# eragonruan/text-detection-ctpn

Hardware: AMD Instinct MI355X
Metric: images/sec at 600x900 (VGG16-CTPN inference) (higher is better)
Workload: dtype bf16

## Files before the change

include/ctpn_hip.h:

```cpp
#ifndef CTPN_HIP_H
#define CTPN_HIP_H

#include <stddef.h>
#include <stdint.h>

#ifdef __cplusplus
extern "C" {
#endif

#define CTPN_ABI_VERSION 10

#define CTPN_OK            0
#define CTPN_ERR_ARG      -1
#define CTPN_ERR_HIP      -2
#define CTPN_ERR_STATE    -3
#define CTPN_ERR_CAPACITY -4
#define CTPN_ERR_NODEVICE -5
#define CTPN_ERR_UNSUPPORTED -6

#define CTPN_PREC_FP32  0
#define CTPN_PREC_BF16  1
#define CTPN_PREC_FP16  2
#define CTPN_PREC_SPLIT 3

// ... 59 lines not shown
                double fx, double fy, void* dst, int dst_on_device, long long dst_capacity,
                int* out_h, int* out_w);

int ctpn_nms(int* keep_out, int* num_out, const float* boxes_host, int boxes_num, int boxes_dim,
             float nms_overlap_thresh, int device_id);

int ctpn_text_lines(const float* boxes, const float* scores, int r, int im_h, int im_w, int mode,
                    int device_id, double* recs_out, int capacity, int* count_out);
int ctpn_text_lines_cfg(const float* boxes, const float* scores, int r, int im_h, int im_w, int mode,
                        int device_id, const double* cfg8, double* recs_out, int capacity, int* count_out);
int ctpn_connector_constants(double* out8);

int ctpn_result_text(const double* recs, int n_lines, double scale, char* out, size_t capacity, size_t* bytes_out, int* lines_out);
int ctpn_write_result_file(const char* path, const double* recs, int n_lines, double scale, int* lines_out);
int ctpn_draw_boxes(uint8_t* img_bgr, int h, int w, const double* recs, int n_lines);

int ctpn_detect(ctpn_ctx* ctx, const uint8_t* images, int images_on_device, int n, int h, int w,
                const float* scales, int mode, double* recs_out, int line_capacity, int* line_counts,
                float* rois_out, int* roi_counts);

int ctpn_detect_submit(ctpn_ctx* ctx, const uint8_t* images, int images_on_device, int n, int h, int w,
                       const float* scales, int slot);
int ctpn_detect_collect(ctpn_ctx* ctx, int slot, int mode, double* recs_out, int line_capacity, int* line_counts,
                        float* rois_out, int* roi_counts);

int ctpn_detect_ragged(ctpn_ctx* ctx, const uint8_t* canvas, int canvas_on_device, int n, int hc, int w, const int* heights,
                       const float* scales, int mode, double* recs_out, int line_capacity, int* line_counts,
                       float* rois_out, int* roi_counts);
int ctpn_detect_submit_ragged(ctpn_ctx* ctx, const uint8_t* canvas, int canvas_on_device, int n, int hc, int w, const int* heights,
                              const float* scales, int slot);

#define CTPN_KIND_CONV_FIRST  0
#define CTPN_KIND_CONV_GEMM   1
#define CTPN_KIND_POOL        2
#define CTPN_KIND_GEMM        3
#define CTPN_KIND_BILSTM      4
#define CTPN_KIND_DECODE      5
#define CTPN_KIND_SORT        6
#define CTPN_KIND_NMS         7
#define CTPN_KIND_COUNT       8
int ctpn_profile_enable(ctpn_ctx* ctx, int on);
int ctpn_profile_reset(ctpn_ctx* ctx);
int ctpn_profile_read(ctpn_ctx* ctx, int kind, double* ms, long long* launches, double* work);

int ctpn_debug_cvt_bf16(int device_id, const float* in, uint16_t* out, int n, int use_hw_instruction);
int ctpn_debug_lds_dma(int device_id, const uint8_t* src, size_t bytes, uint8_t* out_clobber, uint8_t* out_keep);
int ctpn_debug_conv3x3(int device_id, const float* in_nhwc, const float* w_hwio, const float* bias, int n, int h, int w,
                       int ci, int co, int precision, int impl, int fuse_pool, float* out_full, float* out_pool);
#define CTPN_CONV_PLAN_INTS 6
int ctpn_debug_conv3x3_plan(int precision, int n, int h, int w_first, int w_count, int ci, int co, int fuse_pool, int keep_full, int dup_hi,
                            int conv_p64, int split_edge, int cu_count, int* plans);
const char* ctpn_debug_conv3x3_form_name(int kind, int id);
int ctpn_debug_lstm_pre_plan(long long cells, int cu_count, int* plan_out);
int ctpn_debug_lstm_pre(int device_id, const float* x, const float* wx, const float* bias, int n, int hf, int wf, int precision, int cu_count,
                        float* out);
int ctpn_debug_bilstm(int device_id, const float* pre, const float* wh, int rows, int T, int split, int fast_gates, int pre_f16, float* out,
                      int* form_out);
int ctpn_debug_gemm(int device_id, const float* a, const float* w, const float* bias, int M, int K, int Co, int ldc, int in_precision, float* out);
int ctpn_debug_connect(int device_id, const float* rois, int r, int im_h, int im_w, float scale, int mode, double* recs_out,
                       int capacity, int* count_out);
int ctpn_debug_text_lines(ctpn_ctx* ctx, const float* rois, const int* roi_counts, int n, int im_h, int im_w, const float* scales, int mode,
                          double* recs_out, int line_capacity, int* line_counts, int* keep_out, int* keep_counts);

int    ctpn_jpeg_probe(const uint8_t* data, size_t len, int* h, int* w, int* ncomp, int* luma_sampling);
size_t ctpn_jpeg_coef_capacity(int h, int w);
int    ctpn_jpeg_entropy_decode(const uint8_t* data, size_t len, int16_t* coef, size_t coef_capacity, uint16_t* qt, int* layout8);
int    ctpn_decode_jpeg_batch(ctpn_ctx* ctx, const uint8_t* const* files, const size_t* sizes, int n, int h, int w, double fx, double fy,
                              const uint8_t** images_dev_out, int* out_h, int* out_w);
int    ctpn_decode_jpeg_files(ctpn_ctx* ctx, const char* const* paths, int n, int h, int w, double fx, double fy,
                              const uint8_t** images_dev_out, int* out_h, int* out_w);
int    ctpn_jpeg_probe_files(const char* const* paths, int n, int* info4, int threads);
int    ctpn_jpeg_batch_fetch(ctpn_ctx* ctx, const uint8_t* images_dev, uint8_t* host_out, size_t capacity);

int    ctpn_decode_jpeg_batch_device(ctpn_ctx* ctx, const uint8_t* const* files, const size_t* sizes, int n, int h, int w, double fx, double fy,
                                     const uint8_t** images_dev_out, int* out_h, int* out_w);
int    ctpn_decode_jpeg_files_device(ctpn_ctx* ctx, const char* const* paths, int n, int h, int w, double fx, double fy,
                                     const uint8_t** images_dev_out, int* out_h, int* out_w);
int    ctpn_jpeg_entropy_decode_device(ctpn_ctx* ctx, const uint8_t* const* files, const size_t* sizes, int n, int subseq_bits, int16_t* coef_out,
                                       size_t coef_capacity_per_file, uint16_t* qt_out, int* layout8_out, int* status_out);
int    ctpn_jpeg_entropy_device_stats(ctpn_ctx* ctx, long long* out4);

int    ctpn_decode_jpeg_batch_ragged(ctpn_ctx* ctx, const uint8_t* const* files, const size_t* sizes, int n, const int* file_h, const int* file_w,
                                     const double* factors, int hc, int wc, int entropy_on_device, const uint8_t** canvas_dev_out, int* heights_out);
int    ctpn_decode_jpeg_files_ragged(ctpn_ctx* ctx, const char* const* paths, int n, const int* file_h, const int* file_w, const double* factors,
                                     int hc, int wc, int entropy_on_device, const uint8_t** canvas_dev_out, int* heights_out);

size_t ctpn_jpeg_encode_capacity(int h, int w);
int    ctpn_jpeg_entropy_encode(const int16_t* coef, const int* layout8, const uint16_t* qt, uint8_t* out, size_t capacity, size_t* bytes_out);
int    ctpn_encode_jpeg_batch(ctpn_ctx* ctx, const uint8_t* images, int images_on_device, int n, int h, int w, int quality, uint8_t* const* out,
                              const size_t* capacities, size_t* bytes_out);
int    ctpn_write_annotated_files(ctpn_ctx* ctx, const uint8_t* images_dev, int n, int h, int w, const double* recs, int line_capacity,
                                  const int* line_counts, double scale, const char* const* paths, int quality);

int    ctpn_encode_jpeg_batch_device(ctpn_ctx* ctx, const uint8_t* images, int images_on_device, int n, int h, int w, int quality, uint8_t* const* out,
                                     const size_t* capacities, size_t* bytes_out);
int    ctpn_write_annotated_files_device(ctpn_ctx* ctx, const uint8_t* images_dev, int n, int h, int w, const double* recs, int line_capacity,
                                         const int* line_counts, double scale, const char* const* paths, int quality);
int    ctpn_jpeg_entropy_encode_device(ctpn_ctx* ctx, const int16_t* const* coef, const int* layout8, const uint16_t* qt, int n, uint8_t* const* out,
                                       const size_t* capacities, size_t* bytes_out, int* status_out);
int    ctpn_jpeg_entropy_encode_device_stats(ctpn_ctx* ctx, long long* out4);

int    ctpn_line_crop_width(const double* rec9, int crop_h, int max_w, int* width_out);
int    ctpn_crop_lines(ctpn_ctx* ctx, const uint8_t* images, int images_on_device, int n, int h, int w, const double* recs, int line_capacity,
                       const int* line_counts, int crop_h, int max_w, int pad_value, uint8_t* crops_out, int crops_on_device,
                       size_t capacity_bytes, int* widths_out, int* total_out);

// ... 48 lines not shown
```

text-detection-ctpn_amd/_binding.py:

```python
import collections
import ctypes as C
import os
import sys

import numpy as np

_HERE = os.path.dirname(os.path.abspath(__file__))
_LIB = None

CTPN_OK = 0
CTPN_ERR_UNSUPPORTED = -6
CTPN_ERR_CAPACITY = -4
PREC_FP32, PREC_BF16, PREC_FP16, PREC_SPLIT = 0, 1, 2, 3
PRECISIONS = {"fp32": PREC_FP32, "f32": PREC_FP32, "bf16": PREC_BF16, "fp16": PREC_FP16, "f16": PREC_FP16, "split": PREC_SPLIT}


def precision_code(p):
    if isinstance(p, int) and p in (PREC_FP32, PREC_BF16, PREC_FP16, PREC_SPLIT):
        return p
    try:
        return PRECISIONS[p]
    except KeyError:
        raise ValueError("unknown precision %r (fp32 | bf16 | fp16 | split)" % (p,))

# ... 30 lines not shown
        "ctpn_param_name": (C.c_char_p, [C.c_int]),
        "ctpn_param_default": (C.c_int, [C.c_char_p, f64p]),
        "ctpn_last_error": (C.c_char_p, []),
        "ctpn_device_count": (C.c_int, []),
        "ctpn_create": (C.c_int, [C.POINTER(vp), C.c_int, C.c_int, C.c_int, C.c_int, C.c_int]),
        "ctpn_create_postproc": (C.c_int, [C.POINTER(vp), C.c_int, C.c_int, C.c_int, C.c_int]),
        "ctpn_host_thread_budget": (C.c_int, [C.c_int, C.c_int, C.c_int]),
        "ctpn_host_threads": (C.c_int, [vp, i32p]),
        "ctpn_proposal_anchors": (C.c_int, [vp, i32p, C.c_int]),
        "ctpn_debug_connect": (C.c_int, [C.c_int, f32p, C.c_int, C.c_int, C.c_int, C.c_float, C.c_int, f64p, C.c_int, i32p]),
        "ctpn_debug_text_lines": (C.c_int, [vp, f32p, i32p, C.c_int, C.c_int, C.c_int, f32p, C.c_int, f64p, C.c_int, i32p, i32p, i32p]),
        "ctpn_destroy": (C.c_int, [vp]),
        "ctpn_sync": (C.c_int, [vp]),
        "ctpn_stream": (C.c_int, [vp, C.POINTER(vp)]),
        "ctpn_weight_manifest": (C.c_int, [C.c_int, C.POINTER(C.c_char_p), i32p, i32p, C.POINTER(C.c_size_t)]),
        "ctpn_weight_count": (C.c_int, []),
        "ctpn_load_weights_host": (C.c_int, [vp, f32p]),
        "ctpn_load_weights_device": (C.c_int, [vp, vp]),
        "ctpn_broadcast_weights": (C.c_int, [C.POINTER(vp), C.c_int]),
        "ctpn_comm_unique_id": (C.c_int, [C.c_char_p, C.c_size_t]),
        "ctpn_broadcast_weights_rank": (C.c_int, [vp, C.c_char_p, C.c_int, C.c_int, C.c_int]),
        "ctpn_forward": (C.c_int, [vp, vp, C.c_int, C.c_int, C.c_int, C.c_int]),
        "ctpn_forward_blob": (C.c_int, [vp, vp, C.c_int, C.c_int, C.c_int, C.c_int]),
        "ctpn_ragged_valid_rows": (C.c_int, [C.c_int, C.c_int]),
        "ctpn_forward_ragged": (C.c_int, [vp, vp, C.c_int, C.c_int, C.c_int, C.c_int, i32p]),
        "ctpn_detect_ragged": (C.c_int, [vp, vp, C.c_int, C.c_int, C.c_int, C.c_int, i32p, f32p, C.c_int, f64p, C.c_int, i32p, f32p, i32p]),
        "ctpn_detect_submit_ragged": (C.c_int, [vp, vp, C.c_int, C.c_int, C.c_int, C.c_int, i32p, f32p, C.c_int]),
        "ctpn_feat_shape": (C.c_int, [vp, i32p, i32p, i32p]),
        "ctpn_get_tensor": (C.c_int, [vp, C.c_char_p, f32p, C.c_size_t, i32p]),
        "ctpn_proposals": (C.c_int, [vp, f32p, C.c_int, C.c_int, C.c_float, C.c_float, f32p, i32p]),
        "ctpn_proposals_from_host": (C.c_int, [vp, f32p, f32p, C.c_int, C.c_int, C.c_int, f32p, C.c_int, C.c_int,
                                               C.c_float, C.c_float, f32p, i32p]),
        "ctpn_nms": (C.c_int, [i32p, i32p, f32p, C.c_int, C.c_int, C.c_float, C.c_int]),
        "ctpn_resize_dims": (C.c_int, [C.c_int, C.c_int, C.c_double, C.c_double, i32p, i32p]),
        "ctpn_resize": (C.c_int, [C.c_int, vp, C.c_int, C.c_int, C.c_int, C.c_int, C.c_int, C.c_double, C.c_double, vp, C.c_int,
                                  C.c_longlong, i32p, i32p]),
        "ctpn_result_text": (C.c_int, [f64p, C.c_int, C.c_double, C.c_char_p, C.c_size_t, C.POINTER(C.c_size_t), i32p]),
        "ctpn_write_result_file": (C.c_int, [C.c_char_p, f64p, C.c_int, C.c_double, i32p]),
        "ctpn_draw_boxes": (C.c_int, [u8p, C.c_int, C.c_int, f64p, C.c_int]),
        "ctpn_text_lines": (C.c_int, [f32p, f32p, C.c_int, C.c_int, C.c_int, C.c_int, C.c_int, f64p, C.c_int, i32p]),
        "ctpn_text_lines_cfg": (C.c_int, [f32p, f32p, C.c_int, C.c_int, C.c_int, C.c_int, C.c_int, f64p, f64p, C.c_int, i32p]),
        "ctpn_connector_constants": (C.c_int, [f64p]),
        "ctpn_detect": (C.c_int, [vp, vp, C.c_int, C.c_int, C.c_int, C.c_int, f32p, C.c_int, f64p, C.c_int, i32p,
                                  f32p, i32p]),
        "ctpn_detect_submit": (C.c_int, [vp, vp, C.c_int, C.c_int, C.c_int, C.c_int, f32p, C.c_int]),
        "ctpn_detect_collect": (C.c_int, [vp, C.c_int, C.c_int, f64p, C.c_int, i32p, f32p, i32p]),
        "ctpn_debug_cvt_bf16": (C.c_int, [C.c_int, f32p, C.POINTER(C.c_uint16), C.c_int, C.c_int]),
        "ctpn_debug_lds_dma": (C.c_int, [C.c_int, u8p, C.c_size_t, u8p, u8p]),
        "ctpn_debug_conv3x3": (C.c_int, [C.c_int, f32p, f32p, f32p, C.c_int, C.c_int, C.c_int, C.c_int, C.c_int, C.c_int, C.c_int,
                                         C.c_int, f32p, f32p]),
        "ctpn_debug_conv3x3_plan": (C.c_int, [C.c_int] * 13 + [i32p]),
        "ctpn_debug_conv3x3_form_name": (C.c_char_p, [C.c_int, C.c_int]),
        "ctpn_debug_lstm_pre_plan": (C.c_int, [C.c_longlong, C.c_int, i32p]),
        "ctpn_debug_lstm_pre": (C.c_int, [C.c_int, f32p, f32p, f32p, C.c_int, C.c_int, C.c_int, C.c_int, C.c_int, f32p]),
        "ctpn_debug_bilstm": (C.c_int, [C.c_int, f32p, f32p, C.c_int, C.c_int, C.c_int, C.c_int, C.c_int, f32p, i32p]),
        "ctpn_debug_gemm": (C.c_int, [C.c_int, f32p, f32p, f32p, C.c_int, C.c_int, C.c_int, C.c_int, C.c_int, f32p]),
        "ctpn_jpeg_probe": (C.c_int, [u8p, C.c_size_t, i32p, i32p, i32p, i32p]),
        "ctpn_jpeg_coef_capacity": (C.c_size_t, [C.c_int, C.c_int]),
        "ctpn_jpeg_entropy_decode": (C.c_int, [u8p, C.c_size_t, C.POINTER(C.c_int16), C.c_size_t, C.POINTER(C.c_uint16), i32p]),
        "ctpn_decode_jpeg_batch": (C.c_int, [vp, C.POINTER(u8p), C.POINTER(C.c_size_t), C.c_int, C.c_int, C.c_int, C.c_double, C.c_double,
                                             C.POINTER(vp), i32p, i32p]),
        "ctpn_jpeg_batch_fetch": (C.c_int, [vp, vp, u8p, C.c_size_t]),
        "ctpn_decode_jpeg_files": (C.c_int, [vp, C.POINTER(C.c_char_p), C.c_int, C.c_int, C.c_int, C.c_double, C.c_double, C.POINTER(vp), i32p, i32p]),
        "ctpn_jpeg_probe_files": (C.c_int, [C.POINTER(C.c_char_p), C.c_int, i32p, C.c_int]),
        "ctpn_decode_jpeg_batch_device": (C.c_int, [vp, C.POINTER(u8p), C.POINTER(C.c_size_t), C.c_int, C.c_int, C.c_int, C.c_double, C.c_double,
                                                    C.POINTER(vp), i32p, i32p]),
        "ctpn_decode_jpeg_files_device": (C.c_int, [vp, C.POINTER(C.c_char_p), C.c_int, C.c_int, C.c_int, C.c_double, C.c_double, C.POINTER(vp), i32p, i32p]),
        "ctpn_jpeg_entropy_decode_device": (C.c_int, [vp, C.POINTER(u8p), C.POINTER(C.c_size_t), C.c_int, C.c_int, C.POINTER(C.c_int16), C.c_size_t,
                                                      C.POINTER(C.c_uint16), i32p, i32p]),
        "ctpn_jpeg_entropy_device_stats": (C.c_int, [vp, C.POINTER(C.c_longlong)]),
        "ctpn_decode_jpeg_batch_ragged": (C.c_int, [vp, C.POINTER(u8p), C.POINTER(C.c_size_t), C.c_int, i32p, i32p, f64p, C.c_int, C.c_int, C.c_int,
                                                    C.POINTER(vp), i32p]),
        "ctpn_decode_jpeg_files_ragged": (C.c_int, [vp, C.POINTER(C.c_char_p), C.c_int, i32p, i32p, f64p, C.c_int, C.c_int, C.c_int, C.POINTER(vp), i32p]),
        "ctpn_jpeg_encode_capacity": (C.c_size_t, [C.c_int, C.c_int]),
        "ctpn_jpeg_entropy_encode": (C.c_int, [C.POINTER(C.c_int16), i32p, C.POINTER(C.c_uint16), u8p, C.c_size_t, C.POINTER(C.c_size_t)]),
        "ctpn_encode_jpeg_batch": (C.c_int, [vp, vp, C.c_int, C.c_int, C.c_int, C.c_int, C.c_int, C.POINTER(vp), C.POINTER(C.c_size_t),
                                             C.POINTER(C.c_size_t)]),
        "ctpn_write_annotated_files": (C.c_int, [vp, vp, C.c_int, C.c_int, C.c_int, f64p, C.c_int, i32p, C.c_double, C.POINTER(C.c_char_p), C.c_int]),
        "ctpn_encode_jpeg_batch_device": (C.c_int, [vp, vp, C.c_int, C.c_int, C.c_int, C.c_int, C.c_int, C.POINTER(vp), C.POINTER(C.c_size_t),
                                                    C.POINTER(C.c_size_t)]),
        "ctpn_write_annotated_files_device": (C.c_int, [vp, vp, C.c_int, C.c_int, C.c_int, f64p, C.c_int, i32p, C.c_double, C.POINTER(C.c_char_p), C.c_int]),
        "ctpn_jpeg_entropy_encode_device": (C.c_int, [vp, C.POINTER(C.POINTER(C.c_int16)), i32p, C.POINTER(C.c_uint16), C.c_int, C.POINTER(vp), C.POINTER(C.c_size_t),
                                                      C.POINTER(C.c_size_t), i32p]),
        "ctpn_jpeg_entropy_encode_device_stats": (C.c_int, [vp, C.POINTER(C.c_longlong)]),
        "ctpn_line_crop_width": (C.c_int, [f64p, C.c_int, C.c_int, i32p]),
        "ctpn_crop_lines": (C.c_int, [vp, vp, C.c_int, C.c_int, C.c_int, C.c_int, f64p, C.c_int, i32p, C.c_int, C.c_int, C.c_int, vp, C.c_int, C.c_size_t,
                                      i32p, i32p]),
        "ctpn_encode_jpeg_mixed": (C.c_int, [vp, vp, C.c_int, C.c_size_t, C.c_int, i32p, i32p, C.POINTER(C.c_size_t), C.POINTER(C.c_size_t), C.c_int,
                                             C.POINTER(vp), C.POINTER(C.c_size_t), C.POINTER(C.c_size_t)]),
        "ctpn_encode_jpeg_mixed_device": (C.c_int, [vp, vp, C.c_int, C.c_size_t, C.c_int, i32p, i32p, C.POINTER(C.c_size_t), C.POINTER(C.c_size_t), C.c_int,
                                                    C.POINTER(vp), C.POINTER(C.c_size_t), C.POINTER(C.c_size_t)]),
        "ctpn_write_line_crops": (C.c_int, [vp, vp, C.c_int, C.c_int, C.c_int, C.c_int, f64p, C.c_int, i32p, C.c_int, C.c_int, C.c_int, C.c_int,
                                            C.POINTER(C.c_char_p), i32p, i32p]),
        "ctpn_write_line_crops_device": (C.c_int, [vp, vp, C.c_int, C.c_int, C.c_int, C.c_int, f64p, C.c_int, i32p, C.c_int, C.c_int, C.c_int, C.c_int,
                                                   C.POINTER(C.c_char_p), i32p, i32p]),
        "ctpn_write_annotated_files_ragged": (C.c_int, [vp, vp, C.c_int, C.c_int, C.c_int, C.c_int, i32p, f64p, C.c_int, i32p, f64p, C.POINTER(C.c_char_p),
                                                        C.c_int]),
        "ctpn_write_annotated_files_ragged_device": (C.c_int, [vp, vp, C.c_int, C.c_int, C.c_int, C.c_int, i32p, f64p, C.c_int, i32p, f64p,
                                                               C.POINTER(C.c_char_p), C.c_int]),
        "ctpn_crop_lines_ragged": (C.c_int, [vp, vp, C.c_int, C.c_int, C.c_int, C.c_int, i32p, f64p, C.c_int, i32p, C.c_int, C.c_int, C.c_int, vp, C.c_int,
                                             C.c_size_t, i32p, i32p]),
        "ctpn_write_line_crops_ragged": (C.c_int, [vp, vp, C.c_int, C.c_int, C.c_int, C.c_int, i32p, f64p, C.c_int, i32p, C.c_int, C.c_int, C.c_int, C.c_int,
                                                   C.POINTER(C.c_char_p), i32p, i32p]),
        "ctpn_write_line_crops_ragged_device": (C.c_int, [vp, vp, C.c_int, C.c_int, C.c_int, C.c_int, i32p, f64p, C.c_int, i32p, C.c_int, C.c_int, C.c_int, C.c_int,
                                                          C.POINTER(C.c_char_p), i32p, i32p]),
        "ctpn_debug_png_backend": (C.c_int, [C.c_int]),
# ... 528 lines not shown
    out = np.zeros((rows, T, 256), np.float32)
    form = C.c_int(-1)
    _check(load_library().ctpn_debug_bilstm(int(device_id), _ptr(pre, C.c_float), _ptr(wh, C.c_float), rows, T, 1 if split else 0,
                                            1 if fast_gates else 0, 1 if pre_f16 else 0, _ptr(out, C.c_float), C.byref(form)))
    return out, BILSTM_FORMS[form.value]


def debug_gemm(a, w, bias, ldc=None, precision="fp32", device_id=0):
    a = _f32(a); w = _f32(w); bias = _f32(bias)
    (M, K), Co = a.shape, w.shape[1]
    assert w.shape[0] == K and bias.shape == (Co,)
    ldc = Co if ldc is None else int(ldc)
    out = np.zeros((M, ldc), np.float32)
    _check(load_library().ctpn_debug_gemm(int(device_id), _ptr(a, C.c_float), _ptr(w, C.c_float), _ptr(bias, C.c_float), M, K, Co, ldc,
                                          precision_code(precision), _ptr(out, C.c_float)))
    return out


class Context:

    def __init__(self, device_id=0, max_batch=1, max_h=600, max_w=900, precision="bf16", postproc_only=False, options=None):
        self._lib = load_library()
        self._h = C.c_void_p()
        self.precision = precision
        self.postproc_only = bool(postproc_only)
        prec = precision_code(precision)
        if postproc_only:
            _check(self._lib.ctpn_create_postproc(C.byref(self._h), int(device_id), int(max_batch), int(max_h) // 16, int(max_w) // 16))
        else:
            _check(self._lib.ctpn_create(C.byref(self._h), int(device_id), int(max_batch), int(max_h), int(max_w), prec))
        self.device_id = device_id
        self.max_batch, self.max_h, self.max_w = max_batch, max_h, max_w
        opts = {k: int(os.environ[e]) for k, e in OPTION_ENV.items() if os.environ.get(e, "") != ""}
        opts.update(options or {})
        for k, v in opts.items():
            self.set_option(k, v)

    def set_option(self, key, value):
        _check(self._lib.ctpn_set_option(self._h, key.encode(), int(value)))

    def get_option(self, key):
        v = C.c_int(0)
        _check(self._lib.ctpn_get_option(self._h, key.encode(), C.byref(v)))
        return v.value

    def set_param(self, name, value):
        _check(self._lib.ctpn_set_param(self._h, name.encode(), float(value)))

    def get_param(self, name):
        v = C.c_double(0.0)
        _check(self._lib.ctpn_get_param(self._h, name.encode(), C.byref(v)))
        return v.value

    def host_threads(self):
        n = C.c_int(0)
        _check(self._lib.ctpn_host_threads(self._h, C.byref(n)))
        return n.value

    def close(self):
        if getattr(self, "_h", None) is not None and self._h.value:
            self._lib.ctpn_destroy(self._h)
            self._h = C.c_void_p()

    def __del__(self):
        try:
            self.close()
        except Exception:
            pass

    def __enter__(self):
        return self

    def __exit__(self, *a):
        self.close()

    def load_weights(self, arena):
        a = _f32(arena).reshape(-1)
        from .weights import WEIGHT_FLOATS
        if a.size != WEIGHT_FLOATS:
            raise ValueError("weight arena must hold %d floats, got %d" % (WEIGHT_FLOATS, a.size))
        _check(self._lib.ctpn_load_weights_host(self._h, _ptr(a, C.c_float)))

    def load_weights_device(self, dev_ptr):
        _check(self._lib.ctpn_load_weights_device(self._h, C.c_void_p(int(dev_ptr))))

    def broadcast_weights_rank(self, unique_id, rank, world, root=0):
        if len(unique_id) != COMM_ID_BYTES:
            raise ValueError("unique_id must be %d bytes" % COMM_ID_BYTES)
        _check(self._lib.ctpn_broadcast_weights_rank(self._h, C.c_char_p(bytes(unique_id)), int(rank), int(world), int(root)))

    def forward(self, images, device_ptr=None, shape=None):
        if device_ptr is not None:
            n, h, w = shape
            _check(self._lib.ctpn_forward(self._h, C.c_void_p(int(device_ptr)), 1, int(n), int(h), int(w)))
            return
        im = np.ascontiguousarray(images, dtype=np.uint8)
        if im.ndim == 3:
            im = im[None]
        n, h, w, c = im.shape
        assert c == 3
        self._keepalive = im
        _check(self._lib.ctpn_forward(self._h, im.ctypes.data_as(C.c_void_p), 0, n, h, w))

    @staticmethod
    def _canvas(canvas, heights, device_ptr, shape):
        if device_ptr is not None:
# ... 486 lines not shown
```

text-detection-ctpn_amd/csrc/api_ctx.hip:

```cpp
#include "ctx.h"

namespace ctpn {

static thread_local std::string t_err;
void set_error(const std::string& s) { t_err = s; }
int fail(int code, const std::string& s) { t_err = s; return code; }

static int env_int(const char* name, int dflt) { const char* v = std::getenv(name); return v && *v ? std::atoi(v) : dflt; }

static int dev_alloc(ctpn_ctx* c, void** p, size_t bytes, bool zero) {
  if (bytes == 0) bytes = 256;
  CTPN_HIP_TRY(hipMalloc(p, bytes));
  c->allocs.push_back(*p);
  if (zero) CTPN_HIP_TRY(hipMemsetAsync(*p, 0, bytes, c->stream));
  return CTPN_OK;
}

int debug_sync() { static const int v = env_int("CTPN_DEBUG_SYNC", 0); return v; }
const RoctxApi& roctx_api() {
  static const RoctxApi api = [] {
    RoctxApi a;
    if (!env_int("CTPN_ROCTX", 0)) return a;
    void* h = dlopen("librocprofiler-sdk-roctx.so", RTLD_NOW | RTLD_GLOBAL);
    if (!h) h = dlopen("librocprofiler-sdk-roctx.so.1", RTLD_NOW | RTLD_GLOBAL);
    if (!h) {
      const char* rp = std::getenv("ROCM_PATH");
      const std::string p = std::string(rp && *rp ? rp : "/opt/rocm") + "/lib/librocprofiler-sdk-roctx.so";
      h = dlopen(p.c_str(), RTLD_NOW | RTLD_GLOBAL);
    }
    if (h) {
      a.push = (int (*)(const char*))dlsym(h, "roctxRangePushA");
      a.pop = (int (*)())dlsym(h, "roctxRangePop");
      if (!a.push || !a.pop) { a.push = nullptr; a.pop = nullptr; }
    }
    return a;
  }();
  return api;
}
int roctx_on() { return roctx_api().push != nullptr; }

static int prof_drain(ctpn_ctx* c) {
  if (c->pending.empty()) return CTPN_OK;
  CTPN_HIP_TRY(hipStreamSynchronize(c->stream));
  CTPN_HIP_TRY(hipStreamSynchronize(c->stream_p));
  for (auto& r : c->pending) {
    float ms = 0.f;
    if (hipEventElapsedTime(&ms, r.a, r.b) == hipSuccess) {
      c->prof_ms[r.kind] += ms; c->prof_n[r.kind] += r.launches; c->prof_work[r.kind] += r.work;
    }
    c->free_events.push_back(r.a); c->free_events.push_back(r.b);
  }
  c->pending.clear();
  return CTPN_OK;
}

struct PackLayout { size_t tlb, tls, keep, kcnt, rois, rcnt, total; };
static PackLayout pack_layout(size_t mb, size_t post) {
  auto al = [](size_t x) { return (x + 255) & ~(size_t)255; };
  PackLayout L; size_t o = 0;
  L.tlb = o; o = al(o + mb * post * 4 * sizeof(float));
  L.tls = o; o = al(o + mb * post * sizeof(float));
  L.keep = o; o = al(o + mb * post * sizeof(int));
  L.kcnt = o; o = al(o + mb * sizeof(int));
  L.rois = o; o = al(o + mb * post * 5 * sizeof(float));
  L.rcnt = o; o = al(o + mb * sizeof(int));
  L.total = o;
  return L;
}

static int create_impl(ctpn_ctx** out, int device_id, int max_batch, int max_h, int max_w, int precision, bool postproc_only) {
  if (!out) return fail(CTPN_ERR_ARG, "ctpn_create: out is null");
  *out = nullptr;
  if (max_batch <= 0 || max_h < 16 || max_w < 16) return fail(CTPN_ERR_ARG, "ctpn_create: max_batch > 0 and max_h, max_w >= 16 required");
  if (precision < CTPN_PREC_FP32 || precision > CTPN_PREC_SPLIT) return fail(CTPN_ERR_ARG, "ctpn_create: unknown precision");
  int ndev = ctpn_device_count();
  if (ndev <= 0) return fail(CTPN_ERR_NODEVICE, "ctpn_create: no HIP device visible (this library has no CPU fallback)");
  if (device_id < 0 || device_id >= ndev) {
    const char* hv = getenv("HIP_VISIBLE_DEVICES");
    const char* rv = getenv("ROCR_VISIBLE_DEVICES");
    return fail(CTPN_ERR_ARG, "ctpn_create: device_id " + std::to_string(device_id) + " out of range: " + std::to_string(ndev) +
                " device(s) visible (HIP_VISIBLE_DEVICES=" + (hv ? hv : "unset") + ", ROCR_VISIBLE_DEVICES=" + (rv ? rv : "unset") + "); one process per GPU needs LOCAL_RANK < that count");
  }
  CTPN_HIP_TRY(hipSetDevice(device_id));
  hipDeviceProp_t prop;
  CTPN_HIP_TRY(hipGetDeviceProperties(&prop, device_id));
  if (std::string(prop.gcnArchName).find("gfx950") == std::string::npos)
    return fail(CTPN_ERR_NODEVICE, std::string("ctpn_create: device is ") + prop.gcnArchName + ", kernels are built for gfx950 only");

  ctpn_ctx* c = new ctpn_ctx();
  c->device = device_id; c->max_batch = max_batch; c->max_h = max_h; c->max_w = max_w;
  c->prec = prec_dtype(precision);
  c->es = dtype_bytes(c->prec);
  c->wx_row_bytes = c->prec == DType::SPLIT ? (size_t)3 * 512 * 2 : (size_t)512 * c->es;
  c->lstm_split = (dtype_is_half(c->prec) || c->prec == DType::SPLIT) ? 1 : 0;
  c->tail_confine = 0;
  c->postproc_only = postproc_only;
  for (int i = 0; i < TAIL_PARAM_COUNT; ++i) c->tail_raw[i] = tail_param(i)->dflt;
  {
    const unsigned hw = std::thread::hardware_concurrency();
    c->host_threads = ctpn_host_thread_budget((int)(hw ? hw : 1), env_int("LOCAL_WORLD_SIZE", 1), env_int("CTPN_HOST_THREADS", 0));
    const int first_cpu = env_int("CTPN_AFFINITY", 0) ? env_int("LOCAL_RANK", 0) * c->host_threads : -1;
    c->pool.reset(new HostPool(c->host_threads, first_cpu));
  }
  int rc = CTPN_OK;
  auto A = [&](void** p, size_t bytes, bool zero) { if (rc == CTPN_OK) rc = dev_alloc(c, p, bytes, zero); };
  if (hipStreamCreateWithFlags(&c->stream, hipStreamNonBlocking) != hipSuccess) { delete c; return fail(CTPN_ERR_HIP, "hipStreamCreate failed"); }
  if (hipStreamCreateWithFlags(&c->stream_p, hipStreamNonBlocking) != hipSuccess) { (void)hipStreamDestroy(c->stream); delete c; return fail(CTPN_ERR_HIP, "hipStreamCreate failed"); }
  if (hipEventCreateWithFlags(&c->ev_conv, hipEventDisableTiming) != hipSuccess || hipEventCreateWithFlags(&c->ev_tail, hipEventDisableTiming) != hipSuccess) {
    ctpn_destroy(c); return fail(CTPN_ERR_HIP, "ctpn_create: events");
  }
  for (auto& sl : c->slot) {
    const size_t mb = (size_t)max_batch;
    const PackLayout L = pack_layout(mb, (size_t)c->post_max);
    bool ok = hipHostMalloc((void**)&sl.pack, L.total) == hipSuccess;
    if (ok) {
      sl.tlb = (float*)(sl.pack + L.tlb); sl.tls = (float*)(sl.pack + L.tls); sl.keep = (int*)(sl.pack + L.keep); sl.kcnt = (int*)(sl.pack + L.kcnt);
      sl.rois = (float*)(sl.pack + L.rois); sl.rcnt = (int*)(sl.pack + L.rcnt);
    }
    ok = ok &&
              hipHostMalloc((void**)&sl.im_info, mb * 3 * sizeof(float)) == hipSuccess &&
              hipHostMalloc((void**)&sl.crecs, mb * 2 * CONN_CAP * 9 * sizeof(double)) == hipSuccess &&
              hipHostMalloc((void**)&sl.ccnt, mb * 3 * sizeof(int)) == hipSuccess &&
              hipEventCreateWithFlags(&sl.ev_heads, hipEventDisableTiming) == hipSuccess &&
              hipEventCreateWithFlags(&sl.ev_decoded, hipEventDisableTiming) == hipSuccess &&
              hipEventCreateWithFlags(&sl.ev_done, hipEventDisableTiming) == hipSuccess;
    if (!ok) { ctpn_destroy(c); return fail(CTPN_ERR_HIP, "ctpn_create: pinned host buffers / events"); }
  }

  const int hf = lvl(max_h, 4), wf = lvl(max_w, 4);
  c->m5_max = (size_t)max_batch * hf * wf;
  if (!postproc_only) {
  A((void**)&c->arena, (size_t)CTPN_WEIGHT_FLOATS * sizeof(float), false);
  A((void**)&c->w_first, 27 * 64 * sizeof(float), false);
  A(&c->w_first_frags, CF_FRAGS_TOTAL, true);
  for (int i = 0; i < 14; ++i) {
    A((void**)&c->b_conv[i], (size_t)kConvs[i].co * sizeof(float), true);
    if (i > 0) A(&c->wt_conv[i], (size_t)kConvs[i].co * 9 * kConvs[i].ci * (c->prec == DType::SPLIT ? 6 : c->es), true);
  }
  A(&c->wt_x, (size_t)1024 * c->wx_row_bytes, true);
  if (dtype_is_half(c->prec)) A(&c->wt_xf, (size_t)1024 * 512 * 2, true);
  A((void**)&c->b_x, 1024 * sizeof(float), true);
  A((void**)&c->wh, (size_t)2 * 128 * 512 * sizeof(float), true);
  A((void**)&c->wt_fc, (size_t)512 * 256 * sizeof(float), true);
  A((void**)&c->b_fc, 512 * sizeof(float), true);
  A((void**)&c->wt_h, (size_t)64 * 512 * sizeof(float), true);
  A((void**)&c->b_h, 64 * sizeof(float), true);
  A((void**)&c->wt_fold, (size_t)64 * 256 * sizeof(float), true);
  A((void**)&c->b_fold, 64 * sizeof(float), true);

  for (int i = 0; i < 14; ++i) {
    const int hl = lvl(max_h, kConvs[i].level), wl = lvl(max_w, kConvs[i].level);
    const size_t pix_b = (size_t)kConvs[i].co * ((c->prec == DType::SPLIT && i == 13) ? 6 : c->es);
    c->act_conv_bytes[i] = ((size_t)max_batch * (hl + 2) * (wl + 2) + act_slack_pixels(wl)) * pix_b;
    const size_t front = act_front_pixels(wl) * pix_b;
    A(&c->act_conv[i], front + c->act_conv_bytes[i], true);
    if (c->act_conv[i]) c->act_conv[i] = (char*)c->act_conv[i] + front;
  }
  {
    const int pool_src[4] = {1, 3, 6, 9};
    for (int p = 0; p < 4; ++p) {
      const int hl = lvl(max_h, p + 1), wl = lvl(max_w, p + 1);
      c->act_pool_bytes[p] = ((size_t)max_batch * (hl + 2) * (wl + 2) + act_slack_pixels(wl)) * kConvs[pool_src[p]].co * c->es;
      const size_t front = act_front_pixels(wl) * kConvs[pool_src[p]].co * c->es;
      A(&c->act_pool[p], front + c->act_pool_bytes[p], true);
      if (c->act_pool[p]) c->act_pool[p] = (char*)c->act_pool[p] + front;
    }
  }
  if (dtype_is_half(c->prec)) { c->q_img_bytes = conv1_q_bytes(max_batch, max_h, max_w); A(&c->q_img, c->q_img_bytes, true); }
  A((void**)&c->img_dev, (size_t)max_batch * max_h * max_w * 3 * sizeof(float), false);
  c->img_dev_b[0] = c->img_dev;
  A((void**)&c->img_dev_b[1], (size_t)max_batch * max_h * max_w * 3 * sizeof(float), false);
  if (rc == CTPN_OK) {
    bool ok = hipStreamCreateWithFlags(&c->stream_c, hipStreamNonBlocking) == hipSuccess;
    for (int b = 0; b < 2 && ok; ++b)
      ok = hipEventCreateWithFlags(&c->ev_copied[b], hipEventDisableTiming) == hipSuccess && hipEventCreateWithFlags(&c->ev_consumed[b], hipEventDisableTiming) == hipSuccess;
    if (!ok) rc = fail(CTPN_ERR_HIP, "ctpn_create: copy stream / events");
  }
  A((void**)&c->xp, c->m5_max * 1024 * sizeof(float), false);
  A((void**)&c->lstm_out, c->m5_max * 256 * sizeof(float), false);
  A((void**)&c->fc_out, c->m5_max * 512 * sizeof(float), false);
  A((void**)&c->heads, c->m5_max * 64 * sizeof(float), true);
  }
  A((void**)&c->cls_prob, c->m5_max * 20 * sizeof(float), false);
  A((void**)&c->bbox_pred, c->m5_max * 40 * sizeof(float), false);
  A((void**)&c->cls_in, c->m5_max * 20 * sizeof(float), false);
  A((void**)&c->bbox_in, c->m5_max * 40 * sizeof(float), false);
  c->npad_max = next_pow2(hf * wf * 10);
  A((void**)&c->keys, (size_t)max_batch * c->npad_max * sizeof(unsigned long long), false);
  A((void**)&c->keys_tmp, (size_t)max_batch * c->npad_max * sizeof(unsigned long long), false);
  A((void**)&c->boxes4, (size_t)max_batch * hf * wf * 10 * 4 * sizeof(float), false);
  A((void**)&c->sorted_boxes, (size_t)max_batch * c->topn_max * 4 * sizeof(float), false);
  A((void**)&c->sorted_scores, (size_t)max_batch * c->topn_max * sizeof(float), false);
  A((void**)&c->valid_counts, (size_t)max_batch * sizeof(int), true);
  A((void**)&c->keep_idx, (size_t)max_batch * c->topn_max * sizeof(int), false);
  {
    const PackLayout L = pack_layout((size_t)max_batch, (size_t)c->post_max);
    c->pack_bytes = L.total;
    A((void**)&c->out_pack, L.total, true);
    if (c->out_pack) {
      c->tl_boxes = (float*)(c->out_pack + L.tlb); c->tl_scores = (float*)(c->out_pack + L.tls); c->tl_keep = (int*)(c->out_pack + L.keep);
      c->tl_keep_counts = (int*)(c->out_pack + L.kcnt); c->rois = (float*)(c->out_pack + L.rois); c->keep_counts = (int*)(c->out_pack + L.rcnt);
    }
  }
  A((void**)&c->kept_spill, (size_t)max_batch * c->topn_max * 4 * sizeof(float), false);
  A((void**)&c->sorted_anchor, (size_t)max_batch * c->topn_max * sizeof(int), false);
  A((void**)&c->roi_anchor, (size_t)max_batch * c->post_max * sizeof(int), true);
  A((void**)&c->tl_counts, (size_t)max_batch * sizeof(int), true);
  A((void**)&c->tl_spill, (size_t)max_batch * c->post_max * 4 * sizeof(float), false);
  A((void**)&c->nms_mw_scratch, (size_t)NMS_MW_CAP_BATCH * NMS_MW_SCRATCH_BYTES, true);
  A((void**)&c->nms_colid, (size_t)NMS_MW_CAP_BATCH * ((c->topn_max + 15) & ~15), true);
  A((void**)&c->conn_recs, (size_t)max_batch * 2 * CONN_CAP * 9 * sizeof(double), false);
  A((void**)&c->conn_counts, (size_t)max_batch * 3 * sizeof(int), true);
  A((void**)&c->conn_scratch, (size_t)max_batch * 1024 * 20 * sizeof(double), false);
  A((void**)&c->im_info_dev, (size_t)max_batch * 3 * sizeof(float), true);
  if (rc == CTPN_OK && hipStreamSynchronize(c->stream) != hipSuccess) rc = fail(CTPN_ERR_HIP, "ctpn_create: sync failed");
  if (rc != CTPN_OK) { ctpn_destroy(c); return rc; }
  *out = c;
  return CTPN_OK;
}

struct Option { const char* name; int ctpn_ctx::* member; int lo, hi; };
static const Option kOptions[] = {
    {"keep_acts", &ctpn_ctx::keep_acts, 0, 1},
    {"conv1_kernel", &ctpn_ctx::conv1_mfma, 0, 2},
    {"conv1_fuse", &ctpn_ctx::conv1_fuse, 0, 1},
    {"lstm_split", &ctpn_ctx::lstm_split, 0, 1},
    {"nms_columns", &ctpn_ctx::nms_columns, 0, 3},
    {"nms_check", &ctpn_ctx::nms_check, 0, 1},
    {"connect_device", &ctpn_ctx::connect_device, 0, 1},
    {"tail_overlap", &ctpn_ctx::tail_overlap, 0, 1},
    {"conv_p64", &ctpn_ctx::conv_p64, 0, 1},
    {"tail_confine", &ctpn_ctx::tail_confine, 0, 1},
    {"nms_prefix", &ctpn_ctx::nms_prefix, 0, 1},
    {"debug_hog", &ctpn_ctx::debug_hog, 0, 200000},
    {"debug_nms", &ctpn_ctx::debug_nms, 0, 15},
    {"split_edge", &ctpn_ctx::split_edge, 0, 1},
};
static const Option* find_option(const std::string& k) {
  for (const Option& o : kOptions) if (k == o.name) return &o;
  return nullptr;
}

}

extern "C" {

int ctpn_abi_version(void) { return CTPN_ABI_VERSION; }
const char* ctpn_last_error(void) { return t_err.c_str(); }
int ctpn_device_count(void) {
  int n = 0;
  if (hipGetDeviceCount(&n) != hipSuccess) return 0;
  return n;
}

int ctpn_host_thread_budget(int cpu_count, int local_world_size, int requested) {
  if (requested > 0) return requested > 256 ? 256 : requested;
  if (cpu_count < 1) cpu_count = 1;
  if (local_world_size < 1) local_world_size = 1;
  int b = cpu_count / local_world_size;
  return b < 1 ? 1 : (b > 32 ? 32 : b);
}

int ctpn_create(ctpn_ctx** out, int device_id, int max_batch, int max_h, int max_w, int precision) {
  return create_impl(out, device_id, max_batch, max_h, max_w, precision, false);
}

int ctpn_create_postproc(ctpn_ctx** out, int device_id, int max_batch, int max_hf, int max_wf) {
  if (max_hf < 1 || max_wf < 1 || max_hf > (1 << 20) / 16 || max_wf > (1 << 20) / 16) return fail(CTPN_ERR_ARG, "ctpn_create_postproc: feature-map size out of range");
  return create_impl(out, device_id, max_batch, max_hf * 16, max_wf * 16, CTPN_PREC_FP32, true);
}

int ctpn_option_count(void) { return (int)(sizeof(kOptions) / sizeof(kOptions[0])); }
const char* ctpn_option_name(int index) { return index >= 0 && index < ctpn_option_count() ? kOptions[index].name : nullptr; }
int ctpn_set_option(ctpn_ctx* c, const char* key, int value) {
  if (!c || !key) return fail(CTPN_ERR_ARG, "ctpn_set_option: null pointer");
  const Option* o = find_option(key);
  if (!o) return fail(CTPN_ERR_ARG, std::string("ctpn_set_option: unknown option ") + key);
  if (value < o->lo || value > o->hi) return fail(CTPN_ERR_ARG, std::string("ctpn_set_option: value out of range for ") + key);
  if (c->*(o->member) == value) return CTPN_OK;
  CTPN_HIP_TRY(hipSetDevice(c->device));
  CTPN_HIP_TRY(hipStreamSynchronize(c->stream));
  CTPN_HIP_TRY(hipStreamSynchronize(c->stream_p));
  for (auto& sl : c->slot) if (sl.busy) return fail(CTPN_ERR_STATE, "ctpn_set_option: a submitted batch has not been collected");
  c->tail_pending = false;
  c->nms_mw_dirty = true;
  c->*(o->member) = value;
  return CTPN_OK;
}
int ctpn_get_option(ctpn_ctx* c, const char* key, int* value_out) {
  if (!c || !key || !value_out) return fail(CTPN_ERR_ARG, "ctpn_get_option: null pointer");
  const Option* o = find_option(key);
  if (!o) return fail(CTPN_ERR_ARG, std::string("ctpn_get_option: unknown option ") + key);
  *value_out = c->*(o->member);
  return CTPN_OK;
}

int ctpn_set_param(ctpn_ctx* c, const char* name, double value) {
  if (!c || !name) return fail(CTPN_ERR_ARG, "ctpn_set_param: null pointer");
  const int idx = tail_param_index(name);
  if (idx < 0) return fail(CTPN_ERR_ARG, std::string("ctpn_set_param: unknown parameter ") + name);
  if (!tail_param_ok(idx, value)) return fail(CTPN_ERR_ARG, std::string("ctpn_set_param: value out of range for ") + name);
  if (c->tail_raw[idx] == value) return CTPN_OK;
  CTPN_HIP_TRY(hipSetDevice(c->device));
  CTPN_HIP_TRY(hipStreamSynchronize(c->stream));
  CTPN_HIP_TRY(hipStreamSynchronize(c->stream_p));
  for (auto& sl : c->slot) if (sl.busy) return fail(CTPN_ERR_STATE, "ctpn_set_param: a submitted batch has not been collected");
  c->tail_pending = false;
  c->nms_mw_dirty = true;
  c->tail_raw[idx] = value;
  switch (idx) {
    case TP_RPN_PRE_NMS_TOP_N: c->rpn_pre = (int)value; break;
    case TP_RPN_POST_NMS_TOP_N: c->rpn_post = (int)value; break;
    case TP_RPN_NMS_THRESH: c->rpn_nms_thresh = (float)value; break;
    case TP_RPN_MIN_SIZE: c->rpn_min_size = (float)value; break;
    default: connector_cfg_set(c->conn, idx, value); break;
  }
  return CTPN_OK;
}
int ctpn_get_param(ctpn_ctx* c, const char* name, double* value_out) {
  if (!c || !name || !value_out) return fail(CTPN_ERR_ARG, "ctpn_get_param: null pointer");
  const int idx = tail_param_index(name);
  if (idx < 0) return fail(CTPN_ERR_ARG, std::string("ctpn_get_param: unknown parameter ") + name);
  *value_out = c->tail_raw[idx];
  return CTPN_OK;
}

int ctpn_host_threads(ctpn_ctx* c, int* threads_out) {
  if (!c || !threads_out) return fail(CTPN_ERR_ARG, "null pointer");
  *threads_out = c->host_threads;
  return CTPN_OK;
}

int ctpn_destroy(ctpn_ctx* c) {
  if (!c) return CTPN_OK;
  (void)hipSetDevice(c->device);
  if (c->stream) (void)hipStreamSynchronize(c->stream);
  if (c->stream_p) (void)hipStreamSynchronize(c->stream_p);
  if (c->stream_c) { (void)hipStreamSynchronize(c->stream_c); (void)hipStreamDestroy(c->stream_c); }
  for (int b = 0; b < 2; ++b) { if (c->pin_stage[b]) (void)hipHostFree(c->pin_stage[b]); if (c->ev_h2d_done[b]) (void)hipEventDestroy(c->ev_h2d_done[b]); }
  for (int b = 0; b < 2; ++b) { if (c->ev_copied[b]) (void)hipEventDestroy(c->ev_copied[b]); if (c->ev_consumed[b]) (void)hipEventDestroy(c->ev_consumed[b]); }
  for (auto& sl : c->slot) {
    for (void* p : {(void*)sl.pack, (void*)sl.im_info, (void*)sl.crecs, (void*)sl.ccnt}) if (p) (void)hipHostFree(p);
    for (hipEvent_t e : {sl.ev_heads, sl.ev_decoded, sl.ev_done}) if (e) (void)hipEventDestroy(e);
  }
  for (hipEvent_t e : {c->ev_conv, c->ev_tail}) if (e) (void)hipEventDestroy(e);
  for (auto& r : c->ragged) { if (r.host) (void)hipHostFree(r.host); if (r.dev) (void)hipFree(r.dev); if (r.ev_copied) (void)hipEventDestroy(r.ev_copied); }
  if (c->ragged_blob) (void)hipFree(c->ragged_blob);
  for (auto& j : c->jpeg) {
    if (j.coef_host) (void)hipHostFree(j.coef_host);
    if (j.qt_host) (void)hipHostFree(j.qt_host);
    if (j.tab_host) (void)hipHostFree(j.tab_host);
    for (void* p : {(void*)j.coef_dev, (void*)j.qt_dev, (void*)j.out_dev, (void*)j.tab_dev}) if (p) (void)hipFree(p);
    for (hipEvent_t e : {j.ev_h2d, j.ev_ready, j.ev_consumed}) if (e) (void)hipEventDestroy(e);
  }
  for (void* p : {(void*)c->jpeg_planes, (void*)c->jpeg_raw}) if (p) (void)hipFree(p);
  for (void* p : {(void*)c->jh.stage_dev, (void*)c->jh.work_dev}) if (p) (void)hipFree(p);
  for (void* p : {(void*)c->jh.stage_host, (void*)c->jh.res_host}) if (p) (void)hipHostFree(p);
  for (void* p : c->jpeg_retired) (void)hipFree(p);
  for (void* p : {(void*)c->stage.img_dev, (void*)c->stage.rs_dev, (void*)c->stage.recs_dev, (void*)c->stage.cnt_dev, (void*)c->stage.rm_dev}) if (p) (void)hipFree(p);
  if (c->stage.rm_host) (void)hipHostFree(c->stage.rm_host);
  for (void* p : {(void*)c->enc.coef_dev, c->enc.qtab_dev, (void*)c->enc.huff_dev, c->enc.huff_tab_dev, (void*)c->enc.mix_dev}) if (p) (void)hipFree(p);
  for (void* p : {(void*)c->enc.coef_host, c->enc.qtab_host, (void*)c->enc.huff_host, (void*)c->enc.scan_host, (void*)c->enc.mix_host}) if (p) (void)hipHostFree(p);
  if (c->enc.ev_done) (void)hipEventDestroy(c->enc.ev_done);
  if (c->pnge.dev) (void)hipFree(c->pnge.dev);
  for (void* p : {(void*)c->pnge.host, (void*)c->pnge.file_host}) if (p) (void)hipHostFree(p);
  if (c->pnge.ev_done) (void)hipEventDestroy(c->pnge.ev_done);
  for (void* p : {(void*)c->crop.img_dev, (void*)c->crop.out_dev, c->crop.desc_dev}) if (p) (void)hipFree(p);
  if (c->crop.desc_host) (void)hipHostFree(c->crop.desc_host);
  if (c->crop.ev_done) (void)hipEventDestroy(c->crop.ev_done);
  if (c->stream_p) (void)hipStreamDestroy(c->stream_p);
  for (auto& r : c->pending) { (void)hipEventDestroy(r.a); (void)hipEventDestroy(r.b); }
  for (auto e : c->free_events) (void)hipEventDestroy(e);
  for (void* p : c->allocs) (void)hipFree(p);
  if (c->stream) (void)hipStreamDestroy(c->stream);
  delete c;
  return CTPN_OK;
}

int ctpn_sync(ctpn_ctx* c) {
  if (!c) return fail(CTPN_ERR_ARG, "null ctx");
  CTPN_HIP_TRY(hipStreamSynchronize(c->stream));
  CTPN_HIP_TRY(hipStreamSynchronize(c->stream_p));
  if (c->stream_c) CTPN_HIP_TRY(hipStreamSynchronize(c->stream_c));
  return CTPN_OK;
}
int ctpn_stream(ctpn_ctx* c, void** stream_out) {
  if (!c || !stream_out) return fail(CTPN_ERR_ARG, "null pointer");
  *stream_out = (void*)c->stream;
  return CTPN_OK;
}

int ctpn_profile_enable(ctpn_ctx* c, int on) {
  if (!c) return fail(CTPN_ERR_ARG, "null ctx");
  if (!on) { int rc = prof_drain(c); if (rc) return rc; }
  c->prof = on != 0;
  c->prof_mode = on == 2 ? 2 : 1;
  return CTPN_OK;
}
int ctpn_profile_reset(ctpn_ctx* c) {
  if (!c) return fail(CTPN_ERR_ARG, "null ctx");
  int rc = prof_drain(c);
  if (rc) return rc;
  for (int k = 0; k < CTPN_KIND_COUNT; ++k) { c->prof_ms[k] = 0; c->prof_n[k] = 0; c->prof_work[k] = 0; }
  return CTPN_OK;
}
int ctpn_profile_read(ctpn_ctx* c, int kind, double* ms, long long* launches, double* work) {
  if (!c) return fail(CTPN_ERR_ARG, "null ctx");
  if (kind < 0 || kind >= CTPN_KIND_COUNT) return fail(CTPN_ERR_ARG, "kind out of range");
  int rc = prof_drain(c);
  if (rc) return rc;
  if (ms) *ms = c->prof_ms[kind];
  if (launches) *launches = c->prof_n[kind];
  if (work) *work = c->prof_work[kind];
  return CTPN_OK;
}

}
```

text-detection-ctpn_amd/csrc/api_debug.hip:

```cpp
#include "ctx.h"
#include "conv3x3_plan.h"

extern "C" {

int ctpn_debug_cvt_bf16(int device_id, const float* in, uint16_t* out, int n, int use_hw_instruction) {
  if (!in || !out || n <= 0) return fail(CTPN_ERR_ARG, "ctpn_debug_cvt_bf16: bad argument");
  if (ctpn_device_count() <= 0) return fail(CTPN_ERR_NODEVICE, "ctpn_debug_cvt_bf16: no HIP device visible (no CPU fallback)");
  CTPN_HIP_TRY(hipSetDevice(device_id));
  float* d_in = nullptr; uint16_t* d_out = nullptr;
  CTPN_HIP_TRY(hipMalloc((void**)&d_in, (size_t)n * 4));
  CTPN_HIP_TRY(hipMalloc((void**)&d_out, (size_t)n * 2 + 4));
  CTPN_HIP_TRY(hipMemcpy(d_in, in, (size_t)n * 4, hipMemcpyHostToDevice));
  int rc = launch_cvt_bf16(d_in, d_out, n, use_hw_instruction, nullptr);
  if (!rc && hipDeviceSynchronize() != hipSuccess) rc = fail(CTPN_ERR_HIP, "ctpn_debug_cvt_bf16: kernel failed");
  if (!rc && hipMemcpy(out, d_out, (size_t)n * 2, hipMemcpyDeviceToHost) != hipSuccess) rc = fail(CTPN_ERR_HIP, "ctpn_debug_cvt_bf16: copy failed");
  (void)hipFree(d_in); (void)hipFree(d_out);
  return rc;
}

int ctpn_debug_lds_dma(int device_id, const uint8_t* src, size_t bytes, uint8_t* out_clobber, uint8_t* out_keep) {
  if (!src || !out_clobber || !out_keep || bytes == 0 || bytes % 1024 != 0 || bytes > ((size_t)1 << 30)) return fail(CTPN_ERR_ARG, "ctpn_debug_lds_dma: bytes must be a positive multiple of 1024 (<= 1 GiB)");
  if (ctpn_device_count() <= 0) return fail(CTPN_ERR_NODEVICE, "ctpn_debug_lds_dma: no HIP device visible (no CPU fallback)");
  CTPN_HIP_TRY(hipSetDevice(device_id));
  char *d_in = nullptr, *d_a = nullptr, *d_b = nullptr;
// ... 114 lines not shown
        out_pool[(((size_t)in * ho + y) * wo + x) * co + c] = std::max(std::max(at(2 * y, 2 * x), at(2 * y, 2 * x + 1)), std::max(at(2 * y + 1, 2 * x), at(2 * y + 1, 2 * x + 1)));
      }
  }
  if (!rc && out_pool && fuse_pool && !host_pool) rc = fetch(d_pool, ho, wo, out_pool, 0);
  return rc;
}

int ctpn_debug_conv3x3_plan(int precision, int n, int h, int w_first, int w_count, int ci, int co, int fuse_pool, int keep_full, int dup_hi,
                            int conv_p64, int split_edge, int cu_count, int* plans) {
  if (!plans || w_count <= 0) return fail(CTPN_ERR_ARG, "ctpn_debug_conv3x3_plan: no output");
  if (precision < CTPN_PREC_FP32 || precision > CTPN_PREC_SPLIT) return fail(CTPN_ERR_ARG, "ctpn_debug_conv3x3_plan: unknown precision");
  const DType t = prec_dtype(precision);
  if (n <= 0 || h <= 0 || w_first <= 0 || w_first > 0x7fffffff - w_count || ci <= 0 || ci % (t == DType::F32 ? 32 : 64) != 0 || co <= 0 || co % (t == DType::F32 ? 4 : 8) != 0)
    return fail(CTPN_ERR_ARG, "ctpn_debug_conv3x3_plan: shape out of range (Ci a multiple of 32 / 64, Co of 4 / 8)");
  if (dup_hi && t != DType::SPLIT) return fail(CTPN_ERR_ARG, "ctpn_debug_conv3x3_plan: dup_hi is a split-precision layout");
  if (cu_count < 0) return fail(CTPN_ERR_ARG, "ctpn_debug_conv3x3_plan: cu_count is a CU count, or 0 for the current device's");
  if (cu_count == 0) {
    if (ctpn_device_count() <= 0) return fail(CTPN_ERR_NODEVICE, "ctpn_debug_conv3x3_plan: cu_count 0 asks the current device, and no HIP device is visible");
    int dev = 0, rc;
    if ((rc = current_device(dev)) || (rc = device_cu_count(dev, cu_count))) return rc;
  }
  for (int i = 0; i < w_count; ++i) {
    const C3Plan p = c3_plan(t, n, h, w_first + i, ci, co, fuse_pool != 0, keep_full != 0 || !fuse_pool, dup_hi, true, true, (conv_p64 ? 1 : 0) | (split_edge ? 2 : 0), cu_count);
    if (p.main_form == C3M_NONE) return fail(CTPN_ERR_ARG, "ctpn_debug_conv3x3_plan: no kernel for this shape (split precision: Co <= 64 or a multiple of 128)");
    int* o = plans + (size_t)i * CTPN_CONV_PLAN_INTS;
    o[0] = p.main_form; o[1] = p.strip; o[2] = p.strip_cols; o[3] = p.w_cover; o[4] = p.deep; o[5] = p.edge_ks;
  }
  return CTPN_OK;
}

const char* ctpn_debug_conv3x3_form_name(int kind, int id) { return kind == 0 ? c3_main_name(id) : (kind == 1 ? c3_strip_name(id) : nullptr); }

}
namespace {
constexpr int DBG_GUARD_ROWS = 64;
constexpr int DBG_FILL = 0xC3;
bool dbg_fill_intact(const char* p, size_t n) {
  for (size_t i = 0; i < n; ++i) if ((unsigned char)p[i] != DBG_FILL) return false;
  return true;
}
inline uint16_t dbg_to16(DType t, float v) { return t == DType::F16 ? host_f32_to_f16(v) : host_f32_to_bf16(v); }
struct DevBufs {
  std::vector<void*> p;
  ~DevBufs() { for (void* q : p) if (q) (void)hipFree(q); }
  int alloc(void** out, size_t bytes) {
    CTPN_HIP_TRY(hipMalloc(out, bytes));
    p.push_back(*out);
    return CTPN_OK;
  }
};
}
extern "C" {

int ctpn_debug_lstm_pre_plan(long long cells, int cu_count, int* plan_out) {
  if (!plan_out) return fail(CTPN_ERR_ARG, "ctpn_debug_lstm_pre_plan: no output");
  if (cells <= 0 || cells > 0x7fffffffLL) return fail(CTPN_ERR_ARG, "ctpn_debug_lstm_pre_plan: cells out of range (1 .. 2^31 - 1)");
  if (cu_count < 0) return fail(CTPN_ERR_ARG, "ctpn_debug_lstm_pre_plan: cu_count is a CU count, or 0 for the current device's");
  if (cu_count == 0) {
    if (ctpn_device_count() <= 0) return fail(CTPN_ERR_NODEVICE, "ctpn_debug_lstm_pre_plan: cu_count 0 asks the current device, and no HIP device is visible");
    int dev = 0, rc;
    if ((rc = current_device(dev)) || (rc = device_cu_count(dev, cu_count))) return rc;
  }
  const LstmPrePlan p = lstm_pre_plan(cells, cu_count);
  plan_out[0] = p.small ? 0 : 1; plan_out[1] = p.waves; plan_out[2] = (int)p.workgroups; plan_out[3] = p.idle_waves;
  return CTPN_OK;
}

int ctpn_debug_lstm_pre(int device_id, const float* x, const float* wx, const float* bias, int n, int hf, int wf, int precision, int cu_count, float* out) {
  if (!x || !wx || !bias || !out) return fail(CTPN_ERR_ARG, "ctpn_debug_lstm_pre: null pointer");
  if (precision < CTPN_PREC_FP32 || precision > CTPN_PREC_SPLIT) return fail(CTPN_ERR_ARG, "ctpn_debug_lstm_pre: unknown precision");
  if (n <= 0 || hf <= 0 || wf <= 0 || (long long)n * hf * wf > (1 << 24)) return fail(CTPN_ERR_ARG, "ctpn_debug_lstm_pre: n, hf, wf positive, at most 2^24 cells");
  if (cu_count < 0) return fail(CTPN_ERR_ARG, "ctpn_debug_lstm_pre: cu_count is a CU count, or 0 for the current device's");
  if (ctpn_device_count() <= 0) return fail(CTPN_ERR_NODEVICE, "ctpn_debug_lstm_pre: no HIP device visible (no CPU fallback)");
  CTPN_HIP_TRY(hipSetDevice(device_id));
  const DType t = prec_dtype(precision);
  const bool split = t == DType::SPLIT, half = dtype_is_half(t);
  const long long M = (long long)n * hf * wf;
  const int Hp = hf + 2, Wp = wf + 2;
  const int es = t == DType::F32 ? 4 : 2, pix = split ? 1536 : 512;
  const int oes = half ? 2 : 4;
  std::vector<char> hin((size_t)n * Hp * Wp * pix * es);
  auto put = [&](size_t pixel, int c, float v) {
    const size_t o = pixel * pix + c;
    if (t == DType::F32) { std::memcpy(&hin[o * 4], &v, 4); return; }
    const uint16_t b = dbg_to16(t, v);
    std::memcpy(&hin[o * 2], &b, 2);
    if (split) {
      const uint16_t l = host_f32_to_bf16(v - host_bf16_to_f32(b));
      std::memcpy(&hin[(o + 512) * 2], &l, 2);
      std::memcpy(&hin[(o + 1024) * 2], &b, 2);
    }
  };
  for (int in = 0; in < n; ++in) for (int y = 0; y < Hp; ++y) for (int xx = 0; xx < Wp; ++xx) {
    const size_t pixel = ((size_t)in * Hp + y) * Wp + xx;
    const bool inside = y >= 1 && y <= hf && xx >= 1 && xx <= wf;
    const float* src = inside ? x + (((size_t)in * hf + (y - 1)) * wf + (xx - 1)) * 512 : nullptr;
    for (int c = 0; c < 512; ++c) put(pixel, c, inside ? src[c] : 3e4f);
  }
  DevBufs bufs;
  void *d_a = nullptr, *d_wx = nullptr, *d_b = nullptr, *d_wt = nullptr, *d_wtf = nullptr, *d_bx = nullptr, *d_out = nullptr;
  const size_t row_bytes = split ? (size_t)3 * 512 * 2 : (size_t)512 * es;
  const size_t out_bytes = (size_t)M * 1024 * oes, guard_bytes = (size_t)DBG_GUARD_ROWS * 1024 * oes;
  int rc;
  if ((rc = bufs.alloc(&d_a, hin.size())) || (rc = bufs.alloc(&d_wx, (size_t)512 * 1024 * 4)) || (rc = bufs.alloc(&d_b, 1024 * 4)) ||
      (rc = bufs.alloc(&d_wt, 1024 * row_bytes)) || (half && (rc = bufs.alloc(&d_wtf, (size_t)1024 * 512 * 2))) || (rc = bufs.alloc(&d_bx, 1024 * 4)) ||
      (rc = bufs.alloc(&d_out, out_bytes + guard_bytes))) return rc;
// ... 115 lines not shown
```

text-detection-ctpn_amd/csrc/api_detect.hip:

```cpp
#include "ctx.h"

namespace ctpn {

static int enqueue_text_lines(ctpn_ctx* c, ctpn_ctx::Slot& sl, int n, int w, hipStream_t p, int* nms_form = nullptr) {
  const int post = c->rpn_post;
  const float tl_thresh = c->conn.nms_thresh;
  int rc;
  {
    Timed t(c, CTPN_KIND_NMS, (double)n * post * 24.0, p);
    if ((rc = launch_lines_prep(c->rois, c->keep_counts, c->im_info_dev, post, c->conn.min_score, c->tl_boxes, c->tl_scores, c->tl_counts, n, p))) return rc;
    float max_scale = 0.f;
    for (int i = 0; i < n; ++i) max_scale = sl.im_info[3 * i + 2] > max_scale ? sl.im_info[3 * i + 2] : max_scale;
    if (c->nms_columns && nms_columns_tl_ok(lvl(w, 4), post, tl_thresh, max_scale)) {
      const bool mw = nms_multi_wg(c, n, 0);
      if (nms_form) *nms_form = mw ? 2 : 1;
      if ((rc = launch_nms_columns(c->tl_boxes, c->tl_scores, c->tl_counts, post, tl_thresh, post, c->tl_keep, post, c->tl_keep_counts, nullptr,
                                   c->tl_spill, n, lvl(w, 4), p, nullptr, nullptr, c->im_info_dev, mw ? c->nms_mw_scratch : nullptr))) return rc;
    } else {
      if (nms_form) *nms_form = 0;
      if ((rc = launch_nms(c->tl_boxes, c->tl_scores, c->tl_counts, post, tl_thresh, post, c->tl_keep, post, c->tl_keep_counts, nullptr,
                           c->tl_spill, n, p))) return rc;
    }
  }
  if (c->connect_device) {
    if ((rc = launch_connect(c->tl_boxes, c->tl_scores, c->tl_keep, c->tl_keep_counts, post, c->im_info_dev, c->conn_recs, c->conn_counts,
                             c->conn_scratch, CONN_CAP, n, c->conn, p))) return rc;
    CTPN_HIP_TRY(hipMemcpyAsync(sl.crecs, c->conn_recs, (size_t)n * 2 * CONN_CAP * 9 * sizeof(double), hipMemcpyDeviceToHost, p));
    CTPN_HIP_TRY(hipMemcpyAsync(sl.ccnt, c->conn_counts, (size_t)n * 3 * sizeof(int), hipMemcpyDeviceToHost, p));
  }
  return CTPN_OK;
}

static int detect_submit_body(ctpn_ctx* c, const uint8_t* images, int images_on_device, int n, int h, int w, const float* scales, int slot, bool lone,
                              const int* heights) {
  if (!c) return fail(CTPN_ERR_ARG, "ctpn_detect_submit: null ctx");
  if (slot < 0 || slot > 1) return fail(CTPN_ERR_ARG, "ctpn_detect_submit: slot must be 0 or 1");
  ctpn_ctx::Slot& sl = c->slot[slot];
  if (sl.busy) return fail(CTPN_ERR_STATE, "ctpn_detect_submit: slot still holds an uncollected batch");
  int rc = forward_impl(c, images, 0, images_on_device, n, h, w, c->tail_overlap != 0, heights, slot);
  if (rc) {
    const std::string first = ctpn_last_error();
    (void)hipStreamSynchronize(c->stream); (void)hipStreamSynchronize(c->stream_p);
    c->tail_pending = false; c->ev_last_decoded = nullptr; c->ev_last_done = nullptr;
    return fail(rc, first);
  }
  sl.hts.assign(n, h);
  if (heights) sl.hts.assign(heights, heights + n);
  for (int i = 0; i < n; ++i) { sl.im_info[3 * i] = (float)sl.hts[i]; sl.im_info[3 * i + 1] = (float)w; sl.im_info[3 * i + 2] = scales ? scales[i] : 1.0f; }
  hipStream_t p = lone ? c->stream : c->stream_p;
  if (!lone) {
    CTPN_HIP_TRY(hipEventRecord(sl.ev_heads, c->stream));
    CTPN_HIP_TRY(hipStreamWaitEvent(p, sl.ev_heads, 0));
  }
  rc = enqueue_proposals(c, c->heads, 0, n, lvl(h, 4), lvl(w, 4), sl.im_info, c->rpn_pre, c->rpn_post, c->rpn_nms_thresh, c->rpn_min_size, p, sl.ev_decoded,
                         c->fwd_ragged >= 0 ? c->ragged[c->fwd_ragged].dev + n : nullptr);
  if (rc) return rc;
  c->ev_last_decoded = sl.ev_decoded;
  if ((rc = enqueue_text_lines(c, sl, n, w, p))) return rc;
  CTPN_HIP_TRY(hipMemcpyAsync(sl.pack, c->out_pack, c->pack_bytes, hipMemcpyDeviceToHost, p));
  CTPN_HIP_TRY(hipEventRecord(sl.ev_done, p));
  c->ev_last_done = sl.ev_done;
  sl.n = n; sl.h = h; sl.w = w; sl.busy = true;
  return CTPN_OK;
}
static int detect_submit_impl(ctpn_ctx* c, const uint8_t* images, int images_on_device, int n, int h, int w, const float* scales, int slot, bool lone,
                              const int* heights = nullptr) {
  const int rc = detect_submit_body(c, images, images_on_device, n, h, w, scales, slot, lone, heights);
  if (rc != CTPN_OK && c) c->nms_mw_dirty = true;
  return rc;
}

static int lines_of_slot(ctpn_ctx* c, ctpn_ctx::Slot& sl, int n, int w, int mode, double* recs_out, int line_capacity, int* line_counts) {
  const int post = c->rpn_post;
  const ConnectorCfg cfg = c->conn;
  if (c->connect_device) {
    for (int i = 0; i < n; ++i) {
      if (sl.ccnt[3 * i + 2] != 0) return fail(CTPN_ERR_ARG, "text_lines: proposal x1 outside the image (reference raises IndexError)");
      const int cnt = sl.ccnt[3 * i + (mode == CTPN_MODE_O ? 1 : 0)];
      line_counts[i] = cnt;
      if (cnt > line_capacity || cnt > CONN_CAP) return fail(CTPN_ERR_CAPACITY, "ctpn_detect: more lines than line_capacity");
      if (cnt) std::memcpy(recs_out + (size_t)i * line_capacity * 9, sl.crecs + ((size_t)i * 2 + (mode == CTPN_MODE_O ? 1 : 0)) * CONN_CAP * 9, (size_t)cnt * 9 * sizeof(double));
    }
    return CTPN_OK;
  }
  std::vector<int> status(n, 0);
  std::vector<std::string> errs(n);
  auto work = [&](int i) {
    const int nk = sl.kcnt[i];
    std::vector<float> kb((size_t)nk * 4), ks(nk);
    for (int j = 0; j < nk; ++j) {
      const int src = sl.keep[(size_t)i * post + j];
      std::memcpy(&kb[4 * j], &sl.tlb[((size_t)i * post + src) * 4], 4 * sizeof(float));
      ks[j] = sl.tls[(size_t)i * post + src];
    }
    std::vector<double> recs;
    int st = connect_lines(kb.data(), ks.data(), nk, sl.hts[i], w, mode, cfg, recs);
    if (st) { status[i] = st; errs[i] = ctpn_last_error(); return; }
    const int cnt = (int)(recs.size() / 9);
    line_counts[i] = cnt;
    if (cnt > line_capacity) { status[i] = CTPN_ERR_CAPACITY; errs[i] = "ctpn_detect: more lines than line_capacity"; return; }
    if (cnt) std::memcpy(recs_out + (size_t)i * line_capacity * 9, recs.data(), recs.size() * sizeof(double));
  };
  c->pool->run(n, work);
  for (int i = 0; i < n; ++i) if (status[i]) return fail(status[i], errs[i]);
  return CTPN_OK;
}

static int debug_text_lines_body(ctpn_ctx* c, const float* rois, const int* roi_counts, int n, int im_h, int im_w, const float* scales, int mode,
                                 double* recs_out, int line_capacity, int* line_counts, int* keep_out, int* keep_counts) {
  if (!rois || !roi_counts || !recs_out || !line_counts) return fail(CTPN_ERR_ARG, "ctpn_debug_text_lines: null pointer");
  if (keep_out && !keep_counts) return fail(CTPN_ERR_ARG, "ctpn_debug_text_lines: keep_out without keep_counts");
  if (mode != CTPN_MODE_H && mode != CTPN_MODE_O) return fail(CTPN_ERR_ARG, "ctpn_debug_text_lines: mode must be H(0) or O(1)");
  if (n <= 0 || n > c->max_batch) return fail(CTPN_ERR_CAPACITY, "ctpn_debug_text_lines: 1 <= n <= max_batch images");
  if (im_h < 1 || im_w < 16 || line_capacity < 0) return fail(CTPN_ERR_ARG, "ctpn_debug_text_lines: im_h >= 1, im_w >= 16, line_capacity >= 0 required");
  const int post = c->rpn_post, post_max = c->post_max;
  for (int i = 0; i < n; ++i)
    if (roi_counts[i] < 0 || roi_counts[i] > post) return fail(CTPN_ERR_ARG, "ctpn_debug_text_lines: 0 <= roi_counts[i] <= RPN_POST_NMS_TOP_N (1000) rows of [score,x1,y1,x2,y2]");
  if (c->slot[0].busy || c->slot[1].busy) return fail(CTPN_ERR_STATE, "ctpn_debug_text_lines: a submitted batch has not been collected");
  CTPN_HIP_TRY(hipSetDevice(c->device));
  CTPN_HIP_TRY(hipStreamSynchronize(c->stream));
  CTPN_HIP_TRY(hipStreamSynchronize(c->stream_p));
  ctpn_ctx::Slot& sl = c->slot[0];
  hipStream_t p = c->stream_p;
  sl.hts.assign(n, im_h);
  for (int i = 0; i < n; ++i) { sl.im_info[3 * i] = (float)im_h; sl.im_info[3 * i + 1] = (float)im_w; sl.im_info[3 * i + 2] = scales ? scales[i] : 1.0f; }
  if (c->nms_mw_scratch && c->nms_mw_dirty) {
    CTPN_HIP_TRY(hipMemsetAsync(c->nms_mw_scratch, 0, (size_t)NMS_MW_CAP_BATCH * NMS_MW_SCRATCH_BYTES, p));
    c->nms_mw_dirty = false;
  }
  CTPN_HIP_TRY(hipMemcpyAsync(c->im_info_dev, sl.im_info, (size_t)n * 3 * sizeof(float), hipMemcpyHostToDevice, p));
  if (post == post_max) CTPN_HIP_TRY(hipMemcpyAsync(c->rois, rois, (size_t)n * post * 5 * sizeof(float), hipMemcpyHostToDevice, p));
  else CTPN_HIP_TRY(hipMemcpy2DAsync(c->rois, (size_t)post * 5 * sizeof(float), rois, (size_t)post_max * 5 * sizeof(float), (size_t)post * 5 * sizeof(float), n, hipMemcpyHostToDevice, p));
  CTPN_HIP_TRY(hipMemcpyAsync(c->keep_counts, roi_counts, (size_t)n * sizeof(int), hipMemcpyHostToDevice, p));
  int form = 0, rc;
  if ((rc = enqueue_text_lines(c, sl, n, im_w, p, &form))) return rc;
  CTPN_HIP_TRY(hipMemcpyAsync(sl.pack, c->out_pack, c->pack_bytes, hipMemcpyDeviceToHost, p));
  CTPN_HIP_TRY(hipStreamSynchronize(p));
  for (int i = 0; i < n; ++i)
    if (sl.kcnt[i] < 0 || sl.kcnt[i] > post) return fail(CTPN_ERR_HIP, "ctpn_debug_text_lines: device returned an impossible keep count");
  if (keep_counts) std::memcpy(keep_counts, sl.kcnt, (size_t)n * sizeof(int));
  if (keep_out) for (int i = 0; i < n; ++i) std::memcpy(keep_out + (size_t)i * post_max, sl.keep + (size_t)i * post, (size_t)post * sizeof(int));
  if (c->nms_check && form != 0 &&
      (rc = nms_check_generic(c, c->tl_boxes, c->tl_scores, c->tl_counts, post, c->conn.nms_thresh, post, sl.keep, post, sl.kcnt, n, form == 2, p, "connector NMS"))) return rc;
  return lines_of_slot(c, sl, n, im_w, mode, recs_out, line_capacity, line_counts);
}

}

extern "C" {

int ctpn_text_lines_cfg(const float* boxes, const float* scores, int r, int im_h, int im_w, int mode, int device_id, const double* cfg8,
                        double* recs_out, int capacity, int* count_out) {
  if (!count_out) return fail(CTPN_ERR_ARG, "ctpn_text_lines: count_out is null");
  *count_out = 0;
  if (r > 0 && (!boxes || !scores)) return fail(CTPN_ERR_ARG, "ctpn_text_lines: null input");
  ConnectorCfg cfg = default_connector_cfg();
  int rc = connector_cfg_from8(cfg8, cfg);
  if (rc) return rc;
  std::vector<double> recs;
  rc = text_lines_host(boxes, scores, r, im_h, im_w, mode, device_id, cfg, recs);
  if (rc) return rc;
  const int cnt = (int)(recs.size() / 9);
  *count_out = cnt;
  if (cnt > capacity) return fail(CTPN_ERR_CAPACITY, "ctpn_text_lines: more lines than capacity");
  if (cnt && !recs_out) return fail(CTPN_ERR_ARG, "ctpn_text_lines: recs_out is null");
  if (cnt) std::memcpy(recs_out, recs.data(), recs.size() * sizeof(double));
  return CTPN_OK;
}

int ctpn_text_lines(const float* boxes, const float* scores, int r, int im_h, int im_w, int mode, int device_id, double* recs_out,
                    int capacity, int* count_out) {
  return ctpn_text_lines_cfg(boxes, scores, r, im_h, im_w, mode, device_id, nullptr, recs_out, capacity, count_out);
}
// ... 110 lines not shown
```

text-detection-ctpn_amd/csrc/api_forward.hip:

```cpp
#include "ctx.h"

namespace ctpn {

static void parallel_memcpy(HostPool* pool, void* dst, const void* src, size_t bytes) {
  const size_t chunk = (size_t)8 << 20;
  const int nt = (int)std::min<size_t>(8, (bytes + chunk - 1) / chunk);
  if (nt <= 1 || !pool) { std::memcpy(dst, src, bytes); return; }
  const size_t per = ((bytes + nt - 1) / nt + 63) & ~(size_t)63;
  pool->run(nt, [=](int i) {
    const size_t lo = (size_t)i * per, hi = std::min(bytes, lo + per);
    if (lo < hi) std::memcpy((char*)dst + lo, (const char*)src + lo, hi - lo);
  }, 8);
}

static int ragged_upload(ctpn_ctx* c, ctpn_ctx::RaggedSet& r, const int* heights, int n, hipStream_t s) {
  if (!r.host) {
    CTPN_HIP_TRY(hipHostMalloc((void**)&r.host, (size_t)c->max_batch * 2 * sizeof(int)));
    CTPN_HIP_TRY(hipMalloc((void**)&r.dev, (size_t)c->max_batch * 2 * sizeof(int)));
    CTPN_HIP_TRY(hipEventCreateWithFlags(&r.ev_copied, hipEventDisableTiming));
  }
  if (r.copied_valid) CTPN_HIP_TRY(hipEventSynchronize(r.ev_copied));
  for (int i = 0; i < n; ++i) { r.host[i] = heights[i]; r.host[n + i] = ragged_valid_rows(heights[i], 4); }
  CTPN_HIP_TRY(hipMemcpyAsync(r.dev, r.host, (size_t)n * 2 * sizeof(int), hipMemcpyHostToDevice, s));
  CTPN_HIP_TRY(hipEventRecord(r.ev_copied, s));
  r.copied_valid = true;
  return CTPN_OK;
}

static int ragged_mask_act(void* buf, size_t pix_bytes, int level, const int* heights, const int* heights_dev, int n, int hc, int w, hipStream_t s) {
  const int hl = lvl(hc, level), wl = lvl(w, level);
  RaggedMap m;
  m.row_bytes = (long long)(wl + 2) * (long long)pix_bytes; m.img_bytes = (long long)(hl + 2) * m.row_bytes;
  m.top = 1; m.left_bytes = (int)pix_bytes; m.span_bytes = (int)(wl * pix_bytes); m.rows = hl; m.level = level;
  int pad = 0;
  for (int i = 0; i < n; ++i) pad = std::max(pad, hl - ragged_valid_rows(heights[i], level));
  return launch_ragged_mask(buf, m, heights_dev, n, pad, s);
}

int forward_impl(ctpn_ctx* c, const void* images, int is_f32, int images_on_device, int n, int h, int w, bool tail_on_p, const int* heights, int rset) {
  if (!c || !images) return fail(CTPN_ERR_ARG, "null pointer");
  if (c->postproc_only) return fail(CTPN_ERR_STATE, "ctpn_forward: post-processing-only ctx (ctpn_create_postproc) has no network");
  if (!c->weights_loaded) return fail(CTPN_ERR_STATE, "ctpn_forward: weights not loaded");
  if (n <= 0 || n > c->max_batch || h < 16 || w < 16 || h > c->max_h || w > c->max_w)
    return fail(CTPN_ERR_CAPACITY, "ctpn_forward: batch/size outside what the ctx was created for (h, w >= 16)");
  bool ragged = false;
  if (heights) {
    if (is_f32 || rset < 0 || rset > 2) return fail(CTPN_ERR_ARG, "ragged forward: uint8 canvas only");
    for (int i = 0; i < n; ++i) {
      if (heights[i] < 16 || heights[i] > h) return fail(CTPN_ERR_ARG, "ragged forward: every height must lie in 16 .. the canvas height");
      ragged = ragged || heights[i] != h;
    }
  }
  CTPN_HIP_TRY(hipSetDevice(c->device));
  hipStream_t s = c->stream;
  int rc;
  hipStream_t ts = tail_on_p ? c->stream_p : s;
  if (!tail_on_p) {
    if (c->tail_pending) { CTPN_HIP_TRY(hipStreamWaitEvent(s, c->ev_tail, 0)); c->tail_pending = false; }
  }
  auto wait_decoded = [&]() -> int {
    if (!tail_on_p && c->ev_last_decoded) CTPN_HIP_TRY(hipStreamWaitEvent(ts, c->ev_last_decoded, 0));
    return CTPN_OK;
  };
  if (c->gn != n || c->gh != h || c->gw != w) {
    if (c->tail_pending) { CTPN_HIP_TRY(hipStreamWaitEvent(s, c->ev_tail, 0)); c->tail_pending = false; }
    for (int i = 0; i < 14; ++i) CTPN_HIP_TRY(hipMemsetAsync(c->act_conv[i], 0, c->act_conv_bytes[i], s));
    for (int p = 0; p < 4; ++p) CTPN_HIP_TRY(hipMemsetAsync(c->act_pool[p], 0, c->act_pool_bytes[p], s));
    if (c->q_img) CTPN_HIP_TRY(hipMemsetAsync(c->q_img, 0, c->q_img_bytes, s));
    c->gn = n; c->gh = h; c->gw = w;
  }
  const void* img = images;
  int staged = -1;
  if (!images_on_device) {
    staged = c->img_flip;
    c->img_flip ^= 1;
    if (c->consumed_valid[staged]) CTPN_HIP_TRY(hipStreamWaitEvent(c->stream_c, c->ev_consumed[staged], 0));
    const size_t bytes = (size_t)n * h * w * 3 * (is_f32 ? 4 : 1);
    const void* src = images;
    hipPointerAttribute_t attr;
    const bool locked = hipPointerGetAttributes(&attr, images) == hipSuccess && attr.type == hipMemoryTypeHost;
    if (!locked) {
      (void)hipGetLastError();
      if (c->pin_stage_bytes[staged] < bytes) {
        if (c->pin_stage[staged]) { CTPN_HIP_TRY(hipStreamSynchronize(c->stream_c)); CTPN_HIP_TRY(hipHostFree(c->pin_stage[staged])); c->pin_stage[staged] = nullptr; }
        CTPN_HIP_TRY(hipHostMalloc(&c->pin_stage[staged], bytes));
        c->pin_stage_bytes[staged] = bytes;
        if (!c->ev_h2d_done[staged]) CTPN_HIP_TRY(hipEventCreateWithFlags(&c->ev_h2d_done[staged], hipEventDisableTiming));
        c->h2d_valid[staged] = false;
      }
      if (c->h2d_valid[staged]) CTPN_HIP_TRY(hipEventSynchronize(c->ev_h2d_done[staged]));
      parallel_memcpy(c->pool.get(), c->pin_stage[staged], images, bytes);
      src = c->pin_stage[staged];
    }
    CTPN_HIP_TRY(hipMemcpyAsync(c->img_dev_b[staged], src, bytes, hipMemcpyHostToDevice, c->stream_c));
    if (!locked) { CTPN_HIP_TRY(hipEventRecord(c->ev_h2d_done[staged], c->stream_c)); c->h2d_valid[staged] = true; }
    CTPN_HIP_TRY(hipEventRecord(c->ev_copied[staged], c->stream_c));
    CTPN_HIP_TRY(hipStreamWaitEvent(s, c->ev_copied[staged], 0));
    img = c->img_dev_b[staged];
  }
  c->n = n; c->h = h; c->w = w;
  c->fwd_ragged = ragged ? rset : -1;
  const int* hts_dev = nullptr;
  if (ragged) {
    if ((rc = ragged_upload(c, c->ragged[rset], heights, n, s))) return rc;
    hts_dev = c->ragged[rset].dev;
  }
  int jpeg_src = -1;
  if (images_on_device && c->jpeg_ready)
    for (int b = 0; b < 2; ++b)
      if (c->jpeg[b].ready_valid && images == (const void*)c->jpeg[b].out_dev) {
        CTPN_HIP_TRY(hipStreamWaitEvent(s, c->jpeg[b].ev_ready, 0));
        jpeg_src = b;
      }
  bool via_q = false, fuse1 = false;
  {
    Timed t(c, CTPN_KIND_CONV_FIRST, (double)n * h * w * (3.0 + 64.0 * c->es));
    const bool frags = c->prec == DType::SPLIT || (c->conv1_mfma && dtype_is_half(c->prec));
    via_q = !is_f32 && dtype_is_half(c->prec) && c->conv1_mfma >= 2 && c->q_img != nullptr;
    fuse1 = via_q && c->conv1_fuse && !c->keep_acts && !ragged && conv1_fusable(c->prec, n, h, w, 64, 64, true, false);
    if (via_q) {
      if ((rc = launch_image_to_q((const uint8_t*)img, c->q_img, c->prec, n, h, w, s))) return rc;
      if (ragged) {
        RaggedMap m;
        m.row_bytes = (long long)conv1_q_w(w) * 8; m.img_bytes = (long long)conv1_q_h(h) * m.row_bytes;
        m.top = 2; m.left_bytes = 16; m.span_bytes = w * 8; m.rows = h; m.level = 0;
        int pad = 0;
        for (int i = 0; i < n; ++i) pad = std::max(pad, h - heights[i]);
        if ((rc = launch_ragged_mask(c->q_img, m, hts_dev, n, pad, s))) return rc;
      }
      if (!fuse1 && (rc = launch_conv_first_from_q(c->q_img, conv1_p_frags(c->w_first_frags, c->prec), c->act_conv[0], c->prec, n, h, w, 0, w, s))) return rc;
    } else if (ragged) {
      const size_t need = (size_t)n * h * w * 3 * sizeof(float);
      if (need > c->ragged_blob_bytes) {
        CTPN_HIP_TRY(hipStreamSynchronize(s));
        if ((rc = grow_dev((void**)&c->ragged_blob, c->ragged_blob_bytes, need))) return rc;
      }
      if ((rc = launch_ragged_blob((const uint8_t*)img, c->ragged_blob, hts_dev, n, h, w, s))) return rc;
      if ((rc = launch_conv_first(c->ragged_blob, 1, c->w_first, c->b_conv[0], c->act_conv[0], c->prec, n, h, w, s,
                                  frags ? c->w_first_frags : nullptr))) return rc;
    } else if ((rc = launch_conv_first(img, is_f32, c->w_first, c->b_conv[0], c->act_conv[0], c->prec, n, h, w, s,
                                       frags ? c->w_first_frags : nullptr))) return rc;
    if (ragged && (rc = ragged_mask_act(c->act_conv[0], (size_t)64 * c->es, 0, heights, hts_dev, n, h, w, s))) return rc;
  }
  c->act_valid[0] = !fuse1;
  if (jpeg_src >= 0) {
    CTPN_HIP_TRY(hipEventRecord(c->jpeg[jpeg_src].ev_consumed, s));
    c->jpeg[jpeg_src].consumed_valid = true;
  }
  if (staged >= 0) {
    CTPN_HIP_TRY(hipEventRecord(c->ev_consumed[staged], s));
    c->consumed_valid[staged] = true;
  }
  if (c->tail_pending) { CTPN_HIP_TRY(hipStreamWaitEvent(s, c->ev_tail, 0)); c->tail_pending = false; }
  if (c->tail_confine && c->ev_last_done) CTPN_HIP_TRY(hipStreamWaitEvent(s, c->ev_last_done, 0));
  const void* cur = c->act_conv[0];
  int pool_i = 0;
  hipEvent_t stack_a = nullptr, stack_b = nullptr;
  double stack_flops = 0.0;
  const bool stack_timed = c->prof && c->prof_mode == 2;
  if (stack_timed) {
    auto get = [&]() { hipEvent_t e; if (!c->free_events.empty()) { e = c->free_events.back(); c->free_events.pop_back(); } else { (void)hipEventCreate(&e); } return e; };
    stack_a = get(); stack_b = get();
    CTPN_HIP_TRY(hipEventRecord(stack_a, s));
  }
  for (int i = 1; i < 14; ++i) {
    const int hl = lvl(h, kConvs[i].level), wl = lvl(w, kConvs[i].level);
    double flops = 2.0 * (double)n * hl * wl * 9.0 * kConvs[i].ci * kConvs[i].co;
    if (fuse1 && i == 1) flops += 2.0 * (double)n * h * w * 27.0 * 64.0;
    stack_flops += flops;
    const bool fuse = kConvs[i].pool_after != 0;
    void* full = (!fuse || c->keep_acts) ? c->act_conv[i] : nullptr;
    {
      Timed t(c, CTPN_KIND_CONV_GEMM, flops);
      const bool f1 = fuse1 && i == 1;
      if ((rc = launch_conv3x3(cur, c->wt_conv[i], c->b_conv[i], full, fuse ? c->act_pool[pool_i] : nullptr, c->prec, n, hl, wl,
                               kConvs[i].ci, kConvs[i].co, 1, s, (c->prec == DType::SPLIT && i == 13) ? 1 : 0,
                               f1 ? c->q_img : nullptr, f1 ? conv1_p_frags(c->w_first_frags, c->prec) : nullptr, (c->conv_p64 ? 1 : 0) | (c->split_edge ? 2 : 0)))) return rc;
    }
    c->act_valid[i] = full != nullptr;
    if (ragged) {
      const size_t pix = (size_t)kConvs[i].co * ((c->prec == DType::SPLIT && i == 13) ? 6 : c->es);
      if (full && (rc = ragged_mask_act(full, pix, kConvs[i].level, heights, hts_dev, n, h, w, s))) return rc;
      if (fuse && (rc = ragged_mask_act(c->act_pool[pool_i], (size_t)kConvs[i].co * c->es, kConvs[i].level + 1, heights, hts_dev, n, h, w, s))) return rc;
    }
    cur = fuse ? c->act_pool[pool_i] : c->act_conv[i];
    if (fuse) ++pool_i;
  }
  if (stack_timed) {
    CTPN_HIP_TRY(hipEventRecord(stack_b, s));
    ProfRec r{CTPN_KIND_CONV_GEMM, stack_a, stack_b, stack_flops};
    r.launches = 13;
    c->pending.push_back(r);
  }
  const int hf = lvl(h, 4), wf = lvl(w, 4);
  const long long M5 = (long long)n * hf * wf;
  {
    IGemm g{};
    const bool sp = c->prec == DType::SPLIT;
    g.a = cur; g.wt = c->wt_x; g.bias = c->b_x; g.out = c->xp;
    g.M = M5; g.Ci = sp ? 1536 : 512; g.ntaps = 1; g.Co = 1024; g.a_plain = 0; g.H = hf; g.W = wf; g.tap_base_y = 1; g.tap_base_x = 1;
    g.out_bordered = 0; g.ldc = 1024; g.relu = 0;
    Timed t(c, CTPN_KIND_GEMM, 2.0 * (double)M5 * 512 * 1024);
    if (dtype_is_half(c->prec)) { if ((rc = launch_lstm_pre(cur, c->wt_xf, c->b_x, c->xp, c->prec, n, hf, wf, s))) return rc; }
    else if ((rc = launch_igemm(g, sp ? DType::BF16 : c->prec, DType::F32, s))) return rc;
  }
  if (tail_on_p) {
    CTPN_HIP_TRY(hipEventRecord(c->ev_conv, s));
    CTPN_HIP_TRY(hipStreamWaitEvent(ts, c->ev_conv, 0));
  }
  {
    Timed t(c, CTPN_KIND_BILSTM, (double)M5 * (1024.0 + 256.0) * 4.0, ts);
    const bool half = dtype_is_half(c->prec);
    if ((rc = launch_bilstm(c->xp, half ? 1 : 0, c->wh, c->lstm_out, n * hf, wf, ts, (c->lstm_split && c->prec != DType::F32) ? 1 : 0, half ? 1 : 0))) return rc;
  }
  const bool fold_heads = dtype_is_half(c->prec) && !c->keep_acts;
  if (fold_heads) {
    IGemm g{};
    g.a = c->lstm_out; g.wt = c->wt_fold; g.bias = c->b_fold; g.out = c->heads;
    g.M = M5; g.Ci = 256; g.ntaps = 1; g.Co = 60; g.a_plain = 1; g.lda = 256; g.out_bordered = 0; g.ldc = 64; g.relu = 0;
    if ((rc = wait_decoded())) return rc;
    Timed t(c, CTPN_KIND_GEMM, 2.0 * (double)M5 * 256 * 60, ts);
    if ((rc = launch_igemm(g, DType::F32, DType::F32, ts))) return rc;
  } else {
  {
    IGemm g{};
    g.a = c->lstm_out; g.wt = c->wt_fc; g.bias = c->b_fc; g.out = c->fc_out;
    g.M = M5; g.Ci = 256; g.ntaps = 1; g.Co = 512; g.a_plain = 1; g.lda = 256; g.out_bordered = 0; g.ldc = 512; g.relu = 0;
    Timed t(c, CTPN_KIND_GEMM, 2.0 * (double)M5 * 256 * 512, ts);
    if ((rc = launch_igemm(g, DType::F32, DType::F32, ts))) return rc;
  }
  {
    IGemm g{};
    g.a = c->fc_out; g.wt = c->wt_h; g.bias = c->b_h; g.out = c->heads;
    g.M = M5; g.Ci = 512; g.ntaps = 1; g.Co = 60; g.a_plain = 1; g.lda = 512; g.out_bordered = 0; g.ldc = 64; g.relu = 0;
    if ((rc = wait_decoded())) return rc;
    Timed t(c, CTPN_KIND_GEMM, 2.0 * (double)M5 * 512 * 60, ts);
    if ((rc = launch_igemm(g, DType::F32, DType::F32, ts))) return rc;
  }
  }
  if (tail_on_p) { CTPN_HIP_TRY(hipEventRecord(c->ev_tail, ts)); c->tail_pending = true; }
  c->fc_valid = !fold_heads;
  c->forward_done = true;
  c->proposals_done = false;
  return CTPN_OK;
}

}

extern "C" {

int ctpn_forward(ctpn_ctx* c, const uint8_t* images, int images_on_device, int n, int h, int w) {
  return forward_impl(c, images, 0, images_on_device, n, h, w);
}
int ctpn_forward_blob(ctpn_ctx* c, const float* blob, int blob_on_device, int n, int h, int w) {
  return forward_impl(c, blob, 1, blob_on_device, n, h, w);
}

int ctpn_forward_ragged(ctpn_ctx* c, const uint8_t* canvas, int canvas_on_device, int n, int hc, int w, const int* heights) {
  if (!c || !canvas || !heights) return fail(CTPN_ERR_ARG, "ctpn_forward_ragged: null pointer");
  return forward_impl(c, canvas, 0, canvas_on_device, n, hc, w, false, heights, 2);
}

int ctpn_feat_shape(ctpn_ctx* c, int* n, int* hf, int* wf) {
  if (!c) return fail(CTPN_ERR_ARG, "null ctx");
  if (!c->forward_done) return fail(CTPN_ERR_STATE, "no forward yet");
  if (n) *n = c->n; if (hf) *hf = lvl(c->h, 4); if (wf) *wf = lvl(c->w, 4);
  return CTPN_OK;
}

int ctpn_get_tensor(ctpn_ctx* c, const char* name, float* out_host, size_t capacity, int shape4[4]) {
  if (!c || !name || !out_host) return fail(CTPN_ERR_ARG, "null pointer");
  if (!c->forward_done) return fail(CTPN_ERR_STATE, "ctpn_get_tensor: no forward yet");
  CTPN_HIP_TRY(hipSetDevice(c->device));
  const std::string nm(name);
  const int n = c->n, hf = lvl(c->h, 4), wf = lvl(c->w, 4);
  const void* src = nullptr; int H = 0, W = 0, C = 0, ld = 0; bool bordered = false; DType t = DType::F32;
  for (int i = 0; i < 14; ++i) if (nm == kConvs[i].name && !c->act_valid[i])
    return fail(CTPN_ERR_STATE, "ctpn_get_tensor: " + nm + (i == 0 ? " is computed inside conv1_2's window stage" : " is fused with its max-pool") + " and not stored; set the ctx option keep_acts = 1 (ctpn_set_option)");
  for (int i = 0; i < 14; ++i) if (nm == kConvs[i].name) { src = c->act_conv[i]; H = lvl(c->h, kConvs[i].level); W = lvl(c->w, kConvs[i].level); C = kConvs[i].co; ld = C; bordered = true; t = c->prec; }
  const int pool_src[4] = {1, 3, 6, 9};
  for (int p = 0; p < 4; ++p) if (nm == kPoolNames[p]) { src = c->act_pool[p]; H = lvl(c->h, p + 1); W = lvl(c->w, p + 1); C = kConvs[pool_src[p]].co; ld = C; bordered = true; t = c->prec; }
  if (nm == "lstm_pre") { src = c->xp; H = hf; W = wf; C = 1024; ld = 1024; if (dtype_is_half(c->prec)) t = DType::F16; }
  if (nm == "lstm_out") { src = c->lstm_out; H = hf; W = wf; C = 256; ld = 256; }
  if (nm == "lstm_o" && !c->fc_valid)
    return fail(CTPN_ERR_STATE, "ctpn_get_tensor: lstm_o is folded into the heads GEMM in the 16-bit modes; set the ctx option keep_acts = 1 (ctpn_set_option)");
  if (nm == "lstm_o") { src = c->fc_out; H = hf; W = wf; C = 512; ld = 512; }
  if (nm == "heads") { src = c->heads; H = hf; W = wf; C = 60; ld = 64; }
  if (nm == "rpn_cls_prob_reshape") { src = c->cls_prob; H = hf; W = wf; C = 20; ld = 20; }
  if (nm == "rpn_bbox_pred") { src = c->bbox_pred; H = hf; W = wf; C = 40; ld = 40; }
  if (!src) return fail(CTPN_ERR_ARG, "ctpn_get_tensor: unknown tensor name " + nm);
  if ((src == c->cls_prob || src == c->bbox_pred) && !c->proposals_done)
    return fail(CTPN_ERR_STATE, "ctpn_get_tensor: " + nm + " is produced by ctpn_proposals (the softmax is fused into the decode kernel)");
  const size_t need = (size_t)n * H * W * C;
  if (shape4) { shape4[0] = n; shape4[1] = H; shape4[2] = W; shape4[3] = C; }
  if (capacity < need) return fail(CTPN_ERR_CAPACITY, "ctpn_get_tensor: output buffer too small");
  CTPN_HIP_TRY(hipStreamSynchronize(c->stream));
  CTPN_HIP_TRY(hipStreamSynchronize(c->stream_p));
  const bool split = t == DType::SPLIT;
  if (split) ld = (src == c->act_conv[13] ? 3 : 2) * C;
  const int es = split ? 2 : dtype_bytes(t);
  const int Hs = bordered ? H + 2 : H, Ws = bordered ? W + 2 : W;
  const size_t bytes = (size_t)n * Hs * Ws * ld * es;
  std::vector<char> tmp(bytes);
  CTPN_HIP_TRY(hipMemcpy(tmp.data(), src, bytes, hipMemcpyDeviceToHost));
  const int o = bordered ? 1 : 0;
  for (int in = 0; in < n; ++in)
    for (int y = 0; y < H; ++y)
      for (int x = 0; x < W; ++x) {
        const size_t sp = (((size_t)in * Hs + y + o) * Ws + x + o) * ld;
        float* d = out_host + (((size_t)in * H + y) * W + x) * C;
        if (src == c->xp) {
          if (es == 2) {
            const uint16_t* sh = (const uint16_t*)tmp.data() + sp;
            for (int ch = 0; ch < 1024; ++ch) d[ch] = host_f16_to_f32(sh[(ch & ~511) + lstm_gate_col(ch & 511)]);
          } else {
            const float* sf = (const float*)tmp.data() + sp;
            for (int ch = 0; ch < 1024; ++ch) d[ch] = sf[(ch & ~511) + lstm_gate_col(ch & 511)];
          }
        } else if (es == 4) {
          std::memcpy(d, (const float*)tmp.data() + sp, (size_t)C * 4);
        } else {
          const uint16_t* sb = (const uint16_t*)tmp.data() + sp;
          if (split) for (int ch = 0; ch < C; ++ch) d[ch] = host_bf16_to_f32(sb[ch]) + host_bf16_to_f32(sb[C + ch]);
          else if (t == DType::F16) for (int ch = 0; ch < C; ++ch) d[ch] = host_f16_to_f32(sb[ch]);
          else for (int ch = 0; ch < C; ++ch) d[ch] = host_bf16_to_f32(sb[ch]);
        }
      }
  return CTPN_OK;
}

}
```

text-detection-ctpn_amd/csrc/api_proposals.hip:

```cpp
#include "ctx.h"

namespace ctpn {

int nms_check_generic(ctpn_ctx* c, const float* boxes, const float* scores, const int* counts, int stride, float thresh, int post_topn,
                      const int* keep1, int keep_stride, const int* cnt1, int n, bool mw, hipStream_t s, const char* what) {
  std::vector<int> k2((size_t)n * keep_stride), c2(n);
  int* keep2 = nullptr; int* cnt2 = nullptr; float* spill2 = nullptr;
  struct Free3 { int*& a; int*& b; float*& c; ~Free3() { if (a) (void)hipFree(a); if (b) (void)hipFree(b); if (c) (void)hipFree(c); } } guard{keep2, cnt2, spill2};
  CTPN_HIP_TRY(hipMalloc((void**)&keep2, k2.size() * sizeof(int)));
  CTPN_HIP_TRY(hipMalloc((void**)&cnt2, c2.size() * sizeof(int)));
  CTPN_HIP_TRY(hipMalloc((void**)&spill2, (size_t)n * keep_stride * 4 * sizeof(float)));
  int rc = launch_nms(boxes, scores, counts, stride, thresh, post_topn, keep2, keep_stride, cnt2, nullptr, spill2, n, s);
  if (rc) return rc;
  CTPN_HIP_TRY(hipStreamSynchronize(s));
  CTPN_HIP_TRY(hipMemcpy(k2.data(), keep2, k2.size() * sizeof(int), hipMemcpyDeviceToHost));
  CTPN_HIP_TRY(hipMemcpy(c2.data(), cnt2, c2.size() * sizeof(int), hipMemcpyDeviceToHost));
  if (mw) {
    for (int i = 0; i < n; ++i) {
      unsigned ov = 0;
      CTPN_HIP_TRY(hipMemcpy(&ov, c->nms_mw_scratch + (size_t)i * NMS_MW_SCRATCH_BYTES + NMS_MW_OVERFLOW_OFF, 4, hipMemcpyDeviceToHost));
      if (ov) return fail(CTPN_ERR_STATE, "nms_check: a column held more candidates than the multi-workgroup NMS's list (1024): keep lists are incomplete");
    }
  }
  for (int i = 0; i < n; ++i) {
    bool same = cnt1[i] == c2[i];
    for (int k = 0; same && k < c2[i]; ++k) same = keep1[(size_t)i * keep_stride + k] == k2[(size_t)i * keep_stride + k];
    if (!same) return fail(CTPN_ERR_STATE, std::string("nms_check: column-decomposed ") + what + " differs from the generic kernel (boxes off the 16-px anchor grid?)");
  }
  return CTPN_OK;
}

static int enqueue_proposals_impl(ctpn_ctx* c, const float* heads, int heads_are_probs, int n, int hf, int wf, const float* im_info,
                                  int pre_nms_topn, int post_nms_topn, float nms_thresh, float min_size, hipStream_t s, hipEvent_t ev_decoded,
                                  const int* valid_rows_dev) {
  if (!s) s = c->stream;
  if (!im_info) return fail(CTPN_ERR_ARG, "proposals: null pointer");
  if (pre_nms_topn <= 0 || pre_nms_topn > c->topn_max) return fail(CTPN_ERR_CAPACITY, "proposals: pre_nms_topn must be in 1..12000");
  if (post_nms_topn <= 0 || post_nms_topn > c->post_max) return fail(CTPN_ERR_CAPACITY, "proposals: post_nms_topn must be in 1..1000");
  const int per_img = hf * wf * 10;
  const int npad = next_pow2(per_img);
  if (npad > c->npad_max) return fail(CTPN_ERR_CAPACITY, "proposals: feature map larger than the ctx was created for");
  if (n > 4) CTPN_HIP_TRY(hipMemcpyAsync(c->im_info_dev, im_info, (size_t)n * 3 * sizeof(float), hipMemcpyHostToDevice, s));
  ProposalCfg pc{n, hf, wf, pre_nms_topn, post_nms_topn, nms_thresh, min_size};
  int rc;
  bool mw = nms_multi_wg(c, n, hf) && nms_columns_ok(wf, pre_nms_topn, nms_thresh);
  if (c->nms_mw_scratch && c->nms_mw_dirty) {
    CTPN_HIP_TRY(hipMemsetAsync(c->nms_mw_scratch, 0, (size_t)NMS_MW_CAP_BATCH * NMS_MW_SCRATCH_BYTES, s));
    c->nms_mw_dirty = false;
  }
  const bool seg_sort = !(c->nms_columns == 2 || c->nms_columns == 0);
  const double nanch = (double)n * per_img;
  {
    Timed t(c, CTPN_KIND_DECODE, nanch * (60.0 * 4 / 10 + 8 + 16), s);
    if ((rc = launch_decode(heads, 64, heads_are_probs, c->cls_in, c->bbox_in, c->im_info_dev, heads_are_probs ? nullptr : c->cls_prob,
                            heads_are_probs ? nullptr : c->bbox_pred, c->keys, c->boxes4, pc, npad, s, seg_sort && sort_is_segmented(n, per_img), n <= 4 ? im_info : nullptr, valid_rows_dev))) return rc;
  }
  if (ev_decoded) CTPN_HIP_TRY(hipEventRecord(ev_decoded, s));
  {
    Timed t(c, CTPN_KIND_SORT, (double)n * npad * 16.0, s);
    int in_tmp = 0;
    if ((rc = launch_sort_keys(c->keys, c->keys_tmp, n, npad, per_img, s, seg_sort ? &in_tmp : nullptr))) return rc;
    const unsigned long long* sorted_keys = in_tmp ? c->keys_tmp : c->keys;
    for (int i = 0; i < n; ++i) mw = mw && im_info[3 * i + 1] >= (float)((wf - 1) * 16 + 1);
    if ((rc = launch_gather_sorted(sorted_keys, c->boxes4, c->sorted_boxes, c->sorted_scores, c->sorted_anchor, c->valid_counts, n, npad, per_img, pre_nms_topn, s,
                                   mw ? c->nms_colid : nullptr, wf))) return rc;
  }
  if (c->debug_hog > 0 && c->nms_mw_scratch) {
    const int hv = c->debug_hog;
    const int usec = hv > 100000 ? hv - 100000 : hv > 50000 ? hv - 50000 : hv, touch = hv > 100000 ? 4 : hv > 50000 ? 2 : 0;
    const void* src = nullptr; size_t src_bytes = 0;
    for (int i = 0; i < 14; ++i) if (c->act_conv[i] && c->act_conv_bytes[i] > src_bytes) { src = c->act_conv[i]; src_bytes = c->act_conv_bytes[i]; }
    if ((rc = launch_hog((unsigned*)(c->nms_colid), touch == 4 ? 2 * n : n, usec, touch, s, src, src_bytes))) return rc;
  }
  {
    Timed t(c, CTPN_KIND_NMS, (double)n * pre_nms_topn * 24.0, s);
    if (c->nms_columns && nms_columns_ok(wf, pre_nms_topn, nms_thresh)) {
      if ((rc = launch_nms_columns(c->sorted_boxes, c->sorted_scores, c->valid_counts, pre_nms_topn, nms_thresh, post_nms_topn, c->keep_idx,
                                   c->topn_max, c->keep_counts, c->rois, c->kept_spill, n, wf, s, c->sorted_anchor, c->roi_anchor, nullptr,
                                   mw ? c->nms_mw_scratch : nullptr, mw ? c->nms_colid : nullptr, c->nms_prefix ? 4096 : 0, c->debug_nms))) return rc;
      if (c->nms_check) {
        std::vector<int> k1((size_t)n * c->topn_max), c1(n);
        CTPN_HIP_TRY(hipStreamSynchronize(s));
        CTPN_HIP_TRY(hipMemcpy(k1.data(), c->keep_idx, k1.size() * sizeof(int), hipMemcpyDeviceToHost));
        CTPN_HIP_TRY(hipMemcpy(c1.data(), c->keep_counts, c1.size() * sizeof(int), hipMemcpyDeviceToHost));
        if ((rc = nms_check_generic(c, c->sorted_boxes, c->sorted_scores, c->valid_counts, pre_nms_topn, nms_thresh, post_nms_topn, k1.data(), c->topn_max,
                                    c1.data(), n, mw, s, "NMS"))) return rc;
      }
    } else if ((rc = launch_nms(c->sorted_boxes, c->sorted_scores, c->valid_counts, pre_nms_topn, nms_thresh, post_nms_topn, c->keep_idx,
                                c->topn_max, c->keep_counts, c->rois, c->kept_spill, n, s, c->sorted_anchor, c->roi_anchor))) return rc;
  }
  c->last_post = post_nms_topn; c->last_prop_n = n;
  if (!heads_are_probs) c->proposals_done = true;
  return CTPN_OK;
}
int enqueue_proposals(ctpn_ctx* c, const float* heads, int heads_are_probs, int n, int hf, int wf, const float* im_info,
                      int pre_nms_topn, int post_nms_topn, float nms_thresh, float min_size, hipStream_t s,
                      hipEvent_t ev_decoded, const int* valid_rows_dev) {
  const int rc = enqueue_proposals_impl(c, heads, heads_are_probs, n, hf, wf, im_info, pre_nms_topn, post_nms_topn, nms_thresh, min_size, s, ev_decoded, valid_rows_dev);
  if (rc != CTPN_OK) c->nms_mw_dirty = true;
  return rc;
}

static int run_proposals(ctpn_ctx* c, const float* heads, int heads_are_probs, int n, int hf, int wf, const float* im_info,
                         int pre_nms_topn, int post_nms_topn, float nms_thresh, float min_size, float* rois_out, int* counts_out,
                         const int* valid_rows_dev = nullptr) {
  if (!rois_out || !counts_out) return fail(CTPN_ERR_ARG, "proposals: null pointer");
  CTPN_HIP_TRY(hipStreamSynchronize(c->stream_p));
  int rc = enqueue_proposals(c, heads, heads_are_probs, n, hf, wf, im_info, pre_nms_topn, post_nms_topn, nms_thresh, min_size, nullptr, nullptr, valid_rows_dev);
  if (rc) return rc;
  hipStream_t s = c->stream;
  CTPN_HIP_TRY(hipMemcpyAsync(counts_out, c->keep_counts, (size_t)n * sizeof(int), hipMemcpyDeviceToHost, s));
  CTPN_HIP_TRY(hipMemcpyAsync(rois_out, c->rois, (size_t)n * post_nms_topn * 5 * sizeof(float), hipMemcpyDeviceToHost, s));
  CTPN_HIP_TRY(hipStreamSynchronize(s));
  return CTPN_OK;
}

}

namespace {
struct NmsCache {
  std::mutex mu;
  hipStream_t stream = nullptr;
  int cap = 0;
  float* boxes = nullptr; float* spill = nullptr; int* keep = nullptr; int* counts = nullptr;
};
NmsCache g_nms[16];
}

extern "C" {

int ctpn_proposals(ctpn_ctx* c, const float* im_info, int pre_nms_topn, int post_nms_topn, float nms_thresh, float min_size,
                   float* rois_out, int* counts_out) {
  if (!c) return fail(CTPN_ERR_ARG, "null ctx");
  if (!c->forward_done) return fail(CTPN_ERR_STATE, "ctpn_proposals: no forward yet");
  CTPN_HIP_TRY(hipSetDevice(c->device));
  const int* valid = c->fwd_ragged >= 0 ? c->ragged[c->fwd_ragged].dev + c->n : nullptr;
  return run_proposals(c, c->heads, 0, c->n, lvl(c->h, 4), lvl(c->w, 4), im_info, pre_nms_topn, post_nms_topn, nms_thresh, min_size,
                       rois_out, counts_out, valid);
}

int ctpn_proposals_from_host(ctpn_ctx* c, const float* cls_prob, const float* bbox_pred, int n, int hf, int wf, const float* im_info,
                             int pre_nms_topn, int post_nms_topn, float nms_thresh, float min_size, float* rois_out, int* counts_out) {
  if (!c || !cls_prob || !bbox_pred) return fail(CTPN_ERR_ARG, "null pointer");
  if (n <= 0 || n > c->max_batch || hf <= 0 || wf <= 0 || (size_t)n * hf * wf > c->m5_max)
    return fail(CTPN_ERR_CAPACITY, "ctpn_proposals_from_host: shape outside what the ctx was created for");
  CTPN_HIP_TRY(hipSetDevice(c->device));
  const size_t m = (size_t)n * hf * wf;
  CTPN_HIP_TRY(hipMemcpyAsync(c->cls_in, cls_prob, m * 20 * sizeof(float), hipMemcpyHostToDevice, c->stream));
  CTPN_HIP_TRY(hipMemcpyAsync(c->bbox_in, bbox_pred, m * 40 * sizeof(float), hipMemcpyHostToDevice, c->stream));
  return run_proposals(c, nullptr, 1, n, hf, wf, im_info, pre_nms_topn, post_nms_topn, nms_thresh, min_size, rois_out, counts_out);
}

int ctpn_proposal_anchors(ctpn_ctx* c, int* anchors_out, int post_nms_topn) {
  if (!c || !anchors_out) return fail(CTPN_ERR_ARG, "null pointer");
  if (c->last_prop_n <= 0) return fail(CTPN_ERR_STATE, "ctpn_proposal_anchors: no ctpn_proposals / ctpn_proposals_from_host call yet");
  if (post_nms_topn != c->last_post) return fail(CTPN_ERR_ARG, "ctpn_proposal_anchors: post_nms_topn differs from the proposals call");
  CTPN_HIP_TRY(hipSetDevice(c->device));
  CTPN_HIP_TRY(hipStreamSynchronize(c->stream_p));
  CTPN_HIP_TRY(hipMemcpyAsync(anchors_out, c->roi_anchor, (size_t)c->last_prop_n * post_nms_topn * sizeof(int), hipMemcpyDeviceToHost, c->stream));
  CTPN_HIP_TRY(hipStreamSynchronize(c->stream));
  return CTPN_OK;
}

int ctpn_nms(int* keep_out, int* num_out, const float* boxes_host, int boxes_num, int boxes_dim, float thresh, int device_id) {
  if (!keep_out || !num_out) return fail(CTPN_ERR_ARG, "ctpn_nms: null output");
  *num_out = 0;
  if (boxes_num == 0) return CTPN_OK;
  if (!boxes_host || boxes_num < 0 || boxes_dim < 4) return fail(CTPN_ERR_ARG, "ctpn_nms: boxes must be N x (>=4)");
  const int ndev = ctpn_device_count();
  if (ndev <= 0) return fail(CTPN_ERR_NODEVICE, "ctpn_nms: no HIP device visible (this library has no CPU fallback)");
  if (device_id < 0 || device_id >= ndev || device_id >= 16) return fail(CTPN_ERR_ARG, "ctpn_nms: device_id out of range");
  NmsCache& nc = g_nms[device_id];
  std::lock_guard<std::mutex> lk(nc.mu);
  CTPN_HIP_TRY(hipSetDevice(device_id));
  if (!nc.stream) CTPN_HIP_TRY(hipStreamCreateWithFlags(&nc.stream, hipStreamNonBlocking));
  if (nc.cap < boxes_num) {
    if (nc.boxes) { (void)hipFree(nc.boxes); (void)hipFree(nc.spill); (void)hipFree(nc.keep); (void)hipFree(nc.counts); nc.boxes = nullptr; nc.cap = 0; }
    const int cap = boxes_num < 16384 ? 16384 : boxes_num;
    CTPN_HIP_TRY(hipMalloc((void**)&nc.boxes, (size_t)cap * 4 * sizeof(float)));
    CTPN_HIP_TRY(hipMalloc((void**)&nc.spill, (size_t)cap * 4 * sizeof(float)));
    CTPN_HIP_TRY(hipMalloc((void**)&nc.keep, (size_t)cap * sizeof(int)));
    CTPN_HIP_TRY(hipMalloc((void**)&nc.counts, 2 * sizeof(int)));
    nc.cap = cap;
  }
  std::vector<float> b4((size_t)boxes_num * 4);
  for (int i = 0; i < boxes_num; ++i) std::memcpy(&b4[(size_t)i * 4], boxes_host + (size_t)i * boxes_dim, 4 * sizeof(float));
  CTPN_HIP_TRY(hipMemcpyAsync(nc.boxes, b4.data(), b4.size() * sizeof(float), hipMemcpyHostToDevice, nc.stream));
  CTPN_HIP_TRY(hipMemcpyAsync(nc.counts, &boxes_num, sizeof(int), hipMemcpyHostToDevice, nc.stream));
  int rc = launch_nms(nc.boxes, nullptr, nc.counts, boxes_num, thresh, boxes_num, nc.keep, boxes_num, nc.counts + 1, nullptr, nc.spill, 1, nc.stream);
  if (rc) return rc;
// ... 11 lines not shown
```

text-detection-ctpn_amd/csrc/conv3x3.hip:

```cpp
#include "conv3x3_base.h"

namespace ctpn {

int c3_wr_resources(int dev, hipStream_t s, char** dump_out, unsigned** claim_out) {
  static char* dump[CTPN_MAX_DEV] = {nullptr};
  static unsigned* claims[CTPN_MAX_DEV] = {nullptr};
  static unsigned ticket[CTPN_MAX_DEV] = {0};
  static std::mutex mu;
  std::lock_guard<std::mutex> lk(mu);
  if (!dump[dev]) CTPN_HIP_TRY(hipMalloc((void**)&dump[dev], (size_t)1024 * 4096));
  if (!claims[dev]) {
    CTPN_HIP_TRY(hipMalloc((void**)&claims[dev], 64 * 64 * sizeof(unsigned)));
    CTPN_HIP_TRY(hipMemsetAsync(claims[dev], 0, 64 * 64 * sizeof(unsigned), s));
    CTPN_HIP_TRY(hipStreamSynchronize(s));
  }
  *dump_out = dump[dev];
  *claim_out = claims[dev] + (size_t)(ticket[dev]++ % 64) * 64;
  return CTPN_OK;
}

__global__ __launch_bounds__(256) void c3_lds_dma_check_kernel(const char* __restrict__ src, char* __restrict__ out_clobber,
                                                              char* __restrict__ out_keep, int tiles) {
  extern __shared__ __attribute__((aligned(16))) char smem[];
  const int wave = __builtin_amdgcn_readfirstlane(threadIdx.x >> 6), lane = threadIdx.x & 63;
// ... 9 lines not shown
    __builtin_amdgcn_sched_barrier(0);
    const uint4 va = *(const uint4*)(a + lane * 16), vb = *(const uint4*)(b + lane * 16);
    *(uint4*)(out_clobber + (size_t)t * 1024 + lane * 16) = va;
    *(uint4*)(out_keep + (size_t)t * 1024 + lane * 16) = vb;
    __builtin_amdgcn_s_waitcnt(0);
  }
}

int launch_lds_dma_check(const void* src, void* out_clobber, void* out_keep, int tiles, hipStream_t s) {
  if (tiles <= 0) return fail(CTPN_ERR_ARG, "lds_dma_check: no tiles");
  const int grid = tiles < 1024 ? (tiles + 3) / 4 : 256;
  hipLaunchKernelGGL(c3_lds_dma_check_kernel, dim3(grid), dim3(256), 4 * 2048, s, (const char*)src, (char*)out_clobber, (char*)out_keep, tiles);
  CTPN_HIP_TRY(hipGetLastError());
  return CTPN_OK;
}

bool conv1_fusable(DType t, int n, int h, int w, int ci, int co, bool pool, bool keep_full) {
  return dtype_is_half(t) && ci == 64 && co == 64 && pool && !keep_full && n >= 1;
}

int launch_conv3x3(const void* in, const void* wt, const float* bias, void* out, void* pool_out, DType t, int n, int h, int w,
                   int ci, int co, int relu, hipStream_t s, int dup_hi, const void* q1, const void* q1_frags, int split_opts) {
  const int bke = (t == DType::F32) ? 32 : 64;
  if (ci <= 0 || ci % bke != 0) return fail(CTPN_ERR_ARG, "conv3x3: Ci must be a multiple of the 128-byte strip");
  const int epc = (t == DType::F32) ? 4 : 8;
  if (co % epc != 0) return fail(CTPN_ERR_ARG, "conv3x3: Co must be a multiple of a 16-byte chunk");
  if (!out && !pool_out) return fail(CTPN_ERR_ARG, "conv3x3: no output");
  if (dup_hi && t != DType::SPLIT) return fail(CTPN_ERR_ARG, "conv3x3: dup_hi is a split-precision layout");
  Conv3 g{};
  g.in = in; g.wt = wt; g.bias = bias; g.out = out; g.pool_out = pool_out;
  g.N = n; g.H = h; g.W = w; g.Ci = ci; g.Co = co; g.relu = relu;
  g.in_pitch = ci; g.out_pitch = co; g.a_wrap = 0; g.dup_hi = 0;
  if (t == DType::SPLIT) {
    if (!bias) return fail(CTPN_ERR_ARG, "conv3x3 (split precision): bias required");
    g.Ci = 3 * ci; g.in_pitch = 2 * ci; g.a_wrap = 2 * ci / 64; g.out_pitch = (dup_hi ? 3 : 2) * co; g.dup_hi = dup_hi ? 1 : 0;
  }
  const bool pool = pool_out != nullptr;
  const bool split = t == DType::SPLIT;
  int dev = 0, ncu = 0, rc;
  if ((rc = current_device(dev)) || (rc = device_cu_count(dev, ncu))) return rc;
  const C3Plan plan = c3_plan(t, n, h, w, ci, co, pool, out != nullptr, dup_hi, relu != 0, bias != nullptr, split_opts, ncu);
  if (plan.main_form == C3M_NONE) return fail(CTPN_ERR_ARG, "conv3x3 (split precision): Co must be <= 64 or a multiple of 128, with ReLU");
  const bool strip = plan.strip != C3S_NONE, edge = plan.strip == C3S_EDGE, edge_pool = plan.strip == C3S_EDGE_POOL;
  const int r = plan.strip_cols;
  g.w_cover = plan.w_cover;
  if (q1) {
    if (!conv1_fusable(t, n, h, w, ci, co, pool, out != nullptr) || !q1_frags || strip) return fail(CTPN_ERR_ARG, "conv3x3: the fused conv1_1 form is conv1_2's pooled 16-bit launch");
    g.q1 = q1; g.q1_frags = q1_frags;
  }
  static hipStream_t sstream[16] = {nullptr};
  static hipEvent_t ev_fork[16] = {nullptr}, ev_join[16] = {nullptr};
  static std::mutex strip_mu[16];
  std::unique_lock<std::mutex> strip_lock;
  const bool instream = strip && plan.deep != 0;
  auto run_edge = [&](void* dst, bool pooled) -> int {
    hipStream_t es = instream ? s : sstream[dev];
    if (split) return c3_edge_split(in, wt, bias, dst, n, h, w, ci, co, relu, r, pooled, es, true, dup_hi, plan.edge_ks);
    return t == DType::F16 ? c3_edge_f16(in, wt, bias, dst, n, h, w, ci, co, relu, r, pooled, es, instream)
                           : c3_edge_bf16(in, wt, bias, dst, n, h, w, ci, co, relu, r, pooled, es, instream);
  };
  if (strip && !instream) {
    strip_lock = std::unique_lock<std::mutex>(strip_mu[dev]);
    if (!sstream[dev]) {
      CTPN_HIP_TRY(hipStreamCreateWithFlags(&sstream[dev], hipStreamNonBlocking));
      CTPN_HIP_TRY(hipEventCreateWithFlags(&ev_fork[dev], hipEventDisableTiming));
      CTPN_HIP_TRY(hipEventCreateWithFlags(&ev_join[dev], hipEventDisableTiming));
    }
    CTPN_HIP_TRY(hipEventRecord(ev_fork[dev], s));
    CTPN_HIP_TRY(hipStreamWaitEvent(sstream[dev], ev_fork[dev], 0));
    if (edge_pool) {
      if ((rc = run_edge(pool_out, true))) return rc;
      if (out && (rc = run_edge(out, false))) return rc;
    } else if (edge) {
      if ((rc = run_edge(out, false))) return rc;
    } else {
      IGemm ig{};
      ig.a = in; ig.wt = wt; ig.bias = bias; ig.out = out;
      ig.M = (long long)n * h * r; ig.Ci = ci; ig.ntaps = 9; ig.Co = co;
      ig.a_plain = 0; ig.H = h; ig.W = w; ig.rx0 = w - r; ig.rw = r; ig.out_bordered = 1; ig.ldc = co; ig.relu = relu;
      if ((rc = launch_igemm(ig, t, t, sstream[dev]))) return rc;
    }
    CTPN_HIP_TRY(hipEventRecord(ev_join[dev], sstream[dev]));
  }
  switch (t) {
    case DType::F32: rc = c3_run_f32(g, pool, plan.main_form, s); break;
    case DType::BF16: rc = c3_run_bf16(g, pool, plan.main_form, s); break;
    case DType::F16: rc = c3_run_f16(g, pool, plan.main_form, s); break;
    default: rc = c3_run_split(g, pool, plan.main_form, s); break;
  }
  if (rc) return rc;
  if (instream) {
    if (edge_pool) {
      if ((rc = run_edge(pool_out, true))) return rc;
      if (out && (rc = run_edge(out, false))) return rc;
    } else if ((rc = run_edge(out, false))) return rc;
  } else if (strip) CTPN_HIP_TRY(hipStreamWaitEvent(s, ev_join[dev], 0));
  return CTPN_OK;
}

}
```

text-detection-ctpn_amd/csrc/ctx.h:

```cpp
#pragma once
#include <atomic>
#include <condition_variable>
#include <cstdio>
#include <cstdlib>
#include <cstring>
#include <functional>
#include <memory>
#include <mutex>
#include <thread>

#include <pthread.h>
#include <sched.h>

#include <dlfcn.h>

#include "common.h"

namespace ctpn {

struct ConvSpec { const char* name; int ci, co, level; int pool_after; };
static const ConvSpec kConvs[14] = {
    {"conv1_1", 3, 64, 0, 0},    {"conv1_2", 64, 64, 0, 1},   {"conv2_1", 64, 128, 1, 0},  {"conv2_2", 128, 128, 1, 1},
    {"conv3_1", 128, 256, 2, 0}, {"conv3_2", 256, 256, 2, 0}, {"conv3_3", 256, 256, 2, 1}, {"conv4_1", 256, 512, 3, 0},
    {"conv4_2", 512, 512, 3, 0}, {"conv4_3", 512, 512, 3, 1}, {"conv5_1", 512, 512, 4, 0}, {"conv5_2", 512, 512, 4, 0},
    {"conv5_3", 512, 512, 4, 0}, {"rpn_conv/3x3", 512, 512, 4, 0}};
static const char* kPoolNames[4] = {"pool1", "pool2", "pool3", "pool4"};

struct ProfRec { int kind; hipEvent_t a, b; double work; int launches = 1; };

class HostPool {
 public:
  HostPool(int nthreads, int first_cpu) : n_(nthreads < 1 ? 1 : nthreads) {
    for (int t = 1; t < n_; ++t) {
      th_.emplace_back([this] { loop(); });
      if (first_cpu >= 0) pin(th_.back().native_handle(), first_cpu + t);
    }
  }
  ~HostPool() {
    { std::lock_guard<std::mutex> lk(mu_); stop_ = true; ++gen_; }
    cv_.notify_all();
    for (auto& t : th_) t.join();
  }
  int size() const { return n_; }
  void run(int n, const std::function<void(int)>& fn, int max_par = 0) {
    if (n <= 0) return;
    const int par = std::min(n, max_par > 0 ? std::min(max_par, n_) : n_);
    if (par <= 1) { for (int i = 0; i < n; ++i) fn(i); return; }
    std::lock_guard<std::mutex> serial(run_mu_);
    {
      std::lock_guard<std::mutex> lk(mu_);
      fn_ = &fn; total_ = n; next_.store(0); done_.store(0); helpers_ = par - 1; ++gen_;
    }
    cv_.notify_all();
    work();
    std::unique_lock<std::mutex> lk(mu_);
    done_cv_.wait(lk, [&] { return done_.load() >= total_ && active_ == 0; });
    helpers_ = 0;
    fn_ = nullptr;
  }

 private:
  static void pin(pthread_t h, int cpu) {
    cpu_set_t set; CPU_ZERO(&set);
    const unsigned ncpu = std::thread::hardware_concurrency();
    CPU_SET((int)(ncpu > 0 ? (unsigned)cpu % ncpu : (unsigned)cpu), &set);
    (void)pthread_setaffinity_np(h, sizeof(set), &set);
  }
  void work() {
    for (;;) {
      const int i = next_.fetch_add(1);
      if (i >= total_) break;
      (*fn_)(i);
      done_.fetch_add(1);
    }
  }
  void loop() {
    unsigned long long seen = 0;
    for (;;) {
      {
        std::unique_lock<std::mutex> lk(mu_);
        cv_.wait(lk, [&] { return gen_ != seen; });
        seen = gen_;
        if (stop_) return;
        if (helpers_ <= 0) continue;
        --helpers_; ++active_;
      }
      work();
      { std::lock_guard<std::mutex> lk(mu_); --active_; }
      done_cv_.notify_all();
    }
  }
  const int n_;
  std::vector<std::thread> th_;
  std::mutex mu_, run_mu_;
  std::condition_variable cv_, done_cv_;
  const std::function<void(int)>* fn_ = nullptr;
  int total_ = 0, helpers_ = 0, active_ = 0;
  std::atomic<int> next_{0}, done_{0};
  unsigned long long gen_ = 0;
  bool stop_ = false;
};

}

using namespace ctpn;

struct ctpn_ctx {
  int device = 0;
  int max_batch = 0, max_h = 0, max_w = 0;
  DType prec = DType::BF16;
  int es = 2;
  hipStream_t stream = nullptr;
  hipStream_t stream_p = nullptr;
  std::vector<void*> allocs;
  struct Slot {
    char* pack = nullptr;
    float* tlb = nullptr; float* tls = nullptr; int* keep = nullptr; int* kcnt = nullptr; float* rois = nullptr; int* rcnt = nullptr;
    float* im_info = nullptr;
    double* crecs = nullptr; int* ccnt = nullptr;
    hipEvent_t ev_heads = nullptr, ev_decoded = nullptr, ev_done = nullptr;
    int n = 0, h = 0, w = 0; bool busy = false;
    std::vector<int> hts;
  } slot[2];
  hipEvent_t ev_last_decoded = nullptr;
  hipEvent_t ev_last_done = nullptr;
  int tail_confine = 0;
  int tail_overlap = 0;
  hipEvent_t ev_conv = nullptr;
  hipEvent_t ev_tail = nullptr;
  bool tail_pending = false;

  bool weights_loaded = false;
  float* arena = nullptr;
  float* w_first = nullptr;
  void* w_first_frags = nullptr;
  int conv1_mfma = 2;
  struct JpegBufs {
    int16_t* coef_host = nullptr; uint16_t* qt_host = nullptr;
    int16_t* coef_dev = nullptr; uint16_t* qt_dev = nullptr; uint8_t* out_dev = nullptr;
    size_t coef_elems = 0, qt_imgs = 0, out_bytes = 0;
    uint8_t* tab_host = nullptr; uint8_t* tab_dev = nullptr; size_t tab_imgs = 0;
    int out_n = 0, out_h = 0, out_w = 0;
    hipEvent_t ev_h2d = nullptr, ev_ready = nullptr, ev_consumed = nullptr;
    bool h2d_valid = false, consumed_valid = false, ready_valid = false;
  } jpeg[2];
  uint8_t* jpeg_planes = nullptr;
  uint8_t* jpeg_raw = nullptr;
  size_t jpeg_planes_bytes = 0, jpeg_raw_bytes = 0;
  std::vector<void*> jpeg_retired;
  int jpeg_flip = 0;
  bool jpeg_ready = false;
  struct JhWork {
    uint8_t* stage_host = nullptr; uint8_t* stage_dev = nullptr; size_t stage_bytes = 0;
    uint8_t* work_dev = nullptr; size_t work_bytes = 0;
    uint32_t* res_host = nullptr; size_t res_words = 0;
  } jh;
  long long jh_stats[4] = {0, 0, 0, 0};
  struct StageBufs {
    uint8_t* img_dev = nullptr; size_t img_bytes = 0;
    uint8_t* rs_dev = nullptr; size_t rs_bytes = 0;
    double* recs_dev = nullptr; size_t recs_bytes = 0; int* cnt_dev = nullptr; size_t cnt_bytes = 0;
    uint8_t* rm_host = nullptr; size_t rm_host_bytes = 0; uint8_t* rm_dev = nullptr; size_t rm_bytes = 0;
  } stage;
  struct EncBufs {
    int16_t* coef_dev = nullptr; int16_t* coef_host = nullptr; size_t coef_elems = 0;
    void* qtab_dev = nullptr; void* qtab_host = nullptr; int qtab_quality = 0;
    hipEvent_t ev_done = nullptr;
    uint8_t* huff_dev = nullptr; size_t huff_bytes = 0;
    void* huff_tab_dev = nullptr;
    uint8_t* huff_host = nullptr; size_t huff_host_bytes = 0;
    uint8_t* scan_host = nullptr; size_t scan_host_bytes = 0;
    uint8_t* mix_host = nullptr; size_t mix_host_bytes = 0;
    uint8_t* mix_dev = nullptr; size_t mix_bytes = 0;
  } enc;
  long long jhe_stats[4] = {0, 0, 0, 0};
  struct PngEncBufs {
    uint8_t* dev = nullptr; size_t dev_bytes = 0;
    uint8_t* host = nullptr; size_t host_bytes = 0;
    uint8_t* file_host = nullptr; size_t file_host_bytes = 0;
    hipEvent_t ev_done = nullptr;
  } pnge;
  long long pnge_stats[4] = {0, 0, 0, 0};
  struct CropBufs {
    uint8_t* img_dev = nullptr; size_t img_bytes = 0;
    uint8_t* out_dev = nullptr; size_t out_bytes = 0;
    void* desc_dev = nullptr; size_t desc_bytes = 0;
    void* desc_host = nullptr; size_t desc_host_bytes = 0;
    hipEvent_t ev_done = nullptr;
  } crop;
  int debug_nms = 0;
  int debug_hog = 0;
  int nms_prefix = 1;
  int split_edge = 1;
  int conv_p64 = 1;
  int conv1_fuse = 1;
  void* q_img = nullptr;
  size_t q_img_bytes = 0;
  int lstm_split = 0;
  int nms_check = 0;
  float* b_conv[14] = {nullptr};
  void* wt_conv[14] = {nullptr};
  void* wt_x = nullptr;
  size_t wx_row_bytes = 1024;
  void* wt_xf = nullptr;
  float* b_x = nullptr;
  float* wh = nullptr;
  float* wt_fc = nullptr;
  float* b_fc = nullptr;
  float* wt_h = nullptr;
  float* b_h = nullptr;
  float* wt_fold = nullptr;
  float* b_fold = nullptr;

  void* act_conv[14] = {nullptr};
  void* act_pool[4] = {nullptr};
  bool act_valid[14] = {true, true, true, true, true, true, true, true, true, true, true, true, true, true};
  size_t act_conv_bytes[14] = {0};
  size_t act_pool_bytes[4] = {0};
  uint8_t* img_dev = nullptr;
  uint8_t* img_dev_b[2] = {nullptr, nullptr};
  hipStream_t stream_c = nullptr;
  hipEvent_t ev_copied[2] = {nullptr, nullptr}, ev_consumed[2] = {nullptr, nullptr};
  bool consumed_valid[2] = {false, false};
  void* pin_stage[2] = {nullptr, nullptr};
  size_t pin_stage_bytes[2] = {0, 0};
  hipEvent_t ev_h2d_done[2] = {nullptr, nullptr};
  bool h2d_valid[2] = {false, false};
  int img_flip = 0;
  float* xp = nullptr;
  float* lstm_out = nullptr;
  float* fc_out = nullptr;
  float* heads = nullptr;
  float* cls_prob = nullptr;
  float* bbox_pred = nullptr;
  size_t m5_max = 0;

  int npad_max = 0, topn_max = 12000, post_max = 1000;
  unsigned long long* keys = nullptr; unsigned long long* keys_tmp = nullptr;
  float* boxes4 = nullptr;
  float* sorted_boxes = nullptr;
  float* sorted_scores = nullptr;
  int* valid_counts = nullptr;
  int* keep_idx = nullptr;
  int* keep_counts = nullptr;
  float* rois = nullptr;
  float* kept_spill = nullptr;
  int* sorted_anchor = nullptr;
  int* roi_anchor = nullptr;
  int last_post = 0, last_prop_n = 0;
  float* im_info_dev = nullptr;
  char* out_pack = nullptr; size_t pack_bytes = 0;
  float* tl_boxes = nullptr; float* tl_scores = nullptr; int* tl_counts = nullptr;
  int* tl_keep = nullptr; int* tl_keep_counts = nullptr; float* tl_spill = nullptr;
  double* conn_recs = nullptr; int* conn_counts = nullptr; double* conn_scratch = nullptr;
  int nms_columns = 1;
  char* nms_mw_scratch = nullptr;
  bool nms_mw_dirty = false;
  unsigned char* nms_colid = nullptr;
  int connect_device = 0;
  double tail_raw[TAIL_PARAM_COUNT];
  int rpn_pre = 12000, rpn_post = 1000;
  float rpn_nms_thresh = 0.7f, rpn_min_size = 8.0f;
  ConnectorCfg conn = default_connector_cfg();
  bool proposals_done = false;
  bool postproc_only = false;
  std::unique_ptr<ctpn::HostPool> pool;
  int host_threads = 1;
  bool fc_valid = true;
  int keep_acts = 0;
  float* cls_in = nullptr;
  float* bbox_in = nullptr;

  struct RaggedSet {
    int* host = nullptr; int* dev = nullptr;
    hipEvent_t ev_copied = nullptr; bool copied_valid = false;
  } ragged[3];
  float* ragged_blob = nullptr; size_t ragged_blob_bytes = 0;
  int fwd_ragged = -1;

  int n = 0, h = 0, w = 0;
  int gn = -1, gh = -1, gw = -1;
  bool forward_done = false;

  bool prof = false;
  int prof_mode = 1;
  std::vector<ProfRec> pending;
  std::vector<hipEvent_t> free_events;
  double prof_ms[CTPN_KIND_COUNT] = {0};
  long long prof_n[CTPN_KIND_COUNT] = {0};
  double prof_work[CTPN_KIND_COUNT] = {0};
};

namespace ctpn {

static inline DType prec_dtype(int precision) {
  return precision == CTPN_PREC_FP32 ? DType::F32 : precision == CTPN_PREC_FP16 ? DType::F16 : precision == CTPN_PREC_SPLIT ? DType::SPLIT : DType::BF16;
}

static inline int lvl(int v, int level) { for (int i = 0; i < level; ++i) v /= 2; return v; }
static inline size_t act_slack_pixels(int w) { return (size_t)28 * (w + 2) + 384; }
static inline size_t act_front_pixels(int w) { return (size_t)(w + 2) + 64; }

static inline bool nms_multi_wg(const ctpn_ctx* c, int n, int hf) {
  return c->nms_mw_scratch && hf * 10 <= 1024 && ((c->nms_columns == 3 && n <= NMS_MW_CAP_BATCH) || (c->nms_columns == 1 && n <= NMS_MW_MAX_BATCH));
}

static inline int grow_dev(void** p, size_t& have, size_t need) {
  if (need <= have) return CTPN_OK;
  if (*p) CTPN_HIP_TRY(hipFree(*p));
  *p = nullptr; have = 0;
  CTPN_HIP_TRY(hipMalloc(p, need));
  have = need;
  return CTPN_OK;
}

static inline int grow_host(uint8_t** p, size_t& have, size_t need) {
  if (need <= have) return CTPN_OK;
  if (*p) CTPN_HIP_TRY(hipHostFree(*p));
  *p = nullptr; have = 0;
  CTPN_HIP_TRY(hipHostMalloc((void**)p, need));
  have = need;
  return CTPN_OK;
}

int debug_sync();
struct RoctxApi { int (*push)(const char*) = nullptr; int (*pop)() = nullptr; };
const RoctxApi& roctx_api();
int roctx_on();
static const char* kKindNames[CTPN_KIND_COUNT + 1] = {"ctpn:conv_first", "ctpn:conv_gemm", "ctpn:pool", "ctpn:gemm", "ctpn:bilstm",
                                                     "ctpn:decode", "ctpn:sort", "ctpn:nms", "ctpn:conv_stack"};
struct Timed {
  ctpn_ctx* c; int kind; double work; hipEvent_t a = nullptr, b = nullptr; bool on; hipStream_t st;
  Timed(ctpn_ctx* c_, int kind_, double work_, hipStream_t st_ = nullptr) : c(c_), kind(kind_), work(work_), on(c_->prof && (c_->prof_mode == 1 || kind_ == CTPN_KIND_COUNT)), st(st_ ? st_ : c_->stream) {
    if (debug_sync()) { fprintf(stderr, "[ctpn] launch kind %d work %.3g\n", kind, work); fflush(stderr); }
    if (roctx_on()) (void)roctx_api().push(kKindNames[kind]);
    if (!on) return;
    auto get = [&]() { hipEvent_t e; if (!c->free_events.empty()) { e = c->free_events.back(); c->free_events.pop_back(); } else { (void)hipEventCreate(&e); } return e; };
    a = get(); b = get();
    (void)hipEventRecord(a, st);
  }
  ~Timed() {
    if (roctx_on()) (void)roctx_api().pop();
    if (debug_sync()) { hipError_t e = hipStreamSynchronize(st); fprintf(stderr, "[ctpn]   done kind %d: %s\n", kind, hipGetErrorString(e)); fflush(stderr); }
    if (!on) return;
    (void)hipEventRecord(b, st);
    c->pending.push_back({kind, a, b, work});
  }
};

int forward_impl(ctpn_ctx* c, const void* images, int is_f32, int images_on_device, int n, int h, int w, bool tail_on_p = false,
                 const int* heights = nullptr, int rset = 2);
int enqueue_proposals(ctpn_ctx* c, const float* heads, int heads_are_probs, int n, int hf, int wf, const float* im_info,
                      int pre_nms_topn, int post_nms_topn, float nms_thresh, float min_size, hipStream_t s = nullptr,
                      hipEvent_t ev_decoded = nullptr, const int* valid_rows_dev = nullptr );
int nms_check_generic(ctpn_ctx* c, const float* boxes, const float* scores, const int* counts, int stride, float thresh, int post_topn,
                      const int* keep1, int keep_stride, const int* cnt1, int n, bool mw, hipStream_t s, const char* what);
int wait_live_batch(ctpn_ctx* c, const uint8_t* images_dev, hipStream_t qs);
int stage_pixels(ctpn_ctx* c, const uint8_t* images, int on_device, size_t bytes, size_t slack, uint8_t*& buf, size_t& buf_bytes, hipStream_t qs, const uint8_t*& px);
typedef int (*StageSizeCheck)(const std::string& who, int h, int w);
int annotate_batch(ctpn_ctx* c, const std::string& who, const char* format, StageSizeCheck size_check, const uint8_t* images, int on_device, int n, int h, int w, const double* recs,
                   int line_capacity, const int* line_counts, double scale, const char* const* paths, const uint8_t*& px, int& dh, int& dw);
void write_file(const char* path, const uint8_t* data, size_t bytes, int& st, std::string& msg);
int first_failure(const char* who, const std::vector<int>& st, const std::vector<std::string>& msg);
int encode_mixed_dev(ctpn_ctx* c, const char* who, const uint8_t* px_dev, int n, const int* heights, const int* widths, const size_t* pitches, const size_t* offsets,
                     int quality, uint8_t* const* out, const size_t* capacities, size_t* bytes_out, const char* const* paths, bool device_entropy);
bool jpeg_read_file(const char* path, std::vector<uint8_t>& buf, size_t limit = 0);
void jpeg_layout8(const JpegGeom& g, int* layout8);

}
```

Baseline: 3718.

## Run two forward passes concurrently using a second activation set and stream

Adds a second forward-buffer set (activations, LSTM and head buffers) with its own stream. When the other submit slot is still busy, the new batch runs its forward pass on that set so two batches' conv/LSTM work can overlap on the GPU. It also allows the conv strip/edge work to run in-stream, and reworks profiling to merge overlapping spans. The cost is extra device memory and more cross-stream synchronisation. The two forwards also compete for compute units, so overlap gains depend on how well each saturates the GPU.

Measured after the change: 3794, median of 6. 2.1% higher.

```diff
diff --git a/include/ctpn_hip.h b/include/ctpn_hip.h
--- a/include/ctpn_hip.h
+++ b/include/ctpn_hip.h
@@ -135,6 +135,7 @@
                             int conv_p64, int split_edge, int cu_count, int* plans);
 const char* ctpn_debug_conv3x3_form_name(int kind, int id);
 int ctpn_debug_lstm_pre_plan(long long cells, int cu_count, int* plan_out);
+int ctpn_debug_forward_sets(ctpn_ctx* ctx, long long* out4);
 int ctpn_debug_lstm_pre(int device_id, const float* x, const float* wx, const float* bias, int n, int hf, int wf, int precision, int cu_count,
                         float* out);
 int ctpn_debug_bilstm(int device_id, const float* pre, const float* wh, int rows, int T, int split, int fast_gates, int pre_f16, float* out,
diff --git a/text-detection-ctpn_amd/_binding.py b/text-detection-ctpn_amd/_binding.py
--- a/text-detection-ctpn_amd/_binding.py
+++ b/text-detection-ctpn_amd/_binding.py
@@ -106,6 +106,7 @@
         "ctpn_debug_conv3x3_plan": (C.c_int, [C.c_int] * 13 + [i32p]),
         "ctpn_debug_conv3x3_form_name": (C.c_char_p, [C.c_int, C.c_int]),
         "ctpn_debug_lstm_pre_plan": (C.c_int, [C.c_longlong, C.c_int, i32p]),
+        "ctpn_debug_forward_sets": (C.c_int, [vp, C.POINTER(C.c_longlong)]),
         "ctpn_debug_lstm_pre": (C.c_int, [C.c_int, f32p, f32p, f32p, C.c_int, C.c_int, C.c_int, C.c_int, C.c_int, f32p]),
         "ctpn_debug_bilstm": (C.c_int, [C.c_int, f32p, f32p, C.c_int, C.c_int, C.c_int, C.c_int, C.c_int, f32p, i32p]),
         "ctpn_debug_gemm": (C.c_int, [C.c_int, f32p, f32p, f32p, C.c_int, C.c_int, C.c_int, C.c_int, C.c_int, f32p]),
@@ -740,6 +741,12 @@
         _check(self._lib.ctpn_get_param(self._h, name.encode(), C.byref(v)))
         return v.value
 
+    def forward_sets(self):
+        out = (C.c_longlong * 4)()
+        _check(self._lib.ctpn_debug_forward_sets(self._h, out))
+        in_flight = tuple(None if v == 255 else v for v in (int(out[3]) & 255, (int(out[3]) >> 8) & 255))
+        return int(out[0]), int(out[1]), int(out[2]), in_flight
+
     def host_threads(self):
         n = C.c_int(0)
         _check(self._lib.ctpn_host_threads(self._h, C.byref(n)))
diff --git a/text-detection-ctpn_amd/csrc/api_ctx.hip b/text-detection-ctpn_amd/csrc/api_ctx.hip
--- a/text-detection-ctpn_amd/csrc/api_ctx.hip
+++ b/text-detection-ctpn_amd/csrc/api_ctx.hip
@@ -14,6 +14,15 @@
   c->allocs.push_back(*p);
   if (zero) CTPN_HIP_TRY(hipMemsetAsync(*p, 0, bytes, c->stream));
   return CTPN_OK;
+}
+
+int two_forwards_mode() {
+#ifdef CTPN_ABLATION
+  static const int v = env_int("CTPN_TWO_FORWARDS", 2);
+  return v < 0 || v > 3 ? 2 : v;
+#else
+  return 2;
+#endif
 }
 
 int debug_sync() { static const int v = env_int("CTPN_DEBUG_SYNC", 0); return v; }
@@ -41,15 +50,31 @@
 
 static int prof_drain(ctpn_ctx* c) {
   if (c->pending.empty()) return CTPN_OK;
-  CTPN_HIP_TRY(hipStreamSynchronize(c->stream));
+  CTPN_HIP_TRY(sync_forwards(c));
   CTPN_HIP_TRY(hipStreamSynchronize(c->stream_p));
+  struct Span { double t0, t1; float own; };
+  std::vector<Span> spans;
+  hipEvent_t origin = nullptr;
   for (auto& r : c->pending) {
     float ms = 0.f;
     if (hipEventElapsedTime(&ms, r.a, r.b) == hipSuccess) {
-      c->prof_ms[r.kind] += ms; c->prof_n[r.kind] += r.launches; c->prof_work[r.kind] += r.work;
-    }
-    c->free_events.push_back(r.a); c->free_events.push_back(r.b);
-  }
+      c->prof_n[r.kind] += r.launches; c->prof_work[r.kind] += r.work;
+      float off = 0.f;
+      if (!r.span) c->prof_ms[r.kind] += ms;
+      else if (!origin) { origin = r.a; spans.push_back({0.0, (double)ms, ms}); }
+      else if (hipEventElapsedTime(&off, origin, r.a) == hipSuccess) spans.push_back({(double)off, (double)off + (double)ms, ms});
+      else c->prof_ms[r.kind] += ms;
+    }
+  }
+  std::sort(spans.begin(), spans.end(), [](const Span& x, const Span& y) { return x.t0 < y.t0; });
+  double covered = 0.0;
+  for (size_t i = 0; i < spans.size(); ++i) {
+    const Span& sp = spans[i];
+    if (i == 0 || sp.t0 >= covered) c->prof_ms[CTPN_KIND_CONV_GEMM] += sp.own;
+    else if (sp.t1 > covered) c->prof_ms[CTPN_KIND_CONV_GEMM] += sp.t1 - covered;
+    if (i == 0 || sp.t1 > covered) covered = sp.t1;
+  }
+  for (auto& r : c->pending) { c->free_events.push_back(r.a); c->free_events.push_back(r.b); }
   c->pending.clear();
   return CTPN_OK;
 }
@@ -106,7 +131,10 @@
   auto A = [&](void** p, size_t bytes, bool zero) { if (rc == CTPN_OK) rc = dev_alloc(c, p, bytes, zero); };
   if (hipStreamCreateWithFlags(&c->stream, hipStreamNonBlocking) != hipSuccess) { delete c; return fail(CTPN_ERR_HIP, "hipStreamCreate failed"); }
   if (hipStreamCreateWithFlags(&c->stream_p, hipStreamNonBlocking) != hipSuccess) { (void)hipStreamDestroy(c->stream); delete c; return fail(CTPN_ERR_HIP, "hipStreamCreate failed"); }
-  if (hipEventCreateWithFlags(&c->ev_conv, hipEventDisableTiming) != hipSuccess || hipEventCreateWithFlags(&c->ev_tail, hipEventDisableTiming) != hipSuccess) {
+  ctpn_ctx::FwdSet& f0 = c->fs[0];
+  f0.stream = c->stream;
+  if (hipEventCreateWithFlags(&f0.ev_conv, hipEventDisableTiming) != hipSuccess || hipEventCreateWithFlags(&f0.ev_tail, hipEventDisableTiming) != hipSuccess ||
+      hipEventCreateWithFlags(&f0.ev_gate, hipEventDisableTiming) != hipSuccess) {
     ctpn_destroy(c); return fail(CTPN_ERR_HIP, "ctpn_create: events");
   }
   for (auto& sl : c->slot) {
@@ -153,8 +181,8 @@
     const size_t pix_b = (size_t)kConvs[i].co * ((c->prec == DType::SPLIT && i == 13) ? 6 : c->es);
     c->act_conv_bytes[i] = ((size_t)max_batch * (hl + 2) * (wl + 2) + act_slack_pixels(wl)) * pix_b;
     const size_t front = act_front_pixels(wl) * pix_b;
-    A(&c->act_conv[i], front + c->act_conv_bytes[i], true);
-    if (c->act_conv[i]) c->act_conv[i] = (char*)c->act_conv[i] + front;
+    A(&f0.act_conv[i], front + c->act_conv_bytes[i], true);
+    if (f0.act_conv[i]) f0.act_conv[i] = (char*)f0.act_conv[i] + front;
   }
   {
     const int pool_src[4] = {1, 3, 6, 9};
@@ -162,11 +190,11 @@
       const int hl = lvl(max_h, p + 1), wl = lvl(max_w, p + 1);
       c->act_pool_bytes[p] = ((size_t)max_batch * (hl + 2) * (wl + 2) + act_slack_pixels(wl)) * kConvs[pool_src[p]].co * c->es;
       const size_t front = act_front_pixels(wl) * kConvs[pool_src[p]].co * c->es;
-      A(&c->act_pool[p], front + c->act_pool_bytes[p], true);
-      if (c->act_pool[p]) c->act_pool[p] = (char*)c->act_pool[p] + front;
-    }
-  }
-  if (dtype_is_half(c->prec)) { c->q_img_bytes = conv1_q_bytes(max_batch, max_h, max_w); A(&c->q_img, c->q_img_bytes, true); }
+      A(&f0.act_pool[p], front + c->act_pool_bytes[p], true);
+      if (f0.act_pool[p]) f0.act_pool[p] = (char*)f0.act_pool[p] + front;
+    }
+  }
+  if (dtype_is_half(c->prec)) { c->q_img_bytes = conv1_q_bytes(max_batch, max_h, max_w); A(&f0.q_img, c->q_img_bytes, true); }
   A((void**)&c->img_dev, (size_t)max_batch * max_h * max_w * 3 * sizeof(float), false);
   c->img_dev_b[0] = c->img_dev;
   A((void**)&c->img_dev_b[1], (size_t)max_batch * max_h * max_w * 3 * sizeof(float), false);
@@ -176,10 +204,10 @@
       ok = hipEventCreateWithFlags(&c->ev_copied[b], hipEventDisableTiming) == hipSuccess && hipEventCreateWithFlags(&c->ev_consumed[b], hipEventDisableTiming) == hipSuccess;
     if (!ok) rc = fail(CTPN_ERR_HIP, "ctpn_create: copy stream / events");
   }
-  A((void**)&c->xp, c->m5_max * 1024 * sizeof(float), false);
-  A((void**)&c->lstm_out, c->m5_max * 256 * sizeof(float), false);
-  A((void**)&c->fc_out, c->m5_max * 512 * sizeof(float), false);
-  A((void**)&c->heads, c->m5_max * 64 * sizeof(float), true);
+  A((void**)&f0.xp, c->m5_max * 1024 * sizeof(float), false);
+  A((void**)&f0.lstm_out, c->m5_max * 256 * sizeof(float), false);
+  A((void**)&f0.fc_out, c->m5_max * 512 * sizeof(float), false);
+  A((void**)&f0.heads, c->m5_max * 64 * sizeof(float), true);
   }
   A((void**)&c->cls_prob, c->m5_max * 20 * sizeof(float), false);
   A((void**)&c->bbox_pred, c->m5_max * 40 * sizeof(float), false);
@@ -217,6 +245,55 @@
   if (rc != CTPN_OK) { ctpn_destroy(c); return rc; }
   *out = c;
   return CTPN_OK;
+}
+
+static size_t conv_front_bytes(const ctpn_ctx* c, int i) {
+  return act_front_pixels(lvl(c->max_w, kConvs[i].level)) * (size_t)kConvs[i].co * ((c->prec == DType::SPLIT && i == 13) ? 6 : c->es);
+}
+static size_t pool_front_bytes(const ctpn_ctx* c, int p) {
+  const int pool_src[4] = {1, 3, 6, 9};
+  return act_front_pixels(lvl(c->max_w, p + 1)) * (size_t)kConvs[pool_src[p]].co * c->es;
+}
+
+static bool set1_block(ctpn_ctx* c, ctpn_ctx::FwdSet& f, void** p, size_t front, size_t bytes) {
+  void* raw = nullptr;
+  if (hipMalloc(&raw, front + bytes) != hipSuccess) { (void)hipGetLastError(); return false; }
+  f.allocs.push_back(raw);
+  if (hipMemsetAsync(raw, 0, front + bytes, f.stream) != hipSuccess) { (void)hipGetLastError(); return false; }
+  *p = (char*)raw + front;
+  c->set1_bytes += front + bytes;
+  return true;
+}
+
+bool ensure_set1(ctpn_ctx* c, bool need_conv1) {
+  if (two_forwards_mode() == 0 || c->postproc_only || c->keep_acts || (c->prof && c->prof_mode == 1) || c->set1_state < 0) return false;
+  ctpn_ctx::FwdSet& f = c->fs[1];
+  if (c->set1_state == 0) {
+    bool ok = hipStreamCreateWithFlags(&f.stream, hipStreamNonBlocking) == hipSuccess &&
+              hipEventCreateWithFlags(&f.ev_conv, hipEventDisableTiming) == hipSuccess && hipEventCreateWithFlags(&f.ev_tail, hipEventDisableTiming) == hipSuccess &&
+              hipEventCreateWithFlags(&f.ev_gate, hipEventDisableTiming) == hipSuccess;
+    for (int i = 1; i < 14 && ok; ++i)
+      if (!kConvs[i].pool_after) ok = set1_block(c, f, &f.act_conv[i], conv_front_bytes(c, i), c->act_conv_bytes[i]);
+    for (int p = 0; p < 4 && ok; ++p) ok = set1_block(c, f, &f.act_pool[p], pool_front_bytes(c, p), c->act_pool_bytes[p]);
+    if (ok && dtype_is_half(c->prec)) ok = set1_block(c, f, &f.q_img, 0, c->q_img_bytes);
+    ok = ok && set1_block(c, f, (void**)&f.xp, 0, c->m5_max * 1024 * sizeof(float)) && set1_block(c, f, (void**)&f.lstm_out, 0, c->m5_max * 256 * sizeof(float)) &&
+         set1_block(c, f, (void**)&f.heads, 0, c->m5_max * 64 * sizeof(float));
+    if (ok && !dtype_is_half(c->prec)) ok = set1_block(c, f, (void**)&f.fc_out, 0, c->m5_max * 512 * sizeof(float));
+    if (!ok) {
+      (void)hipGetLastError();
+      if (f.stream) (void)hipStreamSynchronize(f.stream);
+      for (void* p : f.allocs) (void)hipFree(p);
+      for (hipEvent_t e : {f.ev_conv, f.ev_tail, f.ev_gate}) if (e) (void)hipEventDestroy(e);
+      if (f.stream) (void)hipStreamDestroy(f.stream);
+      f = ctpn_ctx::FwdSet();
+      c->set1_bytes = 0;
+      c->set1_state = -1;
+      return false;
+    }
+    c->set1_state = 1;
+  }
+  if (need_conv1 && !f.act_conv[0] && !set1_block(c, f, &f.act_conv[0], conv_front_bytes(c, 0), c->act_conv_bytes[0])) return false;
+  return true;
 }
 
 struct Option { const char* name; int ctpn_ctx::* member; int lo, hi; };
@@ -279,10 +356,10 @@
   if (value < o->lo || value > o->hi) return fail(CTPN_ERR_ARG, std::string("ctpn_set_option: value out of range for ") + key);
   if (c->*(o->member) == value) return CTPN_OK;
   CTPN_HIP_TRY(hipSetDevice(c->device));
-  CTPN_HIP_TRY(hipStreamSynchronize(c->stream));
+  CTPN_HIP_TRY(sync_forwards(c));
   CTPN_HIP_TRY(hipStreamSynchronize(c->stream_p));
   for (auto& sl : c->slot) if (sl.busy) return fail(CTPN_ERR_STATE, "ctpn_set_option: a submitted batch has not been collected");
-  c->tail_pending = false;
+  for (auto& f : c->fs) f.tail_pending = false;
   c->nms_mw_dirty = true;
   c->*(o->member) = value;
   return CTPN_OK;
@@ -302,10 +379,10 @@
   if (!tail_param_ok(idx, value)) return fail(CTPN_ERR_ARG, std::string("ctpn_set_param: value out of range for ") + name);
   if (c->tail_raw[idx] == value) return CTPN_OK;
   CTPN_HIP_TRY(hipSetDevice(c->device));
-  CTPN_HIP_TRY(hipStreamSynchronize(c->stream));
+  CTPN_HIP_TRY(sync_forwards(c));
   CTPN_HIP_TRY(hipStreamSynchronize(c->stream_p));
   for (auto& sl : c->slot) if (sl.busy) return fail(CTPN_ERR_STATE, "ctpn_set_param: a submitted batch has not been collected");
-  c->tail_pending = false;
+  for (auto& f : c->fs) f.tail_pending = false;
   c->nms_mw_dirty = true;
   c->tail_raw[idx] = value;
   switch (idx) {
@@ -335,6 +412,7 @@
   if (!c) return CTPN_OK;
   (void)hipSetDevice(c->device);
   if (c->stream) (void)hipStreamSynchronize(c->stream);
+  if (c->fs[1].stream) (void)hipStreamSynchronize(c->fs[1].stream);
   if (c->stream_p) (void)hipStreamSynchronize(c->stream_p);
   if (c->stream_c) { (void)hipStreamSynchronize(c->stream_c); (void)hipStreamDestroy(c->stream_c); }
   for (int b = 0; b < 2; ++b) { if (c->pin_stage[b]) (void)hipHostFree(c->pin_stage[b]); if (c->ev_h2d_done[b]) (void)hipEventDestroy(c->ev_h2d_done[b]); }
@@ -343,9 +421,13 @@
     for (void* p : {(void*)sl.pack, (void*)sl.im_info, (void*)sl.crecs, (void*)sl.ccnt}) if (p) (void)hipHostFree(p);
     for (hipEvent_t e : {sl.ev_heads, sl.ev_decoded, sl.ev_done}) if (e) (void)hipEventDestroy(e);
   }
-  for (hipEvent_t e : {c->ev_conv, c->ev_tail}) if (e) (void)hipEventDestroy(e);
+  for (auto& f : c->fs) {
+    for (hipEvent_t e : {f.ev_conv, f.ev_tail, f.ev_gate}) if (e) (void)hipEventDestroy(e);
+    if (f.ragged_blob) (void)hipFree(f.ragged_blob);
+    for (void* p : f.allocs) (void)hipFree(p);
+  }
+  if (c->fs[1].stream) (void)hipStreamDestroy(c->fs[1].stream);
   for (auto& r : c->ragged) { if (r.host) (void)hipHostFree(r.host); if (r.dev) (void)hipFree(r.dev); if (r.ev_copied) (void)hipEventDestroy(r.ev_copied); }
-  if (c->ragged_blob) (void)hipFree(c->ragged_blob);
   for (auto& j : c->jpeg) {
     if (j.coef_host) (void)hipHostFree(j.coef_host);
     if (j.qt_host) (void)hipHostFree(j.qt_host);
@@ -379,7 +461,7 @@
 
 int ctpn_sync(ctpn_ctx* c) {
   if (!c) return fail(CTPN_ERR_ARG, "null ctx");
-  CTPN_HIP_TRY(hipStreamSynchronize(c->stream));
+  CTPN_HIP_TRY(sync_forwards(c));
   CTPN_HIP_TRY(hipStreamSynchronize(c->stream_p));
   if (c->stream_c) CTPN_HIP_TRY(hipStreamSynchronize(c->stream_c));
   return CTPN_OK;
diff --git a/text-detection-ctpn_amd/csrc/api_debug.hip b/text-detection-ctpn_amd/csrc/api_debug.hip
--- a/text-detection-ctpn_amd/csrc/api_debug.hip
+++ b/text-detection-ctpn_amd/csrc/api_debug.hip
@@ -190,6 +190,15 @@
 }
 extern "C" {
 
+int ctpn_debug_forward_sets(ctpn_ctx* c, long long* out4) {
+  if (!c || !out4) return fail(CTPN_ERR_ARG, "ctpn_debug_forward_sets: null pointer");
+  out4[0] = c->set1_state == 1 ? 2 : 1;
+  out4[1] = c->last == &c->fs[1] ? 1 : 0;
+  out4[2] = (long long)c->set1_bytes;
+  out4[3] = (c->slot[0].busy ? c->slot[0].set : 255) | (c->slot[1].busy ? c->slot[1].set : 255) << 8;
+  return CTPN_OK;
+}
+
 int ctpn_debug_lstm_pre_plan(long long cells, int cu_count, int* plan_out) {
   if (!plan_out) return fail(CTPN_ERR_ARG, "ctpn_debug_lstm_pre_plan: no output");
   if (cells <= 0 || cells > 0x7fffffffLL) return fail(CTPN_ERR_ARG, "ctpn_debug_lstm_pre_plan: cells out of range (1 .. 2^31 - 1)");
diff --git a/text-detection-ctpn_amd/csrc/api_detect.hip b/text-detection-ctpn_amd/csrc/api_detect.hip
--- a/text-detection-ctpn_amd/csrc/api_detect.hip
+++ b/text-detection-ctpn_amd/csrc/api_detect.hip
@@ -31,36 +31,49 @@
   return CTPN_OK;
 }
 
+static ctpn_ctx::FwdSet& pick_set(ctpn_ctx* c, int slot, int n, int h, int w, const int* heights, bool& beside) {
+  const ctpn_ctx::Slot& other = c->slot[slot ^ 1];
+  beside = false;
+  if (!other.busy) return c->fs[0];
+  if (other.set == 1) { beside = true; return c->fs[0]; }
+  if (!ensure_set1(c, !forward_fuses_conv1(c, 0, n, h, w, heights))) return c->fs[0];
+  beside = true;
+  return c->fs[1];
+}
+
 static int detect_submit_body(ctpn_ctx* c, const uint8_t* images, int images_on_device, int n, int h, int w, const float* scales, int slot, bool lone,
                               const int* heights) {
   if (!c) return fail(CTPN_ERR_ARG, "ctpn_detect_submit: null ctx");
   if (slot < 0 || slot > 1) return fail(CTPN_ERR_ARG, "ctpn_detect_submit: slot must be 0 or 1");
   ctpn_ctx::Slot& sl = c->slot[slot];
   if (sl.busy) return fail(CTPN_ERR_STATE, "ctpn_detect_submit: slot still holds an uncollected batch");
-  int rc = forward_impl(c, images, 0, images_on_device, n, h, w, c->tail_overlap != 0, heights, slot);
+  bool beside = false;
+  ctpn_ctx::FwdSet& f = pick_set(c, slot, n, h, w, heights, beside);
+  int rc = forward_impl(c, f, images, 0, images_on_device, n, h, w, c->tail_overlap != 0, heights, slot, beside);
   if (rc) {
     const std::string first = ctpn_last_error();
-    (void)hipStreamSynchronize(c->stream); (void)hipStreamSynchronize(c->stream_p);
-    c->tail_pending = false; c->ev_last_decoded = nullptr; c->ev_last_done = nullptr;
+    (void)sync_forwards(c); (void)hipStreamSynchronize(c->stream_p);
+    for (auto& g : c->fs) { g.tail_pending = false; g.ev_decoded = nullptr; g.dec_slot = -1; }
+    c->ev_last_done = nullptr;
     return fail(rc, first);
   }
   sl.hts.assign(n, h);
   if (heights) sl.hts.assign(heights, heights + n);
   for (int i = 0; i < n; ++i) { sl.im_info[3 * i] = (float)sl.hts[i]; sl.im_info[3 * i + 1] = (float)w; sl.im_info[3 * i + 2] = scales ? scales[i] : 1.0f; }
-  hipStream_t p = lone ? c->stream : c->stream_p;
+  hipStream_t p = lone ? f.stream : c->stream_p;
   if (!lone) {
-    CTPN_HIP_TRY(hipEventRecord(sl.ev_heads, c->stream));
+    CTPN_HIP_TRY(hipEventRecord(sl.ev_heads, f.stream));
     CTPN_HIP_TRY(hipStreamWaitEvent(p, sl.ev_heads, 0));
   }
-  rc = enqueue_proposals(c, c->heads, 0, n, lvl(h, 4), lvl(w, 4), sl.im_info, c->rpn_pre, c->rpn_post, c->rpn_nms_thresh, c->rpn_min_size, p, sl.ev_decoded,
-                         c->fwd_ragged >= 0 ? c->ragged[c->fwd_ragged].dev + n : nullptr);
-  if (rc) return rc;
-  c->ev_last_decoded = sl.ev_decoded;
+  rc = enqueue_proposals(c, f.heads, 0, n, lvl(h, 4), lvl(w, 4), sl.im_info, c->rpn_pre, c->rpn_post, c->rpn_nms_thresh, c->rpn_min_size, p, sl.ev_decoded,
+                         f.fwd_ragged >= 0 ? c->ragged[f.fwd_ragged].dev + n : nullptr);
+  if (rc) return rc;
+  f.ev_decoded = sl.ev_decoded; f.dec_slot = slot;
   if ((rc = enqueue_text_lines(c, sl, n, w, p))) return rc;
   CTPN_HIP_TRY(hipMemcpyAsync(sl.pack, c->out_pack, c->pack_bytes, hipMemcpyDeviceToHost, p));
   CTPN_HIP_TRY(hipEventRecord(sl.ev_done, p));
   c->ev_last_done = sl.ev_done;
-  sl.n = n; sl.h = h; sl.w = w; sl.busy = true;
+  sl.n = n; sl.h = h; sl.w = w; sl.busy = true; sl.set = (int)(&f - c->fs);
   return CTPN_OK;
 }
 static int detect_submit_impl(ctpn_ctx* c, const uint8_t* images, int images_on_device, int n, int h, int w, const float* scales, int slot, bool lone,
@@ -118,7 +131,7 @@
     if (roi_counts[i] < 0 || roi_counts[i] > post) return fail(CTPN_ERR_ARG, "ctpn_debug_text_lines: 0 <= roi_counts[i] <= RPN_POST_NMS_TOP_N (1000) rows of [score,x1,y1,x2,y2]");
   if (c->slot[0].busy || c->slot[1].busy) return fail(CTPN_ERR_STATE, "ctpn_debug_text_lines: a submitted batch has not been collected");
   CTPN_HIP_TRY(hipSetDevice(c->device));
-  CTPN_HIP_TRY(hipStreamSynchronize(c->stream));
+  CTPN_HIP_TRY(sync_forwards(c));
   CTPN_HIP_TRY(hipStreamSynchronize(c->stream_p));
   ctpn_ctx::Slot& sl = c->slot[0];
   hipStream_t p = c->stream_p;
diff --git a/text-detection-ctpn_amd/csrc/api_forward.hip b/text-detection-ctpn_amd/csrc/api_forward.hip
--- a/text-detection-ctpn_amd/csrc/api_forward.hip
+++ b/text-detection-ctpn_amd/csrc/api_forward.hip
@@ -37,7 +37,15 @@
   return launch_ragged_mask(buf, m, heights_dev, n, pad, s);
 }
 
-int forward_impl(ctpn_ctx* c, const void* images, int is_f32, int images_on_device, int n, int h, int w, bool tail_on_p, const int* heights, int rset) {
+bool forward_fuses_conv1(const ctpn_ctx* c, int is_f32, int n, int h, int w, const int* heights) {
+  bool ragged = false;
+  for (int i = 0; heights && i < n; ++i) ragged = ragged || heights[i] != h;
+  const bool via_q = !is_f32 && dtype_is_half(c->prec) && c->conv1_mfma >= 2 && c->fs[0].q_img != nullptr;
+  return via_q && c->conv1_fuse && !c->keep_acts && !ragged && conv1_fusable(c->prec, n, h, w, 64, 64, true, false);
+}
+
+int forward_impl(ctpn_ctx* c, ctpn_ctx::FwdSet& f, const void* images, int is_f32, int images_on_device, int n, int h, int w, bool tail_on_p, const int* heights, int rset,
+                 bool beside) {
   if (!c || !images) return fail(CTPN_ERR_ARG, "null pointer");
   if (c->postproc_only) return fail(CTPN_ERR_STATE, "ctpn_forward: post-processing-only ctx (ctpn_create_postproc) has no network");
   if (!c->weights_loaded) return fail(CTPN_ERR_STATE, "ctpn_forward: weights not loaded");
@@ -52,22 +60,24 @@
     }
   }
   CTPN_HIP_TRY(hipSetDevice(c->device));
-  hipStream_t s = c->stream;
+  hipStream_t s = f.stream;
   int rc;
   hipStream_t ts = tail_on_p ? c->stream_p : s;
+  const ctpn_ctx::FwdSet* prev_set = c->last;
   if (!tail_on_p) {
-    if (c->tail_pending) { CTPN_HIP_TRY(hipStreamWaitEvent(s, c->ev_tail, 0)); c->tail_pending = false; }
-  }
+    if (f.tail_pending) { CTPN_HIP_TRY(hipStreamWaitEvent(s, f.ev_tail, 0)); f.tail_pending = false; }
+  }
+  const bool reader_live = f.ev_decoded && (prev_set == &f || (f.dec_slot >= 0 && c->slot[f.dec_slot].busy));
   auto wait_decoded = [&]() -> int {
-    if (!tail_on_p && c->ev_last_decoded) CTPN_HIP_TRY(hipStreamWaitEvent(ts, c->ev_last_decoded, 0));
+    if (!tail_on_p && reader_live) CTPN_HIP_TRY(hipStreamWaitEvent(ts, f.ev_decoded, 0));
     return CTPN_OK;
   };
-  if (c->gn != n || c->gh != h || c->gw != w) {
-    if (c->tail_pending) { CTPN_HIP_TRY(hipStreamWaitEvent(s, c->ev_tail, 0)); c->tail_pending = false; }
-    for (int i = 0; i < 14; ++i) CTPN_HIP_TRY(hipMemsetAsync(c->act_conv[i], 0, c->act_conv_bytes[i], s));
-    for (int p = 0; p < 4; ++p) CTPN_HIP_TRY(hipMemsetAsync(c->act_pool[p], 0, c->act_pool_bytes[p], s));
-    if (c->q_img) CTPN_HIP_TRY(hipMemsetAsync(c->q_img, 0, c->q_img_bytes, s));
-    c->gn = n; c->gh = h; c->gw = w;
+  if (f.gn != n || f.gh != h || f.gw != w) {
+    if (f.tail_pending) { CTPN_HIP_TRY(hipStreamWaitEvent(s, f.ev_tail, 0)); f.tail_pending = false; }
+    for (int i = 0; i < 14; ++i) if (f.act_conv[i]) CTPN_HIP_TRY(hipMemsetAsync(f.act_conv[i], 0, c->act_conv_bytes[i], s));
+    for (int p = 0; p < 4; ++p) CTPN_HIP_TRY(hipMemsetAsync(f.act_pool[p], 0, c->act_pool_bytes[p], s));
+    if (f.q_img) CTPN_HIP_TRY(hipMemsetAsync(f.q_img, 0, c->q_img_bytes, s));
+    f.gn = n; f.gh = h; f.gw = w;
   }
   const void* img = images;
   int staged = -1;
@@ -98,8 +108,9 @@
     CTPN_HIP_TRY(hipStreamWaitEvent(s, c->ev_copied[staged], 0));
     img = c->img_dev_b[staged];
   }
-  c->n = n; c->h = h; c->w = w;
-  c->fwd_ragged = ragged ? rset : -1;
+  f.n = n; f.h = h; f.w = w;
+  c->last = &f;
+  f.fwd_ragged = ragged ? rset : -1;
   const int* hts_dev = nullptr;
   if (ragged) {
     if ((rc = ragged_upload(c, c->ragged[rset], heights, n, s))) return rc;
@@ -114,35 +125,36 @@
       }
   bool via_q = false, fuse1 = false;
   {
-    Timed t(c, CTPN_KIND_CONV_FIRST, (double)n * h * w * (3.0 + 64.0 * c->es));
+    Timed t(c, CTPN_KIND_CONV_FIRST, (double)n * h * w * (3.0 + 64.0 * c->es), s);
     const bool frags = c->prec == DType::SPLIT || (c->conv1_mfma && dtype_is_half(c->prec));
-    via_q = !is_f32 && dtype_is_half(c->prec) && c->conv1_mfma >= 2 && c->q_img != nullptr;
-    fuse1 = via_q && c->conv1_fuse && !c->keep_acts && !ragged && conv1_fusable(c->prec, n, h, w, 64, 64, true, false);
+    via_q = !is_f32 && dtype_is_half(c->prec) && c->conv1_mfma >= 2 && f.q_img != nullptr;
+    fuse1 = forward_fuses_conv1(c, is_f32, n, h, w, ragged ? heights : nullptr);
+    if (!fuse1 && !f.act_conv[0]) return fail(CTPN_ERR_STATE, "ctpn_forward: the forward set has no buffer for conv1_1's map");
     if (via_q) {
-      if ((rc = launch_image_to_q((const uint8_t*)img, c->q_img, c->prec, n, h, w, s))) return rc;
+      if ((rc = launch_image_to_q((const uint8_t*)img, f.q_img, c->prec, n, h, w, s))) return rc;
       if (ragged) {
         RaggedMap m;
         m.row_bytes = (long long)conv1_q_w(w) * 8; m.img_bytes = (long long)conv1_q_h(h) * m.row_bytes;
         m.top = 2; m.left_bytes = 16; m.span_bytes = w * 8; m.rows = h; m.level = 0;
         int pad = 0;
         for (int i = 0; i < n; ++i) pad = std::max(pad, h - heights[i]);
-        if ((rc = launch_ragged_mask(c->q_img, m, hts_dev, n, pad, s))) return rc;
-      }
-      if (!fuse1 && (rc = launch_conv_first_from_q(c->q_img, conv1_p_frags(c->w_first_frags, c->prec), c->act_conv[0], c->prec, n, h, w, 0, w, s))) return rc;
+        if ((rc = launch_ragged_mask(f.q_img, m, hts_dev, n, pad, s))) return rc;
+      }
+      if (!fuse1 && (rc = launch_conv_first_from_q(f.q_img, conv1_p_frags(c->w_first_frags, c->prec), f.act_conv[0], c->prec, n, h, w, 0, w, s))) return rc;
     } else if (ragged) {
       const size_t need = (size_t)n * h * w * 3 * sizeof(float);
-      if (need > c->ragged_blob_bytes) {
+      if (need > f.ragged_blob_bytes) {
         CTPN_HIP_TRY(hipStreamSynchronize(s));
-        if ((rc = grow_dev((void**)&c->ragged_blob, c->ragged_blob_bytes, need))) return rc;
-      }
-      if ((rc = launch_ragged_blob((const uint8_t*)img, c->ragged_blob, hts_dev, n, h, w, s))) return rc;
-      if ((rc = launch_conv_first(c->ragged_blob, 1, c->w_first, c->b_conv[0], c->act_conv[0], c->prec, n, h, w, s,
+        if ((rc = grow_dev((void**)&f.ragged_blob, f.ragged_blob_bytes, need))) return rc;
+      }
+      if ((rc = launch_ragged_blob((const uint8_t*)img, f.ragged_blob, hts_dev, n, h, w, s))) return rc;
+      if ((rc = launch_conv_first(f.ragged_blob, 1, c->w_first, c->b_conv[0], f.act_conv[0], c->prec, n, h, w, s,
                                   frags ? c->w_first_frags : nullptr))) return rc;
-    } else if ((rc = launch_conv_first(img, is_f32, c->w_first, c->b_conv[0], c->act_conv[0], c->prec, n, h, w, s,
+    } else if ((rc = launch_conv_first(img, is_f32, c->w_first, c->b_conv[0], f.act_conv[0], c->prec, n, h, w, s,
                                        frags ? c->w_first_frags : nullptr))) return rc;
-    if (ragged && (rc = ragged_mask_act(c->act_conv[0], (size_t)64 * c->es, 0, heights, hts_dev, n, h, w, s))) return rc;
-  }
-  c->act_valid[0] = !fuse1;
+    if (ragged && (rc = ragged_mask_act(f.act_conv[0], (size_t)64 * c->es, 0, heights, hts_dev, n, h, w, s))) return rc;
+  }
+  f.act_valid[0] = !fuse1;
   if (jpeg_src >= 0) {
     CTPN_HIP_TRY(hipEventRecord(c->jpeg[jpeg_src].ev_consumed, s));
     c->jpeg[jpeg_src].consumed_valid = true;
@@ -151,9 +163,16 @@
     CTPN_HIP_TRY(hipEventRecord(c->ev_consumed[staged], s));
     c->consumed_valid[staged] = true;
   }
-  if (c->tail_pending) { CTPN_HIP_TRY(hipStreamWaitEvent(s, c->ev_tail, 0)); c->tail_pending = false; }
+  if (f.tail_pending) { CTPN_HIP_TRY(hipStreamWaitEvent(s, f.ev_tail, 0)); f.tail_pending = false; }
   if (c->tail_confine && c->ev_last_done) CTPN_HIP_TRY(hipStreamWaitEvent(s, c->ev_last_done, 0));
-  const void* cur = c->act_conv[0];
+  const int gate = beside ? two_forwards_mode() - 1 : 0;
+  if (gate > 0) {
+    ctpn_ctx::FwdSet& o = c->fs[&f == &c->fs[0] ? 1 : 0];
+    if (o.gate_valid) CTPN_HIP_TRY(hipStreamWaitEvent(s, o.ev_gate, 0));
+  }
+  f.gate_valid = false;
+  const bool own_strips = beside && gate == 0;
+  const void* cur = f.act_conv[0];
   int pool_i = 0;
   hipEvent_t stack_a = nullptr, stack_b = nullptr;
   double stack_flops = 0.0;
@@ -169,54 +188,56 @@
     if (fuse1 && i == 1) flops += 2.0 * (double)n * h * w * 27.0 * 64.0;
     stack_flops += flops;
     const bool fuse = kConvs[i].pool_after != 0;
-    void* full = (!fuse || c->keep_acts) ? c->act_conv[i] : nullptr;
+    void* full = (!fuse || c->keep_acts) ? f.act_conv[i] : nullptr;
     {
-      Timed t(c, CTPN_KIND_CONV_GEMM, flops);
+      Timed t(c, CTPN_KIND_CONV_GEMM, flops, s);
       const bool f1 = fuse1 && i == 1;
-      if ((rc = launch_conv3x3(cur, c->wt_conv[i], c->b_conv[i], full, fuse ? c->act_pool[pool_i] : nullptr, c->prec, n, hl, wl,
+      if ((rc = launch_conv3x3(cur, c->wt_conv[i], c->b_conv[i], full, fuse ? f.act_pool[pool_i] : nullptr, c->prec, n, hl, wl,
                                kConvs[i].ci, kConvs[i].co, 1, s, (c->prec == DType::SPLIT && i == 13) ? 1 : 0,
-                               f1 ? c->q_img : nullptr, f1 ? conv1_p_frags(c->w_first_frags, c->prec) : nullptr, (c->conv_p64 ? 1 : 0) | (c->split_edge ? 2 : 0)))) return rc;
+                               f1 ? f.q_img : nullptr, f1 ? conv1_p_frags(c->w_first_frags, c->prec) : nullptr, (c->conv_p64 ? 1 : 0) | (c->split_edge ? 2 : 0) | (own_strips ? 4 : 0)))) return rc;
     }
-    c->act_valid[i] = full != nullptr;
+    f.act_valid[i] = full != nullptr;
     if (ragged) {
       const size_t pix = (size_t)kConvs[i].co * ((c->prec == DType::SPLIT && i == 13) ? 6 : c->es);
       if (full && (rc = ragged_mask_act(full, pix, kConvs[i].level, heights, hts_dev, n, h, w, s))) return rc;
-      if (fuse && (rc = ragged_mask_act(c->act_pool[pool_i], (size_t)kConvs[i].co * c->es, kConvs[i].level + 1, heights, hts_dev, n, h, w, s))) return rc;
+      if (fuse && (rc = ragged_mask_act(f.act_pool[pool_i], (size_t)kConvs[i].co * c->es, kConvs[i].level + 1, heights, hts_dev, n, h, w, s))) return rc;
     }
-    cur = fuse ? c->act_pool[pool_i] : c->act_conv[i];
+    cur = fuse ? f.act_pool[pool_i] : f.act_conv[i];
     if (fuse) ++pool_i;
   }
   if (stack_timed) {
     CTPN_HIP_TRY(hipEventRecord(stack_b, s));
     ProfRec r{CTPN_KIND_CONV_GEMM, stack_a, stack_b, stack_flops};
-    r.launches = 13;
+    r.launches = 13; r.span = true;
     c->pending.push_back(r);
   }
+  if (two_forwards_mode() == 2 && f.ev_gate) { CTPN_HIP_TRY(hipEventRecord(f.ev_gate, s)); f.gate_valid = true; }
   const int hf = lvl(h, 4), wf = lvl(w, 4);
   const long long M5 = (long long)n * hf * wf;
   {
     IGemm g{};
     const bool sp = c->prec == DType::SPLIT;
-    g.a = cur; g.wt = c->wt_x; g.bias = c->b_x; g.out = c->xp;
+    g.a = cur; g.wt = c->wt_x; g.bias = c->b_x; g.out = f.xp;
     g.M = M5; g.Ci = sp ? 1536 : 512; g.ntaps = 1; g.Co = 1024; g.a_plain = 0; g.H = hf; g.W = wf; g.tap_base_y = 1; g.tap_base_x = 1;
     g.out_bordered = 0; g.ldc = 1024; g.relu = 0;
-    Timed t(c, CTPN_KIND_GEMM, 2.0 * (double)M5 * 512 * 1024);
-    if (dtype_is_half(c->prec)) { if ((rc = launch_lstm_pre(cur, c->wt_xf, c->b_x, c->xp, c->prec, n, hf, wf, s))) return rc; }
+    Timed t(c, CTPN_KIND_GEMM, 2.0 * (double)M5 * 512 * 1024, s);
+    if (dtype_is_half(c->prec)) { if ((rc = launch_lstm_pre(cur, c->wt_xf, c->b_x, f.xp, c->prec, n, hf, wf, s))) return rc; }
     else if ((rc = launch_igemm(g, sp ? DType::BF16 : c->prec, DType::F32, s))) return rc;
   }
+  if (two_forwards_mode() == 3 && f.ev_gate) { CTPN_HIP_TRY(hipEventRecord(f.ev_gate, s)); f.gate_valid = true; }
   if (tail_on_p) {
-    CTPN_HIP_TRY(hipEventRecord(c->ev_conv, s));
-    CTPN_HIP_TRY(hipStreamWaitEvent(ts, c->ev_conv, 0));
+    CTPN_HIP_TRY(hipEventRecord(f.ev_conv, s));
+    CTPN_HIP_TRY(hipStreamWaitEvent(ts, f.ev_conv, 0));
   }
   {
     Timed t(c, CTPN_KIND_BILSTM, (double)M5 * (1024.0 + 256.0) * 4.0, ts);
     const bool half = dtype_is_half(c->prec);
-    if ((rc = launch_bilstm(c->xp, half ? 1 : 0, c->wh, c->lstm_out, n * hf, wf, ts, (c->lstm_split && c->prec != DType::F32) ? 1 : 0, half ? 1 : 0))) return rc;
+    if ((rc = launch_bilstm(f.xp, half ? 1 : 0, c->wh, f.lstm_out, n * hf, wf, ts, (c->lstm_split && c->prec != DType::F32) ? 1 : 0, half ? 1 : 0))) return rc;
   }
   const bool fold_heads = dtype_is_half(c->prec) && !c->keep_acts;
   if (fold_heads) {
     IGemm g{};
-    g.a = c->lstm_out; g.wt = c->wt_fold; g.bias = c->b_fold; g.out = c->heads;
+    g.a = f.lstm_out; g.wt = c->wt_fold; g.bias = c->b_fold; g.out = f.heads;
     g.M = M5; g.Ci = 256; g.ntaps = 1; g.Co = 60; g.a_plain = 1; g.lda = 256; g.out_bordered = 0; g.ldc = 64; g.relu = 0;
     if ((rc = wait_decoded())) return rc;
     Timed t(c, CTPN_KIND_GEMM, 2.0 * (double)M5 * 256 * 60, ts);
@@ -224,22 +245,22 @@
   } else {
   {
     IGemm g{};
-    g.a = c->lstm_out; g.wt = c->wt_fc; g.bias = c->b_fc; g.out = c->fc_out;
+    g.a = f.lstm_out; g.wt = c->wt_fc; g.bias = c->b_fc; g.out = f.fc_out;
     g.M = M5; g.Ci = 256; g.ntaps = 1; g.Co = 512; g.a_plain = 1; g.lda = 256; g.out_bordered = 0; g.ldc = 512; g.relu = 0;
     Timed t(c, CTPN_KIND_GEMM, 2.0 * (double)M5 * 256 * 512, ts);
     if ((rc = launch_igemm(g, DType::F32, DType::F32, ts))) return rc;
   }
   {
     IGemm g{};
-    g.a = c->fc_out; g.wt = c->wt_h; g.bias = c->b_h; g.out = c->heads;
+    g.a = f.fc_out; g.wt = c->wt_h; g.bias = c->b_h; g.out = f.heads;
     g.M = M5; g.Ci = 512; g.ntaps = 1; g.Co = 60; g.a_plain = 1; g.lda = 512; g.out_bordered = 0; g.ldc = 64; g.relu = 0;
     if ((rc = wait_decoded())) return rc;
     Timed t(c, CTPN_KIND_GEMM, 2.0 * (double)M5 * 512 * 60, ts);
     if ((rc = launch_igemm(g, DType::F32, DType::F32, ts))) return rc;
   }
   }
-  if (tail_on_p) { CTPN_HIP_TRY(hipEventRecord(c->ev_tail, ts)); c->tail_pending = true; }
-  c->fc_valid = !fold_heads;
+  if (tail_on_p) { CTPN_HIP_TRY(hipEventRecord(f.ev_tail, ts)); f.tail_pending = true; }
+  f.fc_valid = !fold_heads;
   c->forward_done = true;
   c->proposals_done = false;
   return CTPN_OK;
@@ -250,21 +271,24 @@
 extern "C" {
 
 int ctpn_forward(ctpn_ctx* c, const uint8_t* images, int images_on_device, int n, int h, int w) {
-  return forward_impl(c, images, 0, images_on_device, n, h, w);
+  if (!c) return fail(CTPN_ERR_ARG, "null pointer");
+  return forward_impl(c, c->fs[0], images, 0, images_on_device, n, h, w);
 }
 int ctpn_forward_blob(ctpn_ctx* c, const float* blob, int blob_on_device, int n, int h, int w) {
-  return forward_impl(c, blob, 1, blob_on_device, n, h, w);
+  if (!c) return fail(CTPN_ERR_ARG, "null pointer");
+  return forward_impl(c, c->fs[0], blob, 1, blob_on_device, n, h, w);
 }
 
 int ctpn_forward_ragged(ctpn_ctx* c, const uint8_t* canvas, int canvas_on_device, int n, int hc, int w, const int* heights) {
   if (!c || !canvas || !heights) return fail(CTPN_ERR_ARG, "ctpn_forward_ragged: null pointer");
-  return forward_impl(c, canvas, 0, canvas_on_device, n, hc, w, false, heights, 2);
+  return forward_impl(c, c->fs[0], canvas, 0, canvas_on_device, n, hc, w, false, heights, 2);
 }
 
 int ctpn_feat_shape(ctpn_ctx* c, int* n, int* hf, int* wf) {
   if (!c) return fail(CTPN_ERR_ARG, "null ctx");
   if (!c->forward_done) return fail(CTPN_ERR_STATE, "no forward yet");
-  if (n) *n = c->n; if (hf) *hf = lvl(c->h, 4); if (wf) *wf = lvl(c->w, 4);
+  const ctpn_ctx::FwdSet& f = *c->last;
+  if (n) *n = f.n; if (hf) *hf = lvl(f.h, 4); if (wf) *wf = lvl(f.w, 4);
   return CTPN_OK;
 }
 
@@ -272,20 +296,21 @@
   if (!c || !name || !out_host) return fail(CTPN_ERR_ARG, "null pointer");
   if (!c->forward_done) return fail(CTPN_ERR_STATE, "ctpn_get_tensor: no forward yet");
   CTPN_HIP_TRY(hipSetDevice(c->device));
+  const ctpn_ctx::FwdSet& f = *c->last;
   const std::string nm(name);
-  const int n = c->n, hf = lvl(c->h, 4), wf = lvl(c->w, 4);
+  const int n = f.n, hf = lvl(f.h, 4), wf = lvl(f.w, 4);
   const void* src = nullptr; int H = 0, W = 0, C = 0, ld = 0; bool bordered = false; DType t = DType::F32;
-  for (int i = 0; i < 14; ++i) if (nm == kConvs[i].name && !c->act_valid[i])
+  for (int i = 0; i < 14; ++i) if (nm == kConvs[i].name && !f.act_valid[i])
     return fail(CTPN_ERR_STATE, "ctpn_get_tensor: " + nm + (i == 0 ? " is computed inside conv1_2's window stage" : " is fused with its max-pool") + " and not stored; set the ctx option keep_acts = 1 (ctpn_set_option)");
-  for (int i = 0; i < 14; ++i) if (nm == kConvs[i].name) { src = c->act_conv[i]; H = lvl(c->h, kConvs[i].level); W = lvl(c->w, kConvs[i].level); C = kConvs[i].co; ld = C; bordered = true; t = c->prec; }
+  for (int i = 0; i < 14; ++i) if (nm == kConvs[i].name) { src = f.act_conv[i]; H = lvl(f.h, kConvs[i].level); W = lvl(f.w, kConvs[i].level); C = kConvs[i].co; ld = C; bordered = true; t = c->prec; }
   const int pool_src[4] = {1, 3, 6, 9};
-  for (int p = 0; p < 4; ++p) if (nm == kPoolNames[p]) { src = c->act_pool[p]; H = lvl(c->h, p + 1); W = lvl(c->w, p + 1); C = kConvs[pool_src[p]].co; ld = C; bordered = true; t = c->prec; }
-  if (nm == "lstm_pre") { src = c->xp; H = hf; W = wf; C = 1024; ld = 1024; if (dtype_is_half(c->prec)) t = DType::F16; }
-  if (nm == "lstm_out") { src = c->lstm_out; H = hf; W = wf; C = 256; ld = 256; }
-  if (nm == "lstm_o" && !c->fc_valid)
+  for (int p = 0; p < 4; ++p) if (nm == kPoolNames[p]) { src = f.act_pool[p]; H = lvl(f.h, p + 1); W = lvl(f.w, p + 1); C = kConvs[pool_src[p]].co; ld = C; bordered = true; t = c->prec; }
+  if (nm == "lstm_pre") { src = f.xp; H = hf; W = wf; C = 1024; ld = 1024; if (dtype_is_half(c->prec)) t = DType::F16; }
+  if (nm == "lstm_out") { src = f.lstm_out; H = hf; W = wf; C = 256; ld = 256; }
+  if (nm == "lstm_o" && !f.fc_valid)
     return fail(CTPN_ERR_STATE, "ctpn_get_tensor: lstm_o is folded into the heads GEMM in the 16-bit modes; set the ctx option keep_acts = 1 (ctpn_set_option)");
-  if (nm == "lstm_o") { src = c->fc_out; H = hf; W = wf; C = 512; ld = 512; }
-  if (nm == "heads") { src = c->heads; H = hf; W = wf; C = 60; ld = 64; }
+  if (nm == "lstm_o") { src = f.fc_out; H = hf; W = wf; C = 512; ld = 512; }
+  if (nm == "heads") { src = f.heads; H = hf; W = wf; C = 60; ld = 64; }
   if (nm == "rpn_cls_prob_reshape") { src = c->cls_prob; H = hf; W = wf; C = 20; ld = 20; }
   if (nm == "rpn_bbox_pred") { src = c->bbox_pred; H = hf; W = wf; C = 40; ld = 40; }
   if (!src) return fail(CTPN_ERR_ARG, "ctpn_get_tensor: unknown tensor name " + nm);
@@ -294,10 +319,10 @@
   const size_t need = (size_t)n * H * W * C;
   if (shape4) { shape4[0] = n; shape4[1] = H; shape4[2] = W; shape4[3] = C; }
   if (capacity < need) return fail(CTPN_ERR_CAPACITY, "ctpn_get_tensor: output buffer too small");
-  CTPN_HIP_TRY(hipStreamSynchronize(c->stream));
+  CTPN_HIP_TRY(hipStreamSynchronize(f.stream));
   CTPN_HIP_TRY(hipStreamSynchronize(c->stream_p));
   const bool split = t == DType::SPLIT;
-  if (split) ld = (src == c->act_conv[13] ? 3 : 2) * C;
+  if (split) ld = (src == f.act_conv[13] ? 3 : 2) * C;
   const int es = split ? 2 : dtype_bytes(t);
   const int Hs = bordered ? H + 2 : H, Ws = bordered ? W + 2 : W;
   const size_t bytes = (size_t)n * Hs * Ws * ld * es;
@@ -309,7 +334,7 @@
       for (int x = 0; x < W; ++x) {
         const size_t sp = (((size_t)in * Hs + y + o) * Ws + x + o) * ld;
         float* d = out_host + (((size_t)in * H + y) * W + x) * C;
-        if (src == c->xp) {
+        if (src == f.xp) {
           if (es == 2) {
             const uint16_t* sh = (const uint16_t*)tmp.data() + sp;
             for (int ch = 0; ch < 1024; ++ch) d[ch] = host_f16_to_f32(sh[(ch & ~511) + lstm_gate_col(ch & 511)]);
diff --git a/text-detection-ctpn_amd/csrc/api_proposals.hip b/text-detection-ctpn_amd/csrc/api_proposals.hip
--- a/text-detection-ctpn_amd/csrc/api_proposals.hip
+++ b/text-detection-ctpn_amd/csrc/api_proposals.hip
@@ -69,7 +69,7 @@
     const int hv = c->debug_hog;
     const int usec = hv > 100000 ? hv - 100000 : hv > 50000 ? hv - 50000 : hv, touch = hv > 100000 ? 4 : hv > 50000 ? 2 : 0;
     const void* src = nullptr; size_t src_bytes = 0;
-    for (int i = 0; i < 14; ++i) if (c->act_conv[i] && c->act_conv_bytes[i] > src_bytes) { src = c->act_conv[i]; src_bytes = c->act_conv_bytes[i]; }
+    for (int i = 0; i < 14; ++i) if (c->fs[0].act_conv[i] && c->act_conv_bytes[i] > src_bytes) { src = c->fs[0].act_conv[i]; src_bytes = c->act_conv_bytes[i]; }
     if ((rc = launch_hog((unsigned*)(c->nms_colid), touch == 4 ? 2 * n : n, usec, touch, s, src, src_bytes))) return rc;
   }
   {
@@ -134,8 +134,10 @@
   if (!c) return fail(CTPN_ERR_ARG, "null ctx");
   if (!c->forward_done) return fail(CTPN_ERR_STATE, "ctpn_proposals: no forward yet");
   CTPN_HIP_TRY(hipSetDevice(c->device));
-  const int* valid = c->fwd_ragged >= 0 ? c->ragged[c->fwd_ragged].dev + c->n : nullptr;
-  return run_proposals(c, c->heads, 0, c->n, lvl(c->h, 4), lvl(c->w, 4), im_info, pre_nms_topn, post_nms_topn, nms_thresh, min_size,
+  const ctpn_ctx::FwdSet& f = *c->last;
+  if (f.stream != c->stream) CTPN_HIP_TRY(hipStreamSynchronize(f.stream));
+  const int* valid = f.fwd_ragged >= 0 ? c->ragged[f.fwd_ragged].dev + f.n : nullptr;
+  return run_proposals(c, f.heads, 0, f.n, lvl(f.h, 4), lvl(f.w, 4), im_info, pre_nms_topn, post_nms_topn, nms_thresh, min_size,
                        rois_out, counts_out, valid);
 }
 
diff --git a/text-detection-ctpn_amd/csrc/conv3x3.hip b/text-detection-ctpn_amd/csrc/conv3x3.hip
--- a/text-detection-ctpn_amd/csrc/conv3x3.hip
+++ b/text-detection-ctpn_amd/csrc/conv3x3.hip
@@ -85,12 +85,28 @@
   static hipEvent_t ev_fork[16] = {nullptr}, ev_join[16] = {nullptr};
   static std::mutex strip_mu[16];
   std::unique_lock<std::mutex> strip_lock;
-  const bool instream = strip && plan.deep != 0;
+  const bool deep = strip && plan.deep != 0;
+  const bool instream = deep || (strip && (split_opts & 4) != 0);
   auto run_edge = [&](void* dst, bool pooled) -> int {
     hipStream_t es = instream ? s : sstream[dev];
     if (split) return c3_edge_split(in, wt, bias, dst, n, h, w, ci, co, relu, r, pooled, es, true, dup_hi, plan.edge_ks);
-    return t == DType::F16 ? c3_edge_f16(in, wt, bias, dst, n, h, w, ci, co, relu, r, pooled, es, instream)
-                           : c3_edge_bf16(in, wt, bias, dst, n, h, w, ci, co, relu, r, pooled, es, instream);
+    return t == DType::F16 ? c3_edge_f16(in, wt, bias, dst, n, h, w, ci, co, relu, r, pooled, es, deep)
+                           : c3_edge_bf16(in, wt, bias, dst, n, h, w, ci, co, relu, r, pooled, es, deep);
+  };
+  auto run_strip = [&](hipStream_t es) -> int {
+    if (edge_pool) {
+      if ((rc = run_edge(pool_out, true))) return rc;
+      if (out && (rc = run_edge(out, false))) return rc;
+    } else if (edge) {
+      if ((rc = run_edge(out, false))) return rc;
+    } else {
+      IGemm ig{};
+      ig.a = in; ig.wt = wt; ig.bias = bias; ig.out = out;
+      ig.M = (long long)n * h * r; ig.Ci = ci; ig.ntaps = 9; ig.Co = co;
+      ig.a_plain = 0; ig.H = h; ig.W = w; ig.rx0 = w - r; ig.rw = r; ig.out_bordered = 1; ig.ldc = co; ig.relu = relu;
+      if ((rc = launch_igemm(ig, t, t, es))) return rc;
+    }
+    return CTPN_OK;
   };
   if (strip && !instream) {
     strip_lock = std::unique_lock<std::mutex>(strip_mu[dev]);
@@ -101,18 +117,7 @@
     }
     CTPN_HIP_TRY(hipEventRecord(ev_fork[dev], s));
     CTPN_HIP_TRY(hipStreamWaitEvent(sstream[dev], ev_fork[dev], 0));
-    if (edge_pool) {
-      if ((rc = run_edge(pool_out, true))) return rc;
-      if (out && (rc = run_edge(out, false))) return rc;
-    } else if (edge) {
-      if ((rc = run_edge(out, false))) return rc;
-    } else {
-      IGemm ig{};
-      ig.a = in; ig.wt = wt; ig.bias = bias; ig.out = out;
-      ig.M = (long long)n * h * r; ig.Ci = ci; ig.ntaps = 9; ig.Co = co;
-      ig.a_plain = 0; ig.H = h; ig.W = w; ig.rx0 = w - r; ig.rw = r; ig.out_bordered = 1; ig.ldc = co; ig.relu = relu;
-      if ((rc = launch_igemm(ig, t, t, sstream[dev]))) return rc;
-    }
+    if ((rc = run_strip(sstream[dev]))) return rc;
     CTPN_HIP_TRY(hipEventRecord(ev_join[dev], sstream[dev]));
   }
   switch (t) {
@@ -122,12 +127,8 @@
     default: rc = c3_run_split(g, pool, plan.main_form, s); break;
   }
   if (rc) return rc;
-  if (instream) {
-    if (edge_pool) {
-      if ((rc = run_edge(pool_out, true))) return rc;
-      if (out && (rc = run_edge(out, false))) return rc;
-    } else if ((rc = run_edge(out, false))) return rc;
-  } else if (strip) CTPN_HIP_TRY(hipStreamWaitEvent(s, ev_join[dev], 0));
+  if (instream) { if ((rc = run_strip(s))) return rc; }
+  else if (strip) CTPN_HIP_TRY(hipStreamWaitEvent(s, ev_join[dev], 0));
   return CTPN_OK;
 }
 
diff --git a/text-detection-ctpn_amd/csrc/ctx.h b/text-detection-ctpn_amd/csrc/ctx.h
--- a/text-detection-ctpn_amd/csrc/ctx.h
+++ b/text-detection-ctpn_amd/csrc/ctx.h
@@ -26,7 +26,7 @@
     {"conv5_3", 512, 512, 4, 0}, {"rpn_conv/3x3", 512, 512, 4, 0}};
 static const char* kPoolNames[4] = {"pool1", "pool2", "pool3", "pool4"};
 
-struct ProfRec { int kind; hipEvent_t a, b; double work; int launches = 1; };
+struct ProfRec { int kind; hipEvent_t a, b; double work; int launches = 1; bool span = false; };
 
 class HostPool {
  public:
@@ -120,15 +120,12 @@
     double* crecs = nullptr; int* ccnt = nullptr;
     hipEvent_t ev_heads = nullptr, ev_decoded = nullptr, ev_done = nullptr;
     int n = 0, h = 0, w = 0; bool busy = false;
+    int set = 0;
     std::vector<int> hts;
   } slot[2];
-  hipEvent_t ev_last_decoded = nullptr;
   hipEvent_t ev_last_done = nullptr;
   int tail_confine = 0;
   int tail_overlap = 0;
-  hipEvent_t ev_conv = nullptr;
-  hipEvent_t ev_tail = nullptr;
-  bool tail_pending = false;
 
   bool weights_loaded = false;
   float* arena = nullptr;
@@ -194,7 +191,6 @@
   int split_edge = 1;
   int conv_p64 = 1;
   int conv1_fuse = 1;
-  void* q_img = nullptr;
   size_t q_img_bytes = 0;
   int lstm_split = 0;
   int nms_check = 0;
@@ -212,9 +208,30 @@
   float* wt_fold = nullptr;
   float* b_fold = nullptr;
 
-  void* act_conv[14] = {nullptr};
-  void* act_pool[4] = {nullptr};
-  bool act_valid[14] = {true, true, true, true, true, true, true, true, true, true, true, true, true, true};
+  struct FwdSet {
+    hipStream_t stream = nullptr;
+    void* q_img = nullptr;
+    void* act_conv[14] = {nullptr};
+    void* act_pool[4] = {nullptr};
+    bool act_valid[14] = {true, true, true, true, true, true, true, true, true, true, true, true, true, true};
+    float* xp = nullptr;
+    float* lstm_out = nullptr;
+    float* fc_out = nullptr;
+    float* heads = nullptr;
+    bool fc_valid = true;
+    float* ragged_blob = nullptr; size_t ragged_blob_bytes = 0;
+    int fwd_ragged = -1;
+    int n = 0, h = 0, w = 0;
+    int gn = -1, gh = -1, gw = -1;
+    hipEvent_t ev_conv = nullptr, ev_tail = nullptr;
+    bool tail_pending = false;
+    hipEvent_t ev_decoded = nullptr; int dec_slot = -1;
+    hipEvent_t ev_gate = nullptr; bool gate_valid = false;
+    std::vector<void*> allocs;
+  } fs[2];
+  size_t set1_bytes = 0;
+  int set1_state = 0;
+  FwdSet* last = &fs[0];
   size_t act_conv_bytes[14] = {0};
   size_t act_pool_bytes[4] = {0};
   uint8_t* img_dev = nullptr;
@@ -227,10 +244,6 @@
   hipEvent_t ev_h2d_done[2] = {nullptr, nullptr};
   bool h2d_valid[2] = {false, false};
   int img_flip = 0;
-  float* xp = nullptr;
-  float* lstm_out = nullptr;
-  float* fc_out = nullptr;
-  float* heads = nullptr;
   float* cls_prob = nullptr;
   float* bbox_pred = nullptr;
   size_t m5_max = 0;
@@ -266,7 +279,6 @@
   bool postproc_only = false;
   std::unique_ptr<ctpn::HostPool> pool;
   int host_threads = 1;
-  bool fc_valid = true;
   int keep_acts = 0;
   float* cls_in = nullptr;
   float* bbox_in = nullptr;
@@ -275,11 +287,7 @@
     int* host = nullptr; int* dev = nullptr;
     hipEvent_t ev_copied = nullptr; bool copied_valid = false;
   } ragged[3];
-  float* ragged_blob = nullptr; size_t ragged_blob_bytes = 0;
-  int fwd_ragged = -1;
-
-  int n = 0, h = 0, w = 0;
-  int gn = -1, gh = -1, gw = -1;
+
   bool forward_done = false;
 
   bool prof = false;
@@ -348,8 +356,16 @@
   }
 };
 
-int forward_impl(ctpn_ctx* c, const void* images, int is_f32, int images_on_device, int n, int h, int w, bool tail_on_p = false,
-                 const int* heights = nullptr, int rset = 2);
+int forward_impl(ctpn_ctx* c, ctpn_ctx::FwdSet& f, const void* images, int is_f32, int images_on_device, int n, int h, int w, bool tail_on_p = false,
+                 const int* heights = nullptr, int rset = 2, bool beside = false);
+bool forward_fuses_conv1(const ctpn_ctx* c, int is_f32, int n, int h, int w, const int* heights);
+int two_forwards_mode();
+bool ensure_set1(ctpn_ctx* c, bool need_conv1);
+static inline hipError_t sync_forwards(ctpn_ctx* c) {
+  const hipError_t e = hipStreamSynchronize(c->stream);
+  if (e != hipSuccess || !c->fs[1].stream) return e;
+  return hipStreamSynchronize(c->fs[1].stream);
+}
 int enqueue_proposals(ctpn_ctx* c, const float* heads, int heads_are_probs, int n, int hf, int wf, const float* im_info,
                       int pre_nms_topn, int post_nms_topn, float nms_thresh, float min_size, hipStream_t s = nullptr,
                       hipEvent_t ev_decoded = nullptr, const int* valid_rows_dev = nullptr );
```
